# cure-lab/MagicDrive

Hardware: AMD Instinct MI355X
Metric: 6-view scenes/sec at 224x400, 50-step DDIM (higher is better)
Workload: dtype bf16; 1 GPU; configs[1]: 6-view 224x400, text-only conditioning (camera_param=None -> CFG off), 50-step DDIM, bf16; scenes_per_gpu=64, ddim_steps=50, scheduler=ddim, parallelism=scene-sharded x1, hipgraph=True, streams=2, output_type=latent

## Files before the change

include/mdx.h:

```cpp
#ifndef MDX_H_
#define MDX_H_

#include <stdint.h>

#ifdef __cplusplus
extern "C" {
#endif

#define MDX_OK 0
#define MDX_EINVAL (-1)
#define MDX_ELAUNCH (-2)
#define MDX_EUNSUPPORTED (-3)

#define MDX_ABI_VERSION 10

#define MDX_EPI_NONE 0
#define MDX_EPI_GEGLU 1
#define MDX_EPI_SILU 2

typedef struct MdxGemmDesc {
    const void* A; const void* W; void* C; const void* R;
    const float* bias; const float* temb; const int32_t* sel_ptr; float* ws;
    int64_t M, N, K;
    int64_t lda, ldw, ldc, ldr;
    int64_t batch, sA, sW, sC, sR;
    int64_t temb_sel_stride, temb_b_stride, rows_per_b;
    int64_t epilogue, splitk;
    int64_t c_is_f32;
    int64_t ws_bytes;
    void* Vt;
    int64_t vt_from, vt_T, vt_ld, vt_stride;
    double ln_eps;
    const float* ln_csum;
    void* ln_scratch;
    float* rowstat_out;
    int64_t rowstat_parts;
    const float* ln_stats;
    int64_t ln_stats_parts;
    const void* Wq;
} MdxGemmDesc;
int mdx_gemm_bf16(const MdxGemmDesc* d, void* stream);

typedef struct MdxConvDesc {
    const void* X; const void* Wt; void* Y; const void* R;
    const float* bias; const float* temb; const int32_t* sel_ptr; float* ws;
    int64_t B, Hi, Wi, Cin, Ho, Wo, Cout;
    int64_t kh, kw, sh, sw, ph, pw;
    int64_t ldx, ldy, ldr;
    int64_t temb_sel_stride, temb_b_stride;
    int64_t epilogue, splitk;
    int64_t ws_bytes, reserved1;
} MdxConvDesc;
int mdx_conv2d_bf16(const MdxConvDesc* d, void* stream);

typedef struct MdxConvDirectDesc {
    const void* X; const void* Wt; void* Y; const void* R;
    const float* bias; const float* temb; const int32_t* sel_ptr; void* reserved_p;
    int64_t B, Hi, Wi, Cin, Ho, Wo, Cout;
    int64_t kh, kw, sh, sw, ph, pw;
    int64_t ldx, ldy, ldr;
    int64_t temb_sel_stride, temb_b_stride;
    int64_t epilogue, x_is_f32, y_is_f32, reserved0;
} MdxConvDirectDesc;
int mdx_conv2d_direct(const MdxConvDirectDesc* d, void* stream);

typedef struct MdxAttnDesc {
    const void* Q; const void* K; const void* Vt; void* O;
    const int32_t* kvmap; void* reserved_p;
    int64_t B, H, Tq, Tk, d, nsrc;
    int64_t ldq, sQ, ldk, sK, ldv, sV, ldo, sO;
    double scale;
    int64_t joint;
    int64_t q_prescaled;
} MdxAttnDesc;
int mdx_attention_bf16(const MdxAttnDesc* d, void* stream);

typedef struct MdxGroupNormDesc {
    const void* X; void* Y; const float* gamma; const float* beta;
    int64_t B, HW, C, G, ldx, ldy;
    double eps;
    int64_t silu;
    float* ws; int64_t ws_bytes;
} MdxGroupNormDesc;
int mdx_groupnorm_bf16(const MdxGroupNormDesc* d, void* stream);

typedef struct MdxLayerNormDesc {
    const void* X; void* Y; const float* gamma; const float* beta;
    int64_t M, C, ldx, ldy;
    double eps;
    int64_t reserved0;
} MdxLayerNormDesc;
int mdx_layernorm_bf16(const MdxLayerNormDesc* d, void* stream);

typedef struct MdxSoftmaxDesc {
    const float* X; void* Y;
    int64_t rows, T, ldx, ldy;
    double scale;
    int64_t reserved0;
} MdxSoftmaxDesc;
int mdx_softmax_rows(const MdxSoftmaxDesc* d, void* stream);

#define MDX_EW_ADD 1
#define MDX_EW_COPY 2
#define MDX_EW_UPSAMPLE 3
#define MDX_EW_NCHW_TO_NHWC 4
#define MDX_EW_NHWC_TO_NCHW 5
#define MDX_EW_SILU 6
#define MDX_EW_SCALE 7
typedef struct MdxEwDesc {
    const void* X; void* Y; const int32_t* ymap; const int32_t* xmap;
    int64_t kind, M, C, ldx, ldy;
    int64_t B, Hi, Wi, Ho, Wo;
    int64_t x_is_f32, y_is_f32;
    double alpha;
} MdxEwDesc;
int mdx_elementwise(const MdxEwDesc* d, void* stream);

typedef struct MdxFourierDesc {
    const float* X; void* Y; const uint8_t* mask; const float* null_feat;
    int64_t n, P, F, ldy;
} MdxFourierDesc;
int mdx_fourier_embed(const MdxFourierDesc* d, void* stream);

typedef struct MdxGatherDesc {
    const void* T; void* Y; const int64_t* idx; const uint8_t* mask; const void* null_row; void* reserved_p;
    int64_t n, C, ldt, ldy, n_rows, reserved0;
} MdxGatherDesc;
int mdx_gather_rows(const MdxGatherDesc* d, void* stream);

typedef struct MdxTimeEmbDesc {
    const float* t; float* Y;
    int64_t n, dim, flip_sin_to_cos, ldy;
    double freq_shift, max_period;
} MdxTimeEmbDesc;
int mdx_timestep_embedding(const MdxTimeEmbDesc* d, void* stream);

typedef struct MdxDdimDesc {
    float* x; const float* eps; const float* coef; int32_t* step_ptr; void* x_in; void* reserved_p;
    int64_t n, cfg;
    double guidance;
    int64_t xin_c, xin_ld;
    const float* gv_cond; const float* gv_noise; const uint8_t* gv_mask;
    int64_t gv_mode, gv_view_elems, gv_last_step;
} MdxDdimDesc;
int mdx_cfg_ddim_step(const MdxDdimDesc* d, void* stream);

typedef struct MdxUniPCDesc {
    float* x; const float* eps; const float* coef; int32_t* step_ptr; void* x_in; float* x_last; float* m1; float* m2;
    int64_t n, cfg;
    double guidance;
    int64_t xin_c, xin_ld;
    const float* gv_cond; const float* gv_noise; const uint8_t* gv_mask;
    int64_t gv_mode, gv_view_elems, gv_last_step;
} MdxUniPCDesc;
int mdx_cfg_unipc_step(const MdxUniPCDesc* d, void* stream);

#define MDX_OP_GEMM 1
#define MDX_OP_CONV 2
#define MDX_OP_CONV_DIRECT 3
#define MDX_OP_ATTN 4
#define MDX_OP_GROUPNORM 5
#define MDX_OP_LAYERNORM 6
#define MDX_OP_EW 7
#define MDX_OP_FOURIER 8
#define MDX_OP_GATHER 9
#define MDX_OP_TIMEEMB 10
#define MDX_OP_DDIM 11
#define MDX_OP_UNIPC 12
#define MDX_OP_SOFTMAX 13

#define MDX_DTYPE_BF16 0
#define MDX_DTYPE_F16 1

#define MDX_OP_BYTES 512
typedef struct MdxOp {
    int64_t opcode;
    int64_t dtype;
    unsigned char desc[MDX_OP_BYTES - 16];
} MdxOp;

int mdx_gemm_f16(const MdxGemmDesc* d, void* stream);
int mdx_conv2d_f16(const MdxConvDesc* d, void* stream);
int mdx_conv2d_direct_f16(const MdxConvDirectDesc* d, void* stream);
int mdx_attention_f16(const MdxAttnDesc* d, void* stream);
int mdx_groupnorm_f16(const MdxGroupNormDesc* d, void* stream);
int mdx_layernorm_f16(const MdxLayerNormDesc* d, void* stream);
int mdx_elementwise_f16(const MdxEwDesc* d, void* stream);
int mdx_fourier_embed_f16(const MdxFourierDesc* d, void* stream);
int mdx_gather_rows_f16(const MdxGatherDesc* d, void* stream);
int mdx_timestep_embedding_f16(const MdxTimeEmbDesc* d, void* stream);
int mdx_cfg_ddim_step_f16(const MdxDdimDesc* d, void* stream);
int mdx_cfg_unipc_step_f16(const MdxUniPCDesc* d, void* stream);
int mdx_softmax_rows_f16(const MdxSoftmaxDesc* d, void* stream);

int mdx_program_run(const MdxOp* ops, int64_t n, void* stream);

int mdx_graph_create(const MdxOp* ops, int64_t n, void** graph_out);
int mdx_graph_launch(void* graph, void* stream);
int mdx_graph_destroy(void* graph);

int mdx_abi_version(void);
const char* mdx_build_id(void);
const char* mdx_last_error(void);
const char* mdx_last_kernel(void);
// ... 11 lines not shown
```

magicdrive_amd/_lib.py:

```python
from __future__ import annotations

import ctypes as C
import os
from typing import Dict, List, Tuple

_HERE = os.path.dirname(os.path.abspath(__file__))
LIB_PATH = os.environ.get("MDX_LIB_PATH") or os.path.join(_HERE, "libmdx.so")

ABI_VERSION = 10

OP_GEMM, OP_CONV, OP_CONV_DIRECT, OP_ATTN, OP_GROUPNORM, OP_LAYERNORM = 1, 2, 3, 4, 5, 6
OP_EW, OP_FOURIER, OP_GATHER, OP_TIMEEMB, OP_DDIM, OP_UNIPC, OP_SOFTMAX = 7, 8, 9, 10, 11, 12, 13
OP_BYTES = 512

EPI_NONE, EPI_GEGLU, EPI_SILU = 0, 1, 2
EW_ADD, EW_COPY, EW_UPSAMPLE, EW_NCHW_TO_NHWC, EW_NHWC_TO_NCHW, EW_SILU, EW_SCALE = 1, 2, 3, 4, 5, 6, 7

P, I, D = C.c_void_p, C.c_int64, C.c_double


def _struct(name: str, fields: List[Tuple[str, object]]):
    return type(name, (C.Structure,), {"_fields_": fields})


def _f(kind, names: str):
    return [(n, kind) for n in names.split()]


MdxGemmDesc = _struct("MdxGemmDesc", _f(P, "A W C R bias temb sel_ptr ws") + _f(I, "M N K lda ldw ldc ldr batch sA sW sC sR "
                      "temb_sel_stride temb_b_stride rows_per_b epilogue splitk c_is_f32 ws_bytes") + _f(P, "Vt") + _f(I, "vt_from vt_T vt_ld vt_stride")
                      + _f(D, "ln_eps") + _f(P, "ln_csum ln_scratch") + _f(P, "rowstat_out") + _f(I, "rowstat_parts") + _f(P, "ln_stats") + _f(I, "ln_stats_parts") + _f(P, "Wq"))
MdxConvDesc = _struct("MdxConvDesc", _f(P, "X Wt Y R bias temb sel_ptr ws") + _f(I, "B Hi Wi Cin Ho Wo Cout kh kw sh sw ph pw "
                      "ldx ldy ldr temb_sel_stride temb_b_stride epilogue splitk ws_bytes reserved1"))
MdxConvDirectDesc = _struct("MdxConvDirectDesc", _f(P, "X Wt Y R bias temb sel_ptr reserved_p") + _f(I, "B Hi Wi Cin Ho Wo Cout kh kw sh sw ph pw "
                            "ldx ldy ldr temb_sel_stride temb_b_stride epilogue x_is_f32 y_is_f32 reserved0"))
MdxAttnDesc = _struct("MdxAttnDesc", _f(P, "Q K Vt O kvmap reserved_p") + _f(I, "B H Tq Tk d nsrc ldq sQ ldk sK ldv sV ldo sO")
                      + _f(D, "scale") + _f(I, "joint q_prescaled"))
MdxGroupNormDesc = _struct("MdxGroupNormDesc", _f(P, "X Y gamma beta") + _f(I, "B HW C G ldx ldy") + _f(D, "eps") + _f(I, "silu") + _f(P, "ws") + _f(I, "ws_bytes"))
MdxLayerNormDesc = _struct("MdxLayerNormDesc", _f(P, "X Y gamma beta") + _f(I, "M C ldx ldy") + _f(D, "eps") + _f(I, "reserved0"))
MdxEwDesc = _struct("MdxEwDesc", _f(P, "X Y ymap xmap") + _f(I, "kind M C ldx ldy B Hi Wi Ho Wo x_is_f32 y_is_f32") + _f(D, "alpha"))
MdxFourierDesc = _struct("MdxFourierDesc", _f(P, "X Y mask null_feat") + _f(I, "n P F ldy"))
MdxGatherDesc = _struct("MdxGatherDesc", _f(P, "T Y idx mask null_row reserved_p") + _f(I, "n C ldt ldy n_rows reserved0"))
MdxTimeEmbDesc = _struct("MdxTimeEmbDesc", _f(P, "t Y") + _f(I, "n dim flip_sin_to_cos ldy") + _f(D, "freq_shift max_period"))
MdxDdimDesc = _struct("MdxDdimDesc", _f(P, "x eps coef step_ptr x_in reserved_p") + _f(I, "n cfg") + _f(D, "guidance") + _f(I, "xin_c xin_ld")
                      + _f(P, "gv_cond gv_noise gv_mask") + _f(I, "gv_mode gv_view_elems gv_last_step"))
MdxUniPCDesc = _struct("MdxUniPCDesc", _f(P, "x eps coef step_ptr x_in x_last m1 m2") + _f(I, "n cfg") + _f(D, "guidance") + _f(I, "xin_c xin_ld")
                       + _f(P, "gv_cond gv_noise gv_mask") + _f(I, "gv_mode gv_view_elems gv_last_step"))

MdxSoftmaxDesc = _struct("MdxSoftmaxDesc", _f(P, "X Y") + _f(I, "rows T ldx ldy") + _f(D, "scale") + _f(I, "reserved0"))
DESC_OF_OP = {
    OP_GEMM: MdxGemmDesc, OP_CONV: MdxConvDesc, OP_CONV_DIRECT: MdxConvDirectDesc, OP_ATTN: MdxAttnDesc,
    OP_GROUPNORM: MdxGroupNormDesc, OP_LAYERNORM: MdxLayerNormDesc, OP_EW: MdxEwDesc, OP_FOURIER: MdxFourierDesc,
    OP_GATHER: MdxGatherDesc, OP_TIMEEMB: MdxTimeEmbDesc, OP_DDIM: MdxDdimDesc, OP_UNIPC: MdxUniPCDesc, OP_SOFTMAX: MdxSoftmaxDesc,
}
DTYPE_BF16, DTYPE_F16 = 0, 1
ENTRY_OF_OP = {
    OP_GEMM: "mdx_gemm_bf16", OP_CONV: "mdx_conv2d_bf16", OP_CONV_DIRECT: "mdx_conv2d_direct", OP_ATTN: "mdx_attention_bf16",
    OP_GROUPNORM: "mdx_groupnorm_bf16", OP_LAYERNORM: "mdx_layernorm_bf16", OP_EW: "mdx_elementwise",
    OP_FOURIER: "mdx_fourier_embed", OP_GATHER: "mdx_gather_rows", OP_TIMEEMB: "mdx_timestep_embedding", OP_DDIM: "mdx_cfg_ddim_step",
    OP_UNIPC: "mdx_cfg_unipc_step", OP_SOFTMAX: "mdx_softmax_rows",
}
def entry_name(opcode: int, dtype: int = DTYPE_BF16) -> str:
    n = ENTRY_OF_OP[opcode]
    if dtype == DTYPE_BF16:
        return n
    return (n[:-5] if n.endswith("_bf16") else n) + "_f16"


EXPORTS = sorted(set(ENTRY_OF_OP.values()) | {entry_name(o, DTYPE_F16) for o in ENTRY_OF_OP} | {
    "mdx_program_run", "mdx_graph_create", "mdx_graph_launch", "mdx_graph_destroy",
    "mdx_abi_version", "mdx_build_id", "mdx_last_error", "mdx_last_kernel", "mdx_device_info", "mdx_set_option", "mdx_get_option", "mdx_option_name"})


class MdxOp(C.Structure):
    _fields_ = [("opcode", I), ("dtype", I), ("desc", C.c_ubyte * (OP_BYTES - 16))]


assert C.sizeof(MdxOp) == OP_BYTES
for _d in DESC_OF_OP.values():
    assert C.sizeof(_d) <= OP_BYTES - 16 and C.sizeof(_d) % 8 == 0


class MdxError(RuntimeError):
    pass


_LIB = None


def lib() -> C.CDLL:
    global _LIB
    if _LIB is not None:
        return _LIB
    if not os.path.exists(LIB_PATH):
        raise MdxError(
            f"{LIB_PATH} not found: build it with `python -c 'import __graft_entry__ as g; g.build()'` "
            f"or `make -C magicdrive_amd/csrc`. magicdrive_amd has no CPU / PyTorch fallback.")
    l = C.CDLL(LIB_PATH)
    for name in EXPORTS:
        if not hasattr(l, name):
            raise MdxError(f"libmdx.so does not export {name}")
    for name in list(ENTRY_OF_OP.values()) + [entry_name(o, DTYPE_F16) for o in ENTRY_OF_OP]:
        fn = getattr(l, name)
        fn.restype = C.c_int
        fn.argtypes = [C.c_void_p, C.c_void_p]
    l.mdx_program_run.restype = C.c_int
    l.mdx_program_run.argtypes = [C.c_void_p, C.c_int64, C.c_void_p]
    l.mdx_graph_create.restype = C.c_int
    l.mdx_graph_create.argtypes = [C.c_void_p, C.c_int64, C.POINTER(C.c_void_p)]
    l.mdx_graph_launch.restype = C.c_int
    l.mdx_graph_launch.argtypes = [C.c_void_p, C.c_void_p]
    l.mdx_graph_destroy.restype = C.c_int
    l.mdx_graph_destroy.argtypes = [C.c_void_p]
    l.mdx_abi_version.restype = C.c_int
    l.mdx_last_error.restype = C.c_char_p
    l.mdx_build_id.restype = C.c_char_p
    l.mdx_last_kernel.restype = C.c_char_p
    l.mdx_device_info.restype = C.c_int
    l.mdx_device_info.argtypes = [C.POINTER(C.c_int64)]
    l.mdx_set_option.restype = C.c_int
    l.mdx_set_option.argtypes = [C.c_char_p, C.c_int64]
    l.mdx_get_option.restype = C.c_int
    l.mdx_get_option.argtypes = [C.c_char_p, C.POINTER(C.c_int64)]
    l.mdx_option_name.restype = C.c_char_p
    l.mdx_option_name.argtypes = [C.c_int64]
    if l.mdx_abi_version() != ABI_VERSION:
        raise MdxError(f"libmdx.so ABI {l.mdx_abi_version()} != expected {ABI_VERSION}")
    _LIB = l
    return l


def check(rc: int, what: str = "") -> None:
    if rc != 0:
        msg = lib().mdx_last_error()
        raise MdxError(f"{what} failed (rc={rc}): {msg.decode() if msg else ''}")


def call_op(opcode: int, desc: C.Structure, stream: int, dtype: int = DTYPE_BF16) -> None:
    name = entry_name(opcode, dtype)
    fn = getattr(lib(), name)
    check(fn(C.byref(desc), C.c_void_p(stream)), name)


class Program:

    def __init__(self, ops: List[Tuple]):
        self.n = len(ops)
        self.buf = (MdxOp * max(self.n, 1))()
        for i, t in enumerate(ops):
            code, desc = t[0], t[1]
            self.buf[i].opcode = code
            self.buf[i].dtype = t[2] if len(t) > 2 else DTYPE_BF16
            C.memmove(C.addressof(self.buf[i]) + 16, C.byref(desc), C.sizeof(desc))
        self._graph = C.c_void_p(None)

    def run(self, stream: int) -> None:
        check(lib().mdx_program_run(C.byref(self.buf), self.n, C.c_void_p(stream)), "mdx_program_run")

    def capture(self) -> None:
        if not self._graph:
            check(lib().mdx_graph_create(C.byref(self.buf), self.n, C.byref(self._graph)), "mdx_graph_create")

    def launch(self, stream: int) -> None:
        if not self._graph:
            self.capture()
        check(lib().mdx_graph_launch(self._graph, C.c_void_p(stream)), "mdx_graph_launch")

    def destroy(self) -> None:
        if self._graph and _LIB is not None:
            _LIB.mdx_graph_destroy(self._graph)
        self._graph = C.c_void_p(None)

    def __del__(self):
        try:
            self.destroy()
        except Exception:
            pass


def set_option(key: str, value: int) -> None:
    check(lib().mdx_set_option(key.encode(), int(value)), f"mdx_set_option({key})")


def get_option(key: str) -> int:
    v = C.c_int64(0)
    check(lib().mdx_get_option(key.encode(), C.byref(v)), f"mdx_get_option({key})")
# ... 39 lines not shown
```

magicdrive_amd/csrc/gemm_conv.hip:

```cpp
#include "common.h"
#include "launch.h"
#include "options.h"
#include "gemm_params.h"

namespace mdx {


int launch_gemm_ws(const GCParams& p, hipStream_t st);
bool ws_supported(const GCParams& p);
bool ws_fuses_layernorm(const GCParams& p);
int launch_layernorm_plain(const bf16_t* X, bf16_t* Y, int M, int C, long ldx, long ldy, float eps, hipStream_t st);
int launch_rowstat(const bf16_t* X, int M, int C, long ldx, float* stat, int parts, hipStream_t st);
bool ws_emits_rowstat(const GCParams& p);
int launch_gemm_xl(const GCParams& p, bool conv, int bn, hipStream_t st);
bool xl_supported(const GCParams& p, bool conv, int bn);

template <int BM, int BN, int BK, int WM, int WN, bool CONV, bool PIPE>
__global__ __launch_bounds__(WM * WN * 64, (WM * WN >= 8) ? 2 : 1) void gemm_conv_kernel(GCParams p) {
    constexpr int NTH = WM * WN * 64;
    constexpr int LSTR = BK + 8;
    constexpr int KCH = BK / 8;
    constexpr int TM = BM / (WM * 32), TN = BN / (WN * 32);
    constexpr int A_CH = BM * BK / 8 / NTH;
    constexpr int B_CH = BN * BK / 8 / NTH;
// ... 190 lines not shown
        if (t + 1 < nt) store_tile(buf ^ 1);
        __syncthreads();
    }

    if (p.timing) ts2 = __builtin_amdgcn_s_memtime();
    if (coalesced_out) {
        epilogue_coalesced<BM, BN, TM, TN, NTH>(p, zb, m0, n0, wm * TM * 32, wn * TN * 32, lane, tid, acc, smem, er);
        if (p.timing && tid == 0) {
            unsigned long long* t = p.timing + 5 * ((long)tile_n * p.mt + tile_m);
            t[0] = ts0; t[1] = ts1; t[2] = ts2; t[3] = __builtin_amdgcn_s_memtime();
            t[4] = 0;
        }
        return;
    }
    const int half = lane >> 5;
#pragma unroll
    for (int i = 0; i < TM; ++i) {
        const int m = m0 + wm * TM * 32 + i * 32 + frow;
        if (m >= p.M) continue;
#pragma unroll
        for (int j = 0; j < TN; ++j) {
#pragma unroll
            for (int g = 0; g < 4; ++g) {
                const int nb = n0 + wn * TN * 32 + j * 32 + 8 * g + 4 * half;
                if (nb >= p.N) continue;
                float v[4] = {acc[i][j][4 * g], acc[i][j][4 * g + 1], acc[i][j][4 * g + 2], acc[i][j][4 * g + 3]};
                if (p.splitk > 1) {
                    float* w = p.ws + ((long)kz * p.M + m) * p.N + nb;
                    *(float4*)w = make_float4(v[0], v[1], v[2], v[3]);
                } else if (p.epi == 1) {
                    if (TN == 2 && j == 0) {
                        float gte[4] = {acc[i][TN - 1][4 * g], acc[i][TN - 1][4 * g + 1],
                                        acc[i][TN - 1][4 * g + 2], acc[i][TN - 1][4 * g + 3]};
                        epilogue_store(p, zb, m, nb, v, gte);
                    }
                } else {
                    epilogue_store(p, zb, m, nb, v, nullptr);
                }
            }
        }
    }
}

__global__ __launch_bounds__(256) void splitk_reduce_kernel(GCParams p) {
    const int n4 = p.N / 4;
    long idx = (long)blockIdx.x * 256 + threadIdx.x;
    if (idx >= (long)p.M * n4) return;
    int m = (int)(idx / n4);
    int nb = (int)(idx - (long)m * n4) * 4;
    const bool geglu = p.epi == 1;
    if (geglu && (nb & 63) >= 32) return;
    const int sel = (p.temb && p.sel) ? *p.sel : 0;
    float bv[4] = {0, 0, 0, 0}, bg[4] = {0, 0, 0, 0}, tv[4] = {0, 0, 0, 0};
    if (p.bias) {
#pragma unroll
        for (int j = 0; j < 4; ++j) { bv[j] = p.bias[nb + j]; if (geglu) bg[j] = p.bias[nb + 32 + j]; }
    }
    if (p.temb && !geglu) {
        const float* tb = p.temb + (long)sel * p.temb_sel_stride + (long)(m / p.rows_per_b) * p.temb_b_stride;
#pragma unroll
        for (int j = 0; j < 4; ++j) tv[j] = tb[nb + j];
    }
    const int ncol = geglu ? (nb >> 6) * 32 + (nb & 63) : nb;
    float rf[4] = {0, 0, 0, 0};
    if (p.R) {
        if (p.c_f32) {
            const float4 r4 = *(const float4*)((const float*)p.R + (long)m * p.ldr + ncol);
            rf[0] = r4.x; rf[1] = r4.y; rf[2] = r4.z; rf[3] = r4.w;
        } else {
            const uint2 rv = *(const uint2*)((const bf16_t*)p.R + (long)m * p.ldr + ncol);
            rf[0] = bf2f((bf16_t)(rv.x & 0xffff)); rf[1] = bf2f((bf16_t)(rv.x >> 16));
            rf[2] = bf2f((bf16_t)(rv.y & 0xffff)); rf[3] = bf2f((bf16_t)(rv.y >> 16));
        }
    }
    float v[4] = {0, 0, 0, 0}, g[4] = {0, 0, 0, 0};
    const float* w0 = p.ws + (long)m * p.N + nb;
    const long zs = (long)p.M * p.N;
    const int last = p.splitk - 1;
    for (int z0 = 0; z0 < p.splitk; z0 += 4) {
        float4 a[4], b[4];
#pragma unroll
        for (int i = 0; i < 4; ++i) {
            const float* w = w0 + (long)min(z0 + i, last) * zs;
            a[i] = *(const float4*)w;
            if (geglu) b[i] = *(const float4*)(w + 32);
        }
#pragma unroll
        for (int i = 0; i < 4; ++i) {
            const bool ok = z0 + i <= last;
            v[0] = ok ? v[0] + a[i].x : v[0]; v[1] = ok ? v[1] + a[i].y : v[1]; v[2] = ok ? v[2] + a[i].z : v[2]; v[3] = ok ? v[3] + a[i].w : v[3];
            if (geglu) { g[0] = ok ? g[0] + b[i].x : g[0]; g[1] = ok ? g[1] + b[i].y : g[1]; g[2] = ok ? g[2] + b[i].z : g[2]; g[3] = ok ? g[3] + b[i].w : g[3]; }
        }
    }
    float o[4];
#pragma unroll
    for (int j = 0; j < 4; ++j) {
        if (geglu) {
            float h = v[j], gt = g[j];
            if (p.bias) { h += bv[j]; gt += bg[j]; }
            o[j] = h * gelu_erf_f(gt);
        } else {
            float x = v[j];
            if (p.bias) x += bv[j];
            if (p.temb) x += tv[j];
            if (p.epi == 2) x = silu_f(x);
            o[j] = x;
        }
        if (p.R) o[j] += rf[j];
    }
    if (p.c_f32) {
        *(float4*)((float*)p.C + (long)m * p.ldc + ncol) = make_float4(o[0], o[1], o[2], o[3]);
    } else {
        uint2 ov; ov.x = pack2bf(o[0], o[1]); ov.y = pack2bf(o[2], o[3]);
        *(uint2*)((bf16_t*)p.C + (long)m * p.ldc + ncol) = ov;
    }
}

template <int BM, int BN, int BK, int WM, int WN, bool CONV, bool PIPE>
static int launch_one_(const GCParams& p, hipStream_t st) {
    constexpr size_t ring = (size_t)2 * (BM + BN) * (BK + 8) * sizeof(bf16_t), ctile = (size_t)BM * (BN + 8) * 2;
    constexpr size_t smem = ring > ctile ? ring : ctile;
    if (p.rowstat) return set_error(MDX_EINVAL, "gemm_conv_kernel: rowstat_out reached a route that does not emit row statistics");
    auto kern = gemm_conv_kernel<BM, BN, BK, WM, WN, CONV, PIPE>;
    if (int rc = ensure_dyn_smem((const void*)kern, smem, "gemm_conv")) return rc;
    GCParams q = p;
    q.mt = (p.M + BM - 1) / BM; q.nt = (p.N + BN - 1) / BN;
    const int swz = (int)opt(OPT_GEMM_SWZ);
    q.swz = swz && q.nt > 1 && q.mt >= 128;
    const unsigned nblk = q.swz ? (unsigned)((q.mt + 7) / 8 * 8 * q.nt) : (unsigned)(q.mt * q.nt);
    dim3 grid(nblk, 1, p.batch > 1 ? p.batch : p.splitk);
    hipLaunchKernelGGL(kern, grid, dim3(WM * WN * 64), smem, st, q);
    char tag[96];
    snprintf(tag, sizeof tag, "gemm_conv_kernel<%d,%d,%d,%d,%d,%s>", BM, BN, BK, WM, WN, CONV ? "conv" : "gemm");
    return check_launch(tag);
}

template <int BM, int BN, int BK, int WM, int WN, bool CONV>
static int launch_one(const GCParams& p, hipStream_t st) {
    const int pipe = (int)opt(OPT_GEMM_PIPE);
    if constexpr (BM == 128 && BN == 128 && BK == 64 && WM == 2 && WN == 2) {
        if (pipe) return launch_one_<BM, BN, BK, WM, WN, CONV, true>(p, st);
    }
    return launch_one_<BM, BN, BK, WM, WN, CONV, false>(p, st);
}

int launch_gemm_conv(GCParams p, bool conv, hipStream_t st) {
    if (p.M <= 0 || p.N <= 0 || p.K <= 0) return MDX_OK;
    const bool geglu = p.epi == 1;
    {
        const long nout = geglu ? p.N / 2 : p.N;
        const int wide_on = (int)opt(OPT_EPI_WIDE);
        p.wide = wide_on && !p.c_f32 && (nout % 8) == 0 && (p.ldc % 8) == 0 && (p.sC % 8) == 0 && (((uintptr_t)p.C) & 15) == 0 &&
                 (!p.R || ((p.ldr % 8) == 0 && (p.sR % 8) == 0 && (((uintptr_t)p.R) & 15) == 0));
    }
    if (!opt(OPT_LN_STATS)) { p.rowstat = nullptr; p.rowstat_parts = 0; p.ln_stats = nullptr; p.ln_stats_parts = 0; }
    if (geglu && (p.N % 64) != 0) return set_error(MDX_EINVAL, "GEGLU needs packed N %% 64 == 0 (N=%d)", p.N);
    constexpr int impl = 0;
    const int ws_mode = (int)opt(OPT_GEMM_WS);
    const int xl_mode = (int)opt(OPT_GEMM_XL);
    const int xl_k320 = (int)opt(OPT_XL_K320);
    const int xl_min_tiles = (int)opt(OPT_XL_MIN_TILES);
    const int xl_geglu320 = (int)opt(OPT_XL_GEGLU320);
    const bool geglu_xl = xl_geglu320 && xl_mode == 1 && impl == 0 && !conv && geglu && p.K == 320 && p.splitk <= 1 && ws_mode < 2 &&
                          xl_supported(p, false, 256) && (long)((p.M + 255) / 256) * ((p.N + 255) / 256) >= 1024;
    const bool ws_first = !conv && ws_mode > 0 && p.splitk <= 1 && ws_supported(p) && (ws_mode >= 2 || p.M >= 8192);
    const bool ws_taken = impl == 0 && !geglu_xl && ws_first && !(xl_k320 && xl_mode > 0);
    if (p.rowstat) {
        if (conv || p.batch > 1 || p.epi != 0 || p.c_f32 || p.Vt || p.rowstat_parts < 1) return set_error(MDX_EINVAL, "rowstat_out: plain 2-D GEMM with 16-bit C only");
        if (!(ws_taken && ws_emits_rowstat(p) && opt(OPT_LN_FUSE))) {
            GCParams q = p;
            q.rowstat = nullptr; q.rowstat_parts = 0;
            if (int rc = launch_gemm_conv(q, conv, st)) return rc;
            return launch_rowstat((const bf16_t*)p.C, p.M, p.N, p.ldc, p.rowstat, p.rowstat_parts, st);
        }
    }
    auto try_xl = [&](int& bn_out) -> bool {
        if (impl != 0 || xl_mode <= 0 || p.splitk > 1) return false;
        const int xl_bn = (int)opt(OPT_XL_BN);
        double best = 1e300;
        bn_out = 0;
        const double nslab = p.K / 64.0;
        for (int bn : {320, 256, 160}) {
            if (xl_bn && bn != xl_bn) continue;
            if (!xl_supported(p, conv, bn)) continue;
            const long t = (long)((p.M + 255) / 256) * ((p.N + bn - 1) / bn);
            if (xl_mode < 2 && t < xl_min_tiles) continue;
            const double a = bn == 320 ? 23.7 : bn == 256 ? 13.4 : 16.6, b = bn == 320 ? 1.896 : bn == 256 ? 1.565 : 1.116;
            const double c = (double)((t + 255) / 256) * (a + b * nslab);
            if (c < best) { best = c; bn_out = bn; }
        }
        return bn_out != 0;
    };
    if (p.ln_eps > 0.f) {
        if (conv || p.batch > 1) return set_error(MDX_EINVAL, "fused LayerNorm: plain 2-D GEMM only");
        if (!(ws_taken && ws_fuses_layernorm(p) && opt(OPT_LN_FUSE))) {
            if (!p.ln_scratch) return set_error(MDX_EINVAL, "fused LayerNorm: this shape is not normalised in-kernel and no ln_scratch was given");
            if (int rc = launch_layernorm_plain(p.A, p.ln_scratch, p.M, p.K, p.lda, p.lda, p.ln_eps, st)) return rc;
            p.A = p.ln_scratch; p.ln_eps = 0.f; p.ln_csum = nullptr; p.ln_stats = nullptr; p.ln_stats_parts = 0;
        }
    }
    if (xl_mode >= 2 && p.splitk <= 1 && p.batch <= 1 && !(p.K == 320 && !conv && !xl_k320)) {
        GCParams q = p;
        q.splitk = 1;
        int bn_f;
        const int keep = p.splitk;
        p.splitk = 1;
        const bool ok = try_xl(bn_f);
        p.splitk = keep;
        if (ok) return launch_gemm_xl(q, conv, bn_f, st);
    }
    if (geglu_xl) return launch_gemm_xl(p, false, 256, st);
    if (ws_taken) return launch_gemm_ws(p, st);
    int BM, BN;
    {
        BN = 128;
        if (!geglu && (p.N <= 64 || (p.N % 128 != 0 && p.N <= 192))) BN = 64;
        BM = p.M >= 2048 ? 128 : 64;
        if (opt(OPT_GEMM_SMALL_TILES) && p.batch <= 1) {
            const long t64 = (long)((p.M + 63) / 64) * ((p.N + 63) / 64);
            if (geglu) {
                BM = p.M >= 512 ? 128 : 64;
            } else if (!conv) {
                if (t64 <= 1408) BM = BN = 64;
            } else if (t64 * (long)((p.K + 63) / 64) <= 40000) {
                BM = BN = 64;
            } else if (BN == 128) {
                BM = 128;
            }
        }
        const int big = (int)opt(OPT_GEMM_BM256);
        if (big && BN == 128 && p.M >= big) BM = 256;
        const int fbm = (int)opt(OPT_GEMM_BM), fbn = (int)opt(OPT_GEMM_BN);
        if (fbm == 64 || fbm == 128) BM = fbm;
        if ((fbn == 64 && !geglu) || fbn == 128) BN = fbn;
    }
    long tiles = (long)((p.M + BM - 1) / BM) * ((p.N + BN - 1) / BN) * (p.batch > 1 ? p.batch : 1);
    int splitk = 1;
    if (p.splitk > 0) {
        splitk = p.splitk;
    } else if (p.batch <= 1 && p.ws && tiles < 384 && p.K >= 1024 && (p.N % 4) == 0) {
        long want = (768 + tiles - 1) / tiles;
        long maxs = p.K / 512;
        splitk = (int)min(min(want, maxs), 32L);
        if (splitk < 1) splitk = 1;
    }
    if (p.batch > 1) splitk = 1;
    if (splitk > 1) {
        long per = (long)p.M * p.N * (long)sizeof(float);
        long fit = per > 0 ? p.ws_bytes / per : 0;
        if (fit < splitk) splitk = fit < 1 ? 1 : (int)fit;
    }
    constexpr int BK = 64;
    int kchunk = ((p.K + splitk - 1) / splitk + BK - 1) / BK * BK;
    splitk = (p.K + kchunk - 1) / kchunk;
    if (splitk > 1 && !p.ws) return set_error(MDX_EINVAL, "split-K needs a workspace");
    p.splitk = splitk;
    p.kchunk = kchunk;
    const int timing = (int)opt(OPT_GEMM_TIMING);
    p.timing = (timing && p.ws && splitk == 1) ? (unsigned long long*)p.ws : nullptr;
    if (splitk == 1) {
        int bn_xl;
        if (try_xl(bn_xl)) return launch_gemm_xl(p, conv, bn_xl, st);
    }
    if (impl == 0 && ws_first) return launch_gemm_ws(p, st);
    int rc;
    {
        const int bk = (int)opt(OPT_GEMM_BK);
#define MDX_GC2(BM_, BN_, BK_, WM_, WN_) (conv ? launch_one<BM_, BN_, BK_, WM_, WN_, true>(p, st) : launch_one<BM_, BN_, BK_, WM_, WN_, false>(p, st))
#define MDX_GC(BM_, BN_) (bk == 32 ? MDX_GC2(BM_, BN_, 32, 2, 2) : MDX_GC2(BM_, BN_, 64, 2, 2))
        if (BM == 256 && BN == 128) rc = (bk == 32) ? MDX_GC2(256, 128, 32, 4, 2) : MDX_GC2(256, 128, 64, 4, 2);
        else if (BM == 128 && BN == 128) rc = MDX_GC(128, 128);
        else if (BM == 128 && BN == 64) rc = MDX_GC(128, 64);
        else if (BM == 64 && BN == 128) rc = MDX_GC(64, 128);
        else rc = MDX_GC(64, 64);
#undef MDX_GC2
#undef MDX_GC
    }
    if (rc != MDX_OK) return rc;
    if (splitk > 1) {
        long n = (long)p.M * (p.N / 4);
        hipLaunchKernelGGL(splitk_reduce_kernel, dim3((unsigned)((n + 255) / 256)), dim3(256), 0, st, p);
        return check_launch("splitk_reduce_kernel", false);
    }
    return MDX_OK;
}

}

using namespace mdx;

static int check_common(const char* op, int64_t K, int64_t lda, int64_t ldw, int64_t ldc, int64_t ldr, const void* A, const void* W,
                        const void* C, const char* nA, const char* nW, const char* nC, const char* nlda, const char* nldc) {
    MDX_NEED(need_multiple(op, "K", K, 8));
    MDX_NEED(need_multiple(op, nlda, lda, 8));
    MDX_NEED(need_multiple(op, "ldw", ldw, 8));
    MDX_NEED(need_multiple(op, nldc, ldc, 4));
    MDX_NEED(need_multiple(op, "ldr", ldr, 4));
    MDX_NEED(need_aligned(op, nA, A, 16));
    MDX_NEED(need_aligned(op, nW, W, 16));
    MDX_NEED(need_aligned(op, nC, C, 8));
    return MDX_OK;
}

static int check_epilogue_operands(const char* op, const void* R, const float* bias, const float* temb, const int32_t* sel, const float* ws,
                                   int64_t temb_sel_stride, int64_t temb_b_stride) {
    MDX_NEED(need_aligned(op, "R", R, 8));
    MDX_NEED(need_aligned(op, "bias", bias, 16));
    MDX_NEED(need_aligned(op, "temb", temb, 16));
    MDX_NEED(need_aligned(op, "sel_ptr", sel, 4));
    MDX_NEED(need_aligned(op, "ws", ws, 16));
    if (temb) {
        MDX_NEED(need_multiple(op, "temb_sel_stride", temb_sel_stride, 4));
        MDX_NEED(need_multiple(op, "temb_b_stride", temb_b_stride, 4));
    }
    return MDX_OK;
}

static int launch_gemm_flat(const mdx::GCParams& q, hipStream_t st) {
    using namespace mdx;
    const int xl_mode = (int)opt(OPT_GEMM_XL);
    if (xl_mode <= 0) return MDX_EUNSUPPORTED;
    double best = 1e300; int bn_best = 0;
    for (int bn : {320, 256, 160}) {
        if (!xl_supported(q, false, bn)) continue;
        const long t = (long)((q.M + 255) / 256) * ((q.N + bn - 1) / bn);
        if (t < 128) continue;
        const double a = bn == 320 ? 23.7 : bn == 256 ? 13.4 : 16.6, b = bn == 320 ? 1.896 : bn == 256 ? 1.565 : 1.116;
        const double c = (double)((t + 255) / 256) * (a + b * q.K / 64.0);
        if (c < best) { best = c; bn_best = bn; }
    }
    if (!bn_best) return MDX_EUNSUPPORTED;
    return launch_gemm_xl(q, false, bn_best, st);
}

extern "C" int mdx_gemm_bf16(const MdxGemmDesc* d, void* stream) {
    if (!d || !d->A || !d->W || !d->C) return set_error(MDX_EINVAL, "mdx_gemm_bf16: null operand");
    const char* op = "mdx_gemm_bf16";
    MDX_NEED(need_int(op, "M", d->M)); MDX_NEED(need_int(op, "N", d->N)); MDX_NEED(need_int(op, "K", d->K));
    MDX_NEED(need_int(op, "batch", d->batch)); MDX_NEED(need_int(op, "rows_per_b", d->rows_per_b));
    MDX_NEED(need_int(op, "splitk", d->splitk));
    MDX_NEED(check_common(op, d->K, d->lda, d->ldw, d->ldc, d->ldr, d->A, d->W, d->C, "A", "W", "C", "lda", "ldc"));
    MDX_NEED(check_epilogue_operands(op, d->R, d->bias, d->temb, d->sel_ptr, d->ws, d->temb_sel_stride, d->temb_b_stride));
    if (d->c_is_f32) {
        MDX_NEED(need_aligned(op, "C (fp32)", d->C, 16));
        MDX_NEED(need_aligned(op, "R (fp32)", d->R, 16));
    }
    if (d->batch > 1) {
        MDX_NEED(need_multiple(op, "sA", d->sA, 8)); MDX_NEED(need_multiple(op, "sW", d->sW, 8));
        MDX_NEED(need_multiple(op, "sC", d->sC, 4)); MDX_NEED(need_multiple(op, "sR", d->sR, 4));
    }
    if (d->N % 4) {
        if (d->bias || d->temb || d->R || d->epilogue || d->splitk > 1 || d->ldc < (d->N + 3) / 4 * 4)
            return set_error(MDX_EINVAL, "N=%ld not a multiple of 4 needs a plain epilogue and ldc >= roundup4(N)", (long)d->N);
    }
    GCParams p = {};
    p.A = (const bf16_t*)d->A; p.W = (const bf16_t*)d->W; p.C = d->C; p.R = d->R;
    p.bias = d->bias; p.temb = d->temb; p.sel = d->sel_ptr; p.ws = d->ws;
    p.M = (int)d->M; p.N = (int)d->N; p.K = (int)d->K;
    p.lda = d->lda; p.ldw = d->ldw; p.ldc = d->ldc; p.ldr = d->ldr;
    p.batch = d->batch > 1 ? (int)d->batch : 1;
    p.sA = d->sA; p.sW = d->sW; p.sC = d->sC; p.sR = d->sR;
    p.temb_sel_stride = d->temb_sel_stride; p.temb_b_stride = d->temb_b_stride;
    p.rows_per_b = d->rows_per_b > 0 ? (int)d->rows_per_b : 1;
    p.epi = (int)d->epilogue; p.splitk = (int)d->splitk; p.c_f32 = (int)d->c_is_f32; p.ws_bytes = d->ws_bytes;
    if (d->ln_eps > 0.0) {
        if (!d->ln_csum || p.batch > 1 || d->splitk > 1 || d->c_is_f32 || d->temb || ((uintptr_t)d->ln_scratch & 15))
            return set_error(MDX_EINVAL, "mdx_gemm_bf16: fused LayerNorm needs ln_csum, one batch, no split-K / fp32 C / temb, 16-byte aligned ln_scratch");
        p.ln_eps = (float)d->ln_eps; p.ln_csum = d->ln_csum; p.ln_scratch = (bf16_t*)d->ln_scratch;
        if (d->ln_stats) {
            if (d->ln_stats_parts < 1 || ((uintptr_t)d->ln_stats & 7)) return set_error(MDX_EINVAL, "mdx_gemm_bf16: ln_stats needs ln_stats_parts >= 1 and 8-byte alignment");
            p.ln_stats = d->ln_stats; p.ln_stats_parts = (int)d->ln_stats_parts;
        }
    } else if (d->ln_stats) {
        return set_error(MDX_EINVAL, "mdx_gemm_bf16: ln_stats without ln_eps");
    }
    if (d->Wq) {
        if ((uintptr_t)d->Wq & 15) return set_error(MDX_EINVAL, "mdx_gemm_bf16: Wq must be 16-byte aligned");
        p.Wq = (const bf16_t*)d->Wq;
    }
    if (d->rowstat_out) {
        if (d->rowstat_parts < 1 || ((uintptr_t)d->rowstat_out & 7) || d->Vt || d->epilogue || d->c_is_f32 || p.batch > 1)
            return set_error(MDX_EINVAL, "mdx_gemm_bf16: rowstat_out needs rowstat_parts >= 1, 8-byte alignment, a plain epilogue, 16-bit C, one batch, no Vt");
        p.rowstat = d->rowstat_out; p.rowstat_parts = (int)d->rowstat_parts;
    }
    if (d->Vt) {
        p.Vt = (bf16_t*)d->Vt; p.vt_from = (int)d->vt_from; p.vt_T = (int)d->vt_T; p.vt_ld = d->vt_ld; p.vt_stride = d->vt_stride;
        if (!ws_supported(p) || d->epilogue || d->R || (d->vt_from % 128) || d->vt_from <= 0 || d->vt_from >= d->N || d->vt_T <= 0 ||
            (d->vt_T % 8) || (d->M % d->vt_T) || (d->vt_ld % 8) || (d->vt_stride % 8) || ((uintptr_t)d->Vt & 15))
            return set_error(MDX_EINVAL, "mdx_gemm_bf16: transposed V output needs K=320, plain epilogue, no residual, vt_from %% 128 == 0, vt_T %% 8 == 0, aligned Vt");
        if (!opt(OPT_LN_STATS)) { p.ln_stats = nullptr; p.ln_stats_parts = 0; }
        if (p.ln_eps > 0.f && !opt(OPT_LN_FUSE)) {
            if (!p.ln_scratch) return set_error(MDX_EINVAL, "fused LayerNorm: LN_FUSE=0 needs ln_scratch");
            if (int rc2 = launch_layernorm_plain(p.A, p.ln_scratch, p.M, p.K, p.lda, p.lda, p.ln_eps, (hipStream_t)stream)) return rc2;
            p.A = p.ln_scratch; p.ln_eps = 0.f; p.ln_csum = nullptr; p.ln_stats = nullptr; p.ln_stats_parts = 0;
        }
        { GCParams q = p; const long nout = d->vt_from;
          q.wide = (nout % 8) == 0 && (p.ldc % 8) == 0 && (((uintptr_t)p.C) & 15) == 0;
          return launch_gemm_ws(q, (hipStream_t)stream); }
    }
    const int flatten = (int)opt(OPT_GEMM_FLATTEN);
    if (flatten && p.batch > 1 && p.sA == 0 && p.sW == (long)p.N * p.ldw && !p.bias && !p.temb && !p.R && !p.epi && !p.c_f32 && p.splitk <= 1 &&
        (long)p.batch * p.N < 0x7fffff00L && ((long)p.batch * p.N) % 4 == 0) {
        GCParams q = p;
        q.col_split = p.N; q.N = p.batch * p.N; q.batch = 1; q.sW = 0; q.wide = 0;
        int rcq = launch_gemm_flat(q, (hipStream_t)stream);
        if (rcq != MDX_EUNSUPPORTED) return rcq;
    }
    return launch_gemm_conv(p, false, (hipStream_t)stream);
}

extern "C" int mdx_conv2d_bf16(const MdxConvDesc* d, void* stream) {
    if (!d || !d->X || !d->Wt || !d->Y) return set_error(MDX_EINVAL, "mdx_conv2d_bf16: null operand");
    if (d->Cin % 8) return set_error(MDX_EINVAL, "mdx_conv2d_bf16: Cin=%ld must be a multiple of 8", (long)d->Cin);
    const char* op = "mdx_conv2d_bf16";
    MDX_NEED(need_int(op, "B", d->B)); MDX_NEED(need_int(op, "Hi", d->Hi)); MDX_NEED(need_int(op, "Wi", d->Wi)); MDX_NEED(need_int(op, "Cin", d->Cin));
    MDX_NEED(need_int(op, "Ho", d->Ho)); MDX_NEED(need_int(op, "Wo", d->Wo)); MDX_NEED(need_int(op, "Cout", d->Cout));
    MDX_NEED(need_int(op, "kh", d->kh)); MDX_NEED(need_int(op, "kw", d->kw)); MDX_NEED(need_int(op, "sh", d->sh)); MDX_NEED(need_int(op, "sw", d->sw));
    MDX_NEED(need_int(op, "ph", d->ph)); MDX_NEED(need_int(op, "pw", d->pw)); MDX_NEED(need_int(op, "splitk", d->splitk));
    if (d->B < 0 || d->Ho < 0 || d->Wo < 0 || d->kh < 0 || d->kw < 0 || d->Cin < 0) return set_error(MDX_EINVAL, "%s: negative size", op);
    MDX_NEED(need_int(op, "Ho * Wo", d->Ho * d->Wo));
    MDX_NEED(need_int(op, "B * Ho * Wo", d->B * (d->Ho * d->Wo)));
    MDX_NEED(need_int(op, "kh * kw", d->kh * d->kw));
    int64_t K = d->kh * d->kw * d->Cin;
    MDX_NEED(need_int(op, "kh * kw * Cin", K));
    MDX_NEED(check_common(op, K, d->ldx, K, d->ldy, d->ldr, d->X, d->Wt, d->Y, "X", "Wt", "Y", "ldx", "ldy"));
    MDX_NEED(check_epilogue_operands(op, d->R, d->bias, d->temb, d->sel_ptr, d->ws, d->temb_sel_stride, d->temb_b_stride));
    if (d->epilogue == MDX_EPI_GEGLU) return set_error(MDX_EINVAL, "conv has no GEGLU epilogue");
    if (d->Cout % 4) return set_error(MDX_EINVAL, "mdx_conv2d_bf16: Cout=%ld must be a multiple of 4", (long)d->Cout);
    GCParams p = {};
    p.A = (const bf16_t*)d->X; p.W = (const bf16_t*)d->Wt; p.C = d->Y; p.R = d->R;
    p.bias = d->bias; p.temb = d->temb; p.sel = d->sel_ptr; p.ws = d->ws;
    p.M = (int)(d->B * d->Ho * d->Wo); p.N = (int)d->Cout; p.K = (int)K;
    p.lda = d->ldx; p.ldw = K; p.ldc = d->ldy; p.ldr = d->ldr;
    p.batch = 1;
    p.temb_sel_stride = d->temb_sel_stride; p.temb_b_stride = d->temb_b_stride;
    p.rows_per_b = (int)(d->Ho * d->Wo);
    p.epi = (int)d->epilogue; p.splitk = (int)d->splitk; p.c_f32 = 0; p.ws_bytes = d->ws_bytes;
    p.Hi = (int)d->Hi; p.Wi = (int)d->Wi; p.Cin = (int)d->Cin; p.Ho = (int)d->Ho; p.Wo = (int)d->Wo;
    p.kh = (int)d->kh; p.kw = (int)d->kw; p.sh = (int)d->sh; p.sw = (int)d->sw; p.ph = (int)d->ph; p.pw = (int)d->pw;
    const int cim = (int)opt(OPT_CONV_CIMAJOR);
    p.cimajor = (cim && d->kh * d->kw > 1 && d->Cin % 64 == 0) ? 1 : 0;
    return launch_gemm_conv(p, true, (hipStream_t)stream);
}
```

magicdrive_amd/csrc/gemm_params.h:

```cpp
#pragma once
#include "common.h"

namespace mdx {

struct GCParams {
    const bf16_t* A; const bf16_t* W; void* C; const void* R;
    const float* bias; const float* temb; const int* sel; float* ws;
    int M, N, K;
    long lda, ldw, ldc, ldr;
    long sA, sW, sC, sR;
    long temb_sel_stride, temb_b_stride;
    int rows_per_b;
    int epi, splitk, kchunk, c_f32, batch;
    long ws_bytes;
    int mt, nt, swz;
    int gm, gn;
    int nblk;
    unsigned long long* timing;
    int Hi, Wi, Cin, Ho, Wo, kh, kw, sh, sw, ph, pw;
    int cimajor;
    int wide;
    bf16_t* Vt; int vt_from, vt_T; long vt_ld, vt_stride;
    int col_split;
    const float* ln_csum; float ln_eps; bf16_t* ln_scratch;
    float* rowstat; int rowstat_parts;
    const float* ln_stats; int ln_stats_parts;
    const bf16_t* Wq;
    int dbg;
};

__device__ __forceinline__ bool tile_coords_at(const GCParams& p, int bid, int& tm, int& tn) {
    if (!p.swz) { tm = bid % p.mt; tn = bid / p.mt; return true; }
    const int xcd = bid & 7, local = bid >> 3;
    tn = local % p.nt;
    tm = (local / p.nt) * 8 + xcd;
    return tm < p.mt;
}
__device__ __forceinline__ bool tile_coords(const GCParams& p, int& tm, int& tn) { return tile_coords_at(p, (int)blockIdx.x, tm, tn); }

__device__ __forceinline__ void epilogue_store(const GCParams& p, long zb, int m, int nb,
                                               const float* v, const float* gte) {
    float o[4];
    int ncol;
    const float* tb = nullptr;
    if (p.temb) {
        int sel = p.sel ? *p.sel : 0;
        tb = p.temb + (long)sel * p.temb_sel_stride + (long)(m / p.rows_per_b) * p.temb_b_stride;
    }
    if (p.epi == 1) {
        ncol = (nb >> 6) * 32 + (nb & 63);
#pragma unroll
        for (int j = 0; j < 4; ++j) {
            float h = v[j], g = gte[j];
            if (p.bias) { h += p.bias[nb + j]; g += p.bias[nb + 32 + j]; }
            o[j] = h * gelu_erf_f(g);
        }
    } else {
        ncol = nb;
#pragma unroll
        for (int j = 0; j < 4; ++j) {
            float x = v[j];
            if (p.bias) x += p.bias[nb + j];
            if (tb) x += tb[nb + j];
            if (p.epi == 2) x = silu_f(x);
            o[j] = x;
        }
    }
    if (p.c_f32) {
        float* c = (float*)p.C + zb * p.sC + (long)m * p.ldc + ncol;
        if (p.R) {
            const float* r = (const float*)p.R + zb * p.sR + (long)m * p.ldr + ncol;
#pragma unroll
            for (int j = 0; j < 4; ++j) o[j] += r[j];
        }
        *(float4*)c = make_float4(o[0], o[1], o[2], o[3]);
    } else {
        bf16_t* c = (bf16_t*)p.C + zb * p.sC + (long)m * p.ldc + ncol;
        if (p.R) {
            const bf16_t* r = (const bf16_t*)p.R + zb * p.sR + (long)m * p.ldr + ncol;
            uint2 rv = *(const uint2*)r;
            o[0] += bf2f((bf16_t)(rv.x & 0xffff)); o[1] += bf2f((bf16_t)(rv.x >> 16));
            o[2] += bf2f((bf16_t)(rv.y & 0xffff)); o[3] += bf2f((bf16_t)(rv.y >> 16));
        }
        uint2 ov; ov.x = pack2bf(o[0], o[1]); ov.y = pack2bf(o[2], o[3]);
        *(uint2*)c = ov;
    }
}


template <int BM, int BN, int TN, int NTHR>
struct EpiRegs {
    static constexpr int IT = (BM * (BN / 8) + NTHR - 1) / NTHR;
    float4 bv[TN][4];
    uint4 rv[IT];
};

template <int BM, int BN, int TN, int NTHR>
__device__ __forceinline__ void epi_prefetch(const GCParams& p, long zb, int m0, int n0, int wcol0, int lane, int tid,
                                             EpiRegs<BM, BN, TN, NTHR>& er) {
    const int half = lane >> 5;
    const float4 z4 = make_float4(0.f, 0.f, 0.f, 0.f);
#pragma unroll
    for (int j = 0; j < TN; ++j)
#pragma unroll
        for (int g = 0; g < 4; ++g) {
            const int nb = n0 + wcol0 + j * 32 + 8 * g + 4 * half;
            er.bv[j][g] = (p.bias && nb < p.N) ? *(const float4*)(p.bias + nb) : z4;
        }
    const bool geglu = p.epi == 1;
    const int cpr = (geglu ? BN / 2 : BN) / 8;
    const int n0o = geglu ? n0 / 2 : n0, Nout = geglu ? p.N / 2 : p.N;
    const bf16_t* Rg = (p.R && p.wide) ? (const bf16_t*)p.R + zb * p.sR : nullptr;
#pragma unroll
    for (int i = 0; i < EpiRegs<BM, BN, TN, NTHR>::IT; ++i) {
        const int idx = tid + i * NTHR;
        const int row = idx / cpr;
        const int c8 = (idx - row * cpr) * 8;
        const int m = m0 + row, n = n0o + c8;
        er.rv[i] = make_uint4(0, 0, 0, 0);
        if (Rg && idx < BM * cpr && m < p.M && n < Nout) er.rv[i] = *(const uint4*)(Rg + (long)m * p.ldr + n);
    }
}

__device__ __forceinline__ unsigned add2bf(unsigned a, unsigned b) {
    return pack2bf(bf2f((bf16_t)(a & 0xffff)) + bf2f((bf16_t)(b & 0xffff)), bf2f((bf16_t)(a >> 16)) + bf2f((bf16_t)(b >> 16)));
}

template <int BM, int BNO, int NTHR, int ITMAX>
__device__ __forceinline__ void store_tile_rows(const GCParams& p, long zb, int m0, int n0o, int Nout, int tid, const bf16_t* Cs,
                                                const uint4 (&rv)[ITMAX]) {
    constexpr int CSTR = BNO + 8;
    bf16_t* Cg = (bf16_t*)p.C + zb * p.sC;
    const bool has_r = p.R != nullptr;
    if (p.wide) {
        constexpr int CPR = BNO / 8;
        constexpr int IT = (BM * CPR + NTHR - 1) / NTHR;
        static_assert(IT <= ITMAX, "residual register tile too small");
#pragma unroll
        for (int i = 0; i < IT; ++i) {
            const int idx = tid + i * NTHR;
            const int row = idx / CPR;
            const int c8 = (idx - row * CPR) * 8;
            const int m = m0 + row, n = n0o + c8;
            if (!((idx < BM * CPR) && m < p.M && n < Nout)) continue;
            uint4 v = *(const uint4*)(Cs + row * CSTR + c8);
            if (has_r) { v.x = add2bf(v.x, rv[i].x); v.y = add2bf(v.y, rv[i].y); v.z = add2bf(v.z, rv[i].z); v.w = add2bf(v.w, rv[i].w); }
            *(uint4*)(Cg + (long)m * p.ldc + n) = v;
        }
        return;
    }
    constexpr int CPR = BNO / 4;
    constexpr int IT = (BM * CPR + NTHR - 1) / NTHR;
    const bf16_t* Rg = has_r ? (const bf16_t*)p.R + zb * p.sR : nullptr;
#pragma unroll 1
    for (int i0 = 0; i0 < IT; i0 += 4) {
        uint2 r2[4];
        bool ok[4];
#pragma unroll
        for (int u = 0; u < 4; ++u) {
            const int idx = tid + (i0 + u) * NTHR;
            const int row = idx / CPR, c4 = (idx - row * CPR) * 4;
            ok[u] = (i0 + u) < IT && idx < BM * CPR && m0 + row < p.M && n0o + c4 < Nout;
            r2[u] = make_uint2(0, 0);
            if (Rg && ok[u]) r2[u] = *(const uint2*)(Rg + (long)(m0 + row) * p.ldr + n0o + c4);
        }
#pragma unroll
        for (int u = 0; u < 4; ++u) {
            if (!ok[u]) continue;
            const int idx = tid + (i0 + u) * NTHR;
            const int row = idx / CPR, c4 = (idx - row * CPR) * 4;
            uint2 v = *(const uint2*)(Cs + row * CSTR + c4);
            if (has_r) { v.x = add2bf(v.x, r2[u].x); v.y = add2bf(v.y, r2[u].y); }
            *(uint2*)(Cg + (long)(m0 + row) * p.ldc + n0o + c4) = v;
        }
    }
}

template <int BM, int BN, int TM, int TN, int NTHR>
__device__ __forceinline__ void epilogue_coalesced(const GCParams& p, long zb, int m0, int n0, int wrow0, int wcol0, int lane,
                                                   int tid, f32x16_t (&acc)[TM][TN], unsigned char* smem,
                                                   const EpiRegs<BM, BN, TN, NTHR>& er) {
    const bool geglu = p.epi == 1;
// ... 65 lines not shown
```

magicdrive_amd/csrc/gemm_xl.hip:

```cpp
#include "common.h"
#include "launch.h"
#include "options.h"
#include "gemm_params.h"
#include "xl_layout.h"
#include "xl_dma.h"
#include <type_traits>

namespace mdx {

using namespace mdx_xl;

constexpr int XL_SLOTS = 12;

__device__ __forceinline__ bool xl_tile_coords_at(const GCParams& p, int bid, int& tm, int& tn) {
    if (p.swz != 2) return tile_coords_at(p, bid, tm, tn);
    return raster_tile(bid, p.mt, p.nt, p.gm, p.gn, &tm, &tn);
}
__device__ __forceinline__ bool xl_tile_coords(const GCParams& p, int& tm, int& tn) { return xl_tile_coords_at(p, (int)blockIdx.x, tm, tn); }

template <int BN, bool CONV, int SCHED>
__global__ __launch_bounds__(512, 2) void gemm_xl_kernel(GCParams p) {
    using G = Geo<BN>;
    constexpr int BM = 256, NTH = 512;
    constexpr int TI = G::TI, TJ = G::TJ, TJ0 = G::TJ0, TJ1 = TJ - TJ0, TIH = TI / 2;
    constexpr int A_BYTES = BM * 128, B_BYTES = G::BNP * 128, BUF = A_BYTES + B_BYTES;
    constexpr int PA = G::PA, PB0 = G::PB0, PB1 = G::PB1;
    constexpr int UNIT_MAX = PA > PB0 ? PA : PB0;
    constexpr bool KXS = SCHED == 4;
    static_assert(!KXS || (BN == 320 && CONV), "the shared-tap schedule is the 320-wide conv's");
    constexpr int AS_ROWS = 272, AS_BYTES = AS_ROWS * 128;
    constexpr int ZROW_OFF = 264 * 128;
    constexpr int B_STRIDE = KXS ? (G::BNP * 128) : (BM * 128 + G::BNP * 128);
    constexpr int B_BASE = KXS ? 2 * AS_BYTES - BM * 128 : 0;
    extern __shared__ __attribute__((aligned(16))) unsigned char smem[];

    const int tid = threadIdx.x, lane = tid & 63;
    const int wave = __builtin_amdgcn_readfirstlane(tid >> 6);
    const int grp = wave >> 2;
    const int wm = wave % G::WM, wn = wave / G::WM;
    int tile_m, tile_n;
    if (!xl_tile_coords(p, tile_m, tile_n)) return;
    unsigned long long ts_[8] = {0, 0, 0, 0, 0, 0, 0, 0};
#define XL_STAMP(k) if (p.timing) ts_[k] = __builtin_amdgcn_s_memtime();
    XL_STAMP(0)
    const int m0 = tile_m * BM, n0 = tile_n * BN;
    const int nt = p.K / 64;

    long a_base_el;
    int hw = 1, Wo = 1;
    if (CONV) {
        hw = p.Ho * p.Wo; Wo = p.Wo;
        const int b = m0 / hw, rem = m0 - b * hw;
        const int oy = rem / Wo, ox = rem - oy * Wo;
        a_base_el = (((long)b * p.Hi + (oy * p.sh - p.ph)) * p.Wi + (ox * p.sw - p.pw)) * p.lda;
    } else {
        a_base_el = (long)m0 * p.lda;
    }
    const xl_rsrc_t rsA = xl_make_rsrc(p.A + a_base_el);
    const xl_rsrc_t rsB = xl_make_rsrc(p.W + (long)n0 * p.ldw);
    const unsigned lds0 = (unsigned)(unsigned long long)(lds_void_t*)smem;

    unsigned xs_bits = 0;
    const unsigned xs_vb = (unsigned)((long)(lane >> 3) * p.lda * 2 + (((lane & 7) ^ ((lane >> 3) & 7)) << 4));
    const unsigned xb_vb = (unsigned)((long)(lane >> 3) * p.ldw * 2 + (((lane & 7) ^ ((lane >> 4) & 3)) << 4));
    unsigned a_voff[2][PA];
    unsigned a_taps[2][PA];
    int a_lds[2][PA];
#pragma unroll
    for (int h = 0; h < 2; ++h)
#pragma unroll
        for (int e = 0; e < PA; ++e) {
            const int row0 = a_piece_row0<BN>(h, wave, e);
            a_lds[h][e] = row0 * 128;
            const int R = piece_lane_row(row0, lane);
            const int cl = piece_lane_chunk(row0, lane);
            const int m = m0 + R;
            a_taps[h][e] = 0;
            if constexpr (KXS) {
                const long q = (long)m0 + R - 1;
                unsigned bits = 0;
                if (q >= 0 && q < p.M) {
                    const int b_ = (int)(q / hw), y_ = (int)(q - (long)b_ * hw) / Wo;
#pragma unroll
                    for (int ky = 0; ky < 3; ++ky) if ((unsigned)(y_ + ky - 1) < (unsigned)p.Hi) bits |= 1u << ky;
                }
                xs_bits |= bits << (3 * (2 * h + e));
            } else
            if (CONV) {
                const int mm = min(m, p.M - 1);
                const int b = mm / hw, rem = mm - b * hw;
                const int oy = rem / Wo, ox = rem - oy * Wo;
                const int iy0 = oy * p.sh - p.ph, ix0 = ox * p.sw - p.pw;
                const long pix = ((long)b * p.Hi + iy0) * p.Wi + ix0;
                a_voff[h][e] = (unsigned)((pix * p.lda - a_base_el) * 2 + cl * 16);
                unsigned bits = 0;
#pragma unroll
                for (int t = 0; t < 9; ++t) {
                    const int iy = iy0 + t / 3, ix = ix0 + t % 3;
                    if (m < p.M && (unsigned)iy < (unsigned)p.Hi && (unsigned)ix < (unsigned)p.Wi) bits |= 1u << t;
                }
                a_taps[h][e] = bits;
            } else {
                a_voff[h][e] = m < p.M ? (unsigned)(((long)R * p.lda) * 2 + cl * 16) : XL_OOB;
            }
        }
    unsigned b_voff[2][UNIT_MAX];
    int b_lds[2][UNIT_MAX];
#pragma unroll
    for (int part = 0; part < 2; ++part)
#pragma unroll
        for (int e = 0; e < (part ? PB1 : PB0); ++e) {
            const int row0 = b_piece_row0<BN>(part, wave, e);
            if (row0 < 0) {
                b_lds[part][e] = A_BYTES + b_dummy_row0<BN>(wave) * 128;
                b_voff[part][e] = XL_OOB;
            } else {
                b_lds[part][e] = A_BYTES + row0 * 128;
                const int R = piece_lane_row(row0, lane);
                const int cl = piece_lane_chunk(row0, lane);
                b_voff[part][e] = (n0 + R < p.N) ? (unsigned)(((long)R * p.ldw) * 2 + cl * 16) : XL_OOB;
            }
        }

    if constexpr (KXS) {
        const int R = 256 + (lane >> 3);
        const long q = (long)m0 + R - 1;
        if (wave == 7 && R < 258 && q < p.M) {
            const int b_ = (int)(q / hw), y_ = (int)(q - (long)b_ * hw) / Wo;
#pragma unroll
            for (int ky = 0; ky < 3; ++ky) if ((unsigned)(y_ + ky - 1) < (unsigned)p.Hi) xs_bits |= 1u << (12 + ky);
        }
    }
    const int row_bytes = (int)(p.lda * 2);
    auto a_soff = [&](int T, int& tap) -> int {
        if (CONV) {
            const int cb = T / 9;
            tap = T - cb * 9;
            const int ky = tap / 3, kx = tap - ky * 3;
            return (ky * p.Wi + kx) * row_bytes + cb * 128;
        }
        tap = 0;
        return T * 128;
    };
    auto b_soff = [&](int T) -> int {
        if (CONV) {
            const int cb = T / 9, tap = T - cb * 9;
            return (tap * p.Cin + cb * 64) * 2;
        }
        return T * 128;
    };
#ifdef MDX_XL_ABLATE
    const bool do_mma = !(p.dbg & 1), do_dma = !(p.dbg & 2);
    const bool a_oob = CONV && (p.dbg & 16), a_skip = CONV && (p.dbg & 32);
    const bool a_oob_kx = CONV && (p.dbg & 64);
#else
    constexpr bool do_mma = true, do_dma = true, a_oob = false, a_skip = false, a_oob_kx = false;
#endif
#define XL_PIECE_A(h, e, T)                                                                                                       \
    if constexpr ((e) < PA) {                                                                                                     \
        if ((T) < nt && do_dma && !(a_skip && ((T) % 9) != 0)) {                                                                  \
            int tap_;                                                                                                             \
            const int so_ = a_soff((T), tap_);                                                                                    \
            unsigned vo_ = CONV ? (((a_taps[h][(e) < PA ? (e) : 0] >> tap_) & 1u) ? a_voff[h][(e) < PA ? (e) : 0] : XL_OOB)       \
                                : a_voff[h][(e) < PA ? (e) : 0];                                                                  \
            if ((a_oob && tap_ != 0) || (a_oob_kx && (tap_ % 3) != 0)) vo_ = XL_OOB;                                              \
            xl_glds(rsA, lds0 + ((T) & 1) * BUF + a_lds[h][(e) < PA ? (e) : 0], vo_, so_);                                        \
        }                                                                                                                         \
    }
#define XL_PIECE_B(part, e, T)                                                                                                    \
    if constexpr ((e) < ((part) ? PB1 : PB0)) {                                                                                   \
        if ((T) < nt && do_dma)                                                                                                   \
            xl_glds_b(rsB, lds0 + ((T) & 1) * B_STRIDE + B_BASE + b_lds[part][(e) < UNIT_MAX ? (e) : 0],                            \
                      b_voff[part][(e) < UNIT_MAX ? (e) : 0], b_soff((T)));                                                       \
    }
#define XL_ISSUE_A(h, T) { XL_PIECE_A(h, 0, T) XL_PIECE_A(h, 1, T) }
#define XS_PIECE_A(h, e, G)                                                                                                       \
    if ((G) < ng && do_dma) {                                                                                                     \
        unsigned va_ = xs_vb;                                                                                                     \
        asm volatile("" : "+v"(va_));                                                                                             \
        const unsigned vo_ = va_ + (unsigned)((a_lds[h][e] >> 7) * row_bytes);                                                    \
        xl_glds(rsA, lds0 + ((G) & 1) * AS_BYTES + a_lds[h][e], ((xs_bits >> (3 * (2 * (h) + (e)) + xs_ky)) & 1u) ? vo_ : XL_OOB, xs_so); \
    }
#define XS_PIECE_B(part, e, T)                                                                                                    \
    if constexpr ((e) < ((part) ? PB1 : PB0)) {                                                                                   \
        if ((T) < nt && do_dma) {                                                                                                 \
            const int r0_ = (b_lds[part][(e) < UNIT_MAX ? (e) : 0] - A_BYTES) >> 7;                                               \
            unsigned vb_ = xb_vb;                                                                                                 \
            asm volatile("" : "+v"(vb_));    \
            const unsigned vo_ = (vb_ ^ (unsigned)(((r0_ >> 3) & 1) << 6)) + (unsigned)(r0_ * (int)(p.ldw * 2));                  \
            xl_glds_b(rsB, lds0 + ((T) & 1) * B_STRIDE + B_BASE + b_lds[part][(e) < UNIT_MAX ? (e) : 0], vo_, b_soff((T)));        \
        }                                                                                                                         \
    }
#define XS_ISSUE_B(part, T) { XS_PIECE_B(part, 0, T) XS_PIECE_B(part, 1, T) XS_PIECE_B(part, 2, T) }
#define XS_ISSUE_A0(G) { XS_PIECE_A(0, 0, G) XS_PIECE_A(0, 1, G) }
#define XS_ISSUE_A1X(G)                                                                                                           \
    {                                                                                                                             \
        XS_PIECE_A(1, 0, G) XS_PIECE_A(1, 1, G)                                                                                   \
        unsigned va2_ = xs_vb;                                                                                                    \
        asm volatile("" : "+v"(va2_));                                                                                            \
        if ((G) < ng && do_dma)                                                                                                   \
            xl_glds(rsA, lds0 + ((G) & 1) * AS_BYTES + (wave == 7 ? 256 * 128 : ZROW_OFF),                                        \
                    ((xs_bits >> (12 + xs_ky)) & 1u) ? va2_ + (unsigned)(256 * row_bytes) : XL_OOB, xs_so);                       \
    }
#define XL_ISSUE_B(part, T) { XL_PIECE_B(part, 0, T) XL_PIECE_B(part, 1, T) XL_PIECE_B(part, 2, T) }

    const int fo0 = frag_off(0, lane, 0), fo1 = frag_off(0, lane, 1);
    const int a_rd = a_tile_row0<BN>(wm, 0) * 128;
    const int b_rd = A_BYTES + b_tile_row0<BN>(wn, 0) * 128;
    if constexpr (KXS) {
#pragma unroll
        for (int i = 0; i < TI; ++i) {
            const int m_ = m0 + a_tile_row0<BN>(wm, i) + (lane & 15);
            const int ox_ = m_ % Wo;
            if (ox_ == 0) xs_bits |= 1u << (16 + i);
            if (ox_ == Wo - 1) xs_bits |= 1u << (24 + i);
        }
    }

    f32x4_t acc[TI][TJ];
#pragma unroll
    for (int i = 0; i < TI; ++i)
#pragma unroll
        for (int j = 0; j < TJ; ++j)
#pragma unroll
            for (int r = 0; r < 4; ++r) acc[i][j][r] = 0.f;

    constexpr int NBF = (BN == 320) ? TJ0 : TJ;
    Frag8 af[TIH][2], bfr[NBF][2];
#define XL_READ_A(h, buf_)                                                                                                        \
    {                                                                                                                             \
        const unsigned char* s_ = smem + (buf_) * BUF + a_rd + (h) * TIH * 2048;                                                  \
        _Pragma("unroll") for (int i = 0; i < TIH; ++i) {                                                                         \
            af[i][0].u = *(const uint4*)(s_ + i * 2048 + fo0);                                                                    \
            af[i][1].u = *(const uint4*)(s_ + i * 2048 + fo1);                                                                    \
        }                                                                                                                         \
    }
#define XS_READ_A(h, ab_)                                                                                                         \
    {                                                                                                                             \
        const unsigned char* s_ = smem + (ab_) * AS_BYTES;                                                                        \
        unsigned bb_ = xs_bsel;                                                                                                   \
        asm volatile("" : "+v"(bb_));    \
        const int f0_ = xs_f0, f1_ = xs_f0 ^ 64;                                                                                  \
        _Pragma("unroll") for (int i = 0; i < TIH; ++i) {                                                                         \
            const int it_ = (h) * TIH + i;                                                                                        \
            const bool z_ = (bb_ >> it_) & 1u;                                                                                    \
            const int o0_ = z_ ? ZROW_OFF - it_ * 2048 : f0_, o1_ = z_ ? ZROW_OFF - it_ * 2048 : f1_;                             \
            af[i][0].u = *(const uint4*)(s_ + o0_ + it_ * 2048);                                                                  \
            af[i][1].u = *(const uint4*)(s_ + o1_ + it_ * 2048);                                                                  \
        }                                                                                                                         \
    }
#define XL_READ_B(J0, NJ, buf_)                                                                                                   \
    {                                                                                                                             \
        const unsigned char* s_ = smem + (buf_) * B_STRIDE + B_BASE + b_rd;                                                       \
        _Pragma("unroll") for (int j = (J0); j < (J0) + (NJ); ++j) {                                                              \
            bfr[j][0].u = *(const uint4*)(s_ + j * 2048 + fo0);                                                                   \
            bfr[j][1].u = *(const uint4*)(s_ + j * 2048 + fo1);                                                                   \
        }                                                                                                                         \
    }
#define XL_READ_B_TO(D0, J0, NJ, buf_)                                                                                            \
    {                                                                                                                             \
        const unsigned char* s_ = smem + (buf_) * B_STRIDE + B_BASE + b_rd;                                                       \
        _Pragma("unroll") for (int j = 0; j < (NJ); ++j) {                                                                        \
            bfr[(D0) + j][0].u = *(const uint4*)(s_ + ((J0) + j) * 2048 + fo0);                                                   \
            bfr[(D0) + j][1].u = *(const uint4*)(s_ + ((J0) + j) * 2048 + fo1);                                                   \
        }                                                                                                                         \
    }
#define XL_MMA_TO(h, D0, J0, NJ)                                                                                                  \
    if (do_mma) {                                                                                                                 \
        __builtin_amdgcn_s_setprio(1);                                                                                            \
        _Pragma("unroll") for (int kk = 0; kk < 2; ++kk)                                                                          \
            _Pragma("unroll") for (int i = 0; i < TIH; ++i)                                                                       \
                _Pragma("unroll") for (int j = 0; j < (NJ); ++j)                                                                  \
                    acc[(h) * TIH + i][(J0) + j] =                                                                                \
                        MDX_MFMA_16x16x32(bfr[(D0) + j][kk].v, af[i][kk].v, acc[(h) * TIH + i][(J0) + j]); \
        __builtin_amdgcn_s_setprio(0);                                                                                            \
    }
#define XL_MMA(h, J0, NJ)                                                                                                         \
    if (do_mma) {                                                                                                                 \
        __builtin_amdgcn_s_setprio(1);                                                                                            \
        _Pragma("unroll") for (int kk = 0; kk < 2; ++kk)                                                                          \
            _Pragma("unroll") for (int i = 0; i < TIH; ++i)                                                                       \
                _Pragma("unroll") for (int j = (J0); j < (J0) + (NJ); ++j)                                                        \
                    acc[(h) * TIH + i][j] =                                                                                       \
                        MDX_MFMA_16x16x32(bfr[j][kk].v, af[i][kk].v, acc[(h) * TIH + i][j]);       \
        __builtin_amdgcn_s_setprio(0);                                                                                            \
    }
#define XL_MSEG(h, I0, I1, I2, I3)                                                                                                \
    {                                                                                                                             \
        __builtin_amdgcn_s_setprio(1);                                                                                            \
        constexpr int P_ = 2 * TIH;                                                                                               \
        _Pragma("unroll") for (int pr = 0; pr < P_; ++pr) {                                                                       \
            const int kk = pr / TIH, i = pr % TIH;                                                                                \
            if (pr == 1) { I0 }                                                                                                   \
            if (pr == 1 + (P_ - 1) / 4) { I1 }                                                                                    \
            if (pr == 1 + 2 * (P_ - 1) / 4) { I2 }                                                                                \
            if (pr == 1 + 3 * (P_ - 1) / 4) { I3 }                                                                                \
            __builtin_amdgcn_sched_barrier(0);                                                                                    \
            if (do_mma) {                                                                                                         \
                _Pragma("unroll") for (int j = 0; j < TJ; ++j)                                                                    \
// ... 170 lines not shown
            XL_READ_B(TJ0, TJ1, buf)
            XL_SEG2(XL_ISSUE_B(0, t + 1))
            XL_MMA(0, TJ0, TJ1)
            XL_MMA_END()
            XL_READ_A(1, buf)
            XL_SEG2(XL_ISSUE_A(0, t + 2))
            XL_MMA(1, TJ0, TJ1)
            XL_MMA_END()
            XL_SEG2(XL_ISSUE_B(1, t + 2) if (t + 2 < nt) xl_wait_vmcnt<PA + PB1>(); else xl_wait_vmcnt<0>();)
            XL_MMA(1, 0, TJ0)
            XL_MMA_END()
        }
#undef XL_SEG2
    } else     if constexpr (SCHED == 0) {
        constexpr int INFLIGHT = PA + PB0 + PB1;
        XL_ISSUE_A(0, 0)
        XL_ISSUE_B(0, 0)
        XL_ISSUE_B(1, 0)
        XL_ISSUE_A(1, 0)
        XL_ISSUE_A(0, 1)
        XL_ISSUE_B(0, 1)
        XL_ISSUE_B(1, 1)
        if (nt > 1) xl_wait_vmcnt<INFLIGHT>(); else xl_wait_vmcnt<0>();
        __builtin_amdgcn_s_barrier();
        __builtin_amdgcn_sched_barrier(0);
        XL_STAMP(2)
        if (grp == 1) {
            __builtin_amdgcn_s_barrier();
            __builtin_amdgcn_sched_barrier(0);
        }
        for (int t = 0; t < nt; ++t) {
            const int buf = t & 1;
            XL_READ_A(0, buf)
            XL_READ_B(0, TJ0, buf)
            XL_ISSUE_A(1, t + 1)
            XL_SEG_END()
            XL_MMA(0, 0, TJ0)
            XL_MMA_END()
            XL_READ_B(TJ0, TJ1, buf)
            XL_ISSUE_A(0, t + 2)
            XL_SEG_END()
            XL_MMA(0, TJ0, TJ1)
            XL_MMA_END()
            XL_READ_A(1, buf)
            XL_ISSUE_B(0, t + 2)
            XL_SEG_END()
            XL_MMA(1, TJ0, TJ1)
            XL_MMA_END()
            XL_ISSUE_B(1, t + 2)
            if (t + 2 < nt) xl_wait_vmcnt<INFLIGHT>(); else xl_wait_vmcnt<0>();
            XL_SEG_END()
            XL_MMA(1, 0, TJ0)
            XL_MMA_END()
        }
    } else {
        XL_ISSUE_A(0, 0)
        XL_ISSUE_B(0, 0)
        XL_ISSUE_B(1, 0)
        XL_ISSUE_A(1, 0)
        XL_ISSUE_A(0, 1)
        XL_ISSUE_B(0, 1)
        if (nt > 1) xl_wait_vmcnt<PA + PB0>(); else xl_wait_vmcnt<0>();
        __builtin_amdgcn_s_barrier();
        __builtin_amdgcn_sched_barrier(0);
        XL_STAMP(2)
        if (grp == 1) {
            __builtin_amdgcn_s_barrier();
            __builtin_amdgcn_sched_barrier(0);
        }
        for (int t = 0; t < nt; ++t) {
            const int buf = t & 1;
            XL_READ_A(0, buf)
            XL_READ_B(0, TJ, buf)
            if (t + 1 < nt) xl_wait_vmcnt<PA + PB0>(); else xl_wait_vmcnt<0>();
            XL_SEG_END()
            XL_MSEG(0, XL_PIECE_B(1, 0, t + 1), XL_PIECE_B(1, 1, t + 1), XL_PIECE_A(1, 0, t + 1), XL_PIECE_A(1, 1, t + 1))
            XL_MMA_END()
            XL_READ_A(1, buf)
            if (t + 1 < nt) xl_wait_vmcnt<PA>();
            XL_SEG_END()
            XL_MSEG(1, XL_PIECE_A(0, 0, t + 2), XL_PIECE_A(0, 1, t + 2), XL_PIECE_B(0, 0, t + 2), XL_PIECE_B(0, 1, t + 2))
            XL_MMA_END()
        }
    }
    if (grp == 0) {
        __builtin_amdgcn_s_barrier();
        __builtin_amdgcn_sched_barrier(0);
    }
#undef XL_PIECE_A
#undef XS_PIECE_A
#undef XS_PIECE_B
#undef XS_ISSUE_B
#undef XS_ISSUE_A0
#undef XS_ISSUE_A1X
#undef XS_READ_A
#undef XL_PIECE_B
#undef XL_ISSUE_A
#undef XL_ISSUE_B
#undef XL_READ_A
#undef XL_READ_B
#undef XL_READ_B_TO
#undef XL_MMA_TO
#undef XL_MMA
#undef XL_MSEG
#undef XL_SEG_END
#undef XL_MMA_END

    XL_STAMP(3)
#ifdef MDX_XL_ABLATE
    if (p.dbg & 4) return;
#endif
    constexpr int NH = (BN == 320) ? 2 : 1;
    constexpr int HROWS = BM / NH;
    const bool geglu = p.epi == 1;
    const bool has_t = p.temb != nullptr && !geglu;
    const int BNo = geglu ? BN / 2 : BN;
    const int CSTR = BNo + 8;
    bf16_t* Cs = (bf16_t*)smem;
    float* addend = (float*)(smem + (size_t)HROWS * (BN + 8) * 2);
    const int b0 = has_t ? m0 / p.rows_per_b : 0;
    if (add_early) {
#pragma unroll
        for (int u = 0; u < ADD_N; ++u) {
            const int idx = u * NTH + tid;
            if (idx < BN) addend[idx] = (n0 + idx < p.N) ? addb[u] : 0.f;
        }
    } else {
        const int nslots = has_t ? XL_SLOTS : 1;
        const int sel = (has_t && p.sel) ? *p.sel : 0;
        const int bmax = has_t ? (p.M - 1) / p.rows_per_b : 0;
        for (int idx = tid; idx < nslots * BN; idx += NTH) {
            const int slot = idx / BN, n = idx - slot * BN, col = n0 + n;
            float v = 0.f;
            if (col < p.N) {
                if (p.bias) v = p.bias[col];
                if (has_t && b0 + slot <= bmax) v += p.temb[(long)sel * p.temb_sel_stride + (long)(b0 + slot) * p.temb_b_stride + col];
            }
            addend[idx] = v;
        }
    }
    const int n0o = geglu ? n0 / 2 : n0, Nout = geglu ? p.N / 2 : p.N;
    const bf16_t* Rg = p.R ? (const bf16_t*)p.R : nullptr;
    bf16_t* Cg = (bf16_t*)p.C;
    constexpr int CPR = BN >> 3;
    constexpr int RPP = NTH / CPR;
    constexpr int RIT = (HROWS + RPP - 1) / RPP;
    const int rrow0 = tid / CPR, rc8 = (tid - rrow0 * CPR) * 8;
    const bool ractive = tid < RPP * CPR && n0 + rc8 < p.N;
#ifdef MDX_XL_R2_RESIDUAL
    const bool rpref = NH == 1 && Rg != nullptr && p.wide && !geglu;
#else
    const bool rpref = Rg != nullptr && p.wide && !geglu;
#endif
    uint4 rpre[RIT];
    auto fetch_residual = [&](int hh) {
        const int mh_ = m0 + hh * HROWS;
        const int c8 = (n0 + rc8 + 8 > p.N) ? (p.N - 8 - n0 < 0 ? 0 : p.N - 8 - n0) : rc8;
        const bf16_t* rb = Rg + n0 + c8;
        const int rmax = min(HROWS - 1, p.M - 1 - mh_);
#pragma unroll
        for (int u = 0; u < RIT; ++u) {
            const int row = min(rrow0 + u * RPP, rmax);
            rpre[u] = *(const uint4*)(rb + (long)(mh_ + row) * p.ldr);
        }
    };
#pragma unroll 1
    for (int hh = 0; hh < NH; ++hh) {
        if (rpref && NH == 1) fetch_residual(hh);
        xl_wait_lgkm0();
        __builtin_amdgcn_s_barrier();
        asm volatile("" ::: "memory");
        XL_STAMP(6)
        {
            const int fr = lane & 15, fq = lane >> 4;
            auto stage = [&](auto epi_c, auto hast_c) {
                constexpr int EPI = decltype(epi_c)::value;
                constexpr bool HAS_T = decltype(hast_c)::value;
                constexpr bool HOIST = BN != 320 && !HAS_T;
                float4 a4h[HOIST ? TJ : 1], g4h[HOIST ? TJ : 1];
                if constexpr (HOIST) {
#pragma unroll
                    for (int j = 0; j < TJ; ++j) {
                        const int nl = wn * TJ * 16 + j * 16 + 4 * fq;
                        a4h[j] = *(const float4*)(addend + nl);
                        if constexpr (EPI == 1) g4h[j] = *(const float4*)(addend + ((nl + 32) < BN ? nl + 32 : nl));
                    }
                }
#pragma unroll
                for (int i = 0; i < TI; ++i) {
                    const int mt_ = wm * TI * 16 + i * 16;
                    if (NH > 1 && mt_ / HROWS != hh) continue;
                    const int ml = mt_ + fr;
                    int slot = 0;
                    if constexpr (HAS_T) slot = min(min(m0 + ml, p.M - 1) / p.rows_per_b - b0, XL_SLOTS - 1);
                    const float* ad = addend + slot * BN;
                    bf16_t* crow = Cs + (ml - hh * HROWS) * CSTR;
#pragma unroll
                    for (int j = 0; j < TJ; ++j) {
                        if (EPI == 1 && (j & 2)) continue;
                        const int nl = wn * TJ * 16 + j * 16 + 4 * fq;
                        float4 a4;
                        if constexpr (HOIST) a4 = a4h[j]; else a4 = *(const float4*)(ad + nl);
                        const float bb[4] = {a4.x, a4.y, a4.z, a4.w};
                        float o[4];
                        if constexpr (EPI == 1) {
                            float4 g4;
                            if constexpr (HOIST) g4 = g4h[j]; else g4 = *(const float4*)(ad + nl + 32);
                            const float gg[4] = {g4.x, g4.y, g4.z, g4.w};
#pragma unroll
                            for (int e = 0; e < 4; e += 2) {
                                const float x0 = acc[i][j][e] + bb[e], x1 = acc[i][j][e + 1] + bb[e + 1];
                                const f32x2_t gt = {acc[i][(TJ == 4) ? (j | 2) : j][e] + gg[e], acc[i][(TJ == 4) ? (j | 2) : j][e + 1] + gg[e + 1]};
                                const f32x2_t ge = gelu_erf_f2(gt);
                                o[e] = x0 * ge.x; o[e + 1] = x1 * ge.y;
                            }
                        } else {
#pragma unroll
                            for (int e = 0; e < 4; ++e) {
                                float x = acc[i][j][e] + bb[e];
                                if constexpr (EPI == 2) x = silu_f(x);
                                o[e] = x;
                            }
                        }
                        const int cl = EPI == 1 ? ((nl >> 6) * 32 + (nl & 31)) : nl;
                        uint2 ov; ov.x = pack2bf(o[0], o[1]); ov.y = pack2bf(o[2], o[3]);
                        *(uint2*)(crow + cl) = ov;
                    }
                }
            };
            using std::integral_constant;
            if (geglu) {
                if constexpr (BN == 256) stage(integral_constant<int, 1>{}, integral_constant<bool, false>{});
            } else {
                if (has_t) stage(integral_constant<int, 0>{}, integral_constant<bool, true>{});
                else stage(integral_constant<int, 0>{}, integral_constant<bool, false>{});
            }
        }
        XL_STAMP(7)
        xl_wait_lgkm0();
        __builtin_amdgcn_s_barrier();
        asm volatile("" ::: "memory");
        XL_STAMP(4)
#ifdef MDX_XL_ABLATE
        if (p.dbg & 8) continue;
#endif
        const int mh = m0 + hh * HROWS;
        if (p.col_split) {
            const int cs = p.col_split;
            const bool pairs = (cs & 1) == 0;
            const int cpr = BNo >> 1;
            const int total = HROWS * cpr;
            const int bfirst = n0 / cs;
            const int tfirst = n0 - bfirst * cs;
            bool fast_done = false;
            if constexpr (NTH % (BN >> 1) == 0) if (!geglu) {
                fast_done = true;
                constexpr int RPP2 = NTH / (BN >> 1);
                constexpr int UB = 8;
                static_assert((HROWS / RPP2) % UB == 0, "col_split fast epilogue: the row walk has no remainder handling");
                const int c2 = (tid % cpr) * 2, r0 = tid / cpr;
                int b = bfirst, t = tfirst + c2;
                while (t >= cs) { t -= cs; ++b; }
                const bool ok0 = n0 + c2 < p.N, ok1 = n0 + c2 + 1 < p.N;
                const bool split = !pairs && t + 1 >= cs;
                bf16_t* d0 = Cg + (long)b * p.sC + (long)(mh + r0) * p.ldc + t;
                bf16_t* d1 = split ? Cg + (long)(b + 1) * p.sC + (long)(mh + r0) * p.ldc : d0 + 1;
                const bf16_t* src = Cs + r0 * CSTR + c2;
                const int rmax = min(HROWS, p.M - mh);
#pragma unroll 1
                for (int u0 = 0; u0 < HROWS / RPP2; u0 += UB) {
                    unsigned v[UB];
#pragma unroll
                    for (int u = 0; u < UB; ++u) v[u] = *(const unsigned*)(src + (long)(u0 + u) * RPP2 * CSTR);
#pragma unroll
                    for (int u = 0; u < UB; ++u) {
                        const int row = r0 + (u0 + u) * RPP2;
                        if (row >= rmax || !ok0) continue;
                        const long ro = (long)(u0 + u) * RPP2 * p.ldc;
                        if (pairs && ok1) {
                            *(unsigned*)(d0 + ro) = v[u];
                        } else {
                            d0[ro] = (bf16_t)(v[u] & 0xffffu);
                            if (ok1) d1[ro] = (bf16_t)(v[u] >> 16);
                        }
                    }
                }
            }
            if (!fast_done) {
#pragma unroll 1
            for (int idx = tid; idx < total; idx += NTH) {
                const int row = idx / cpr, c2 = (idx - row * cpr) * 2;
                if (mh + row >= p.M || n0 + c2 >= p.N) continue;
                const unsigned v = *(const unsigned*)(Cs + row * CSTR + c2);
                int b = bfirst, t = tfirst + c2;
                while (t >= cs) { t -= cs; ++b; }
                bf16_t* dst = Cg + (long)b * p.sC + (long)(mh + row) * p.ldc + t;
                if (pairs) {
                    *(unsigned*)dst = v;
                } else {
                    *dst = (bf16_t)(v & 0xffffu);
                    if (n0 + c2 + 1 < p.N) {
                        if (t + 1 < cs) dst[1] = (bf16_t)(v >> 16);
                        else Cg[(long)(b + 1) * p.sC + (long)(mh + row) * p.ldc] = (bf16_t)(v >> 16);
                    }
                }
            }
            }
        } else if (rpref) {
            if (NH == 2) fetch_residual(hh);
            const bf16_t* cs_ = Cs + rrow0 * CSTR + rc8;
            bf16_t* cg_ = Cg + (long)(mh + rrow0) * p.ldc + n0 + rc8;
#pragma unroll
            for (int u = 0; u < RIT; ++u) {
                const int row = rrow0 + u * RPP;
                if (!ractive || row >= HROWS || mh + row >= p.M) continue;
                uint4 v = *(const uint4*)(cs_ + u * RPP * CSTR);
                v.x = add2bf(v.x, rpre[u].x); v.y = add2bf(v.y, rpre[u].y); v.z = add2bf(v.z, rpre[u].z); v.w = add2bf(v.w, rpre[u].w);
                *(uint4*)(cg_ + (long)u * RPP * p.ldc) = v;
            }
        } else if (BN != 320 && p.wide && !Rg) {
            const int cpr = BNo >> 3;
            const int total = HROWS * cpr;
#pragma unroll 1
            for (int i0 = 0; i0 < total; i0 += 8 * NTH) {
                uint4 v[8];
#pragma unroll
                for (int u = 0; u < 8; ++u) {
                    const int idx = min(i0 + u * NTH + tid, total - 1);
                    const int row = idx / cpr;
                    v[u] = *(const uint4*)(Cs + row * CSTR + (idx - row * cpr) * 8);
                }
#pragma unroll
                for (int u = 0; u < 8; ++u) {
                    const int idx = i0 + u * NTH + tid;
                    const int row = idx / cpr, c8 = (idx - row * cpr) * 8;
                    if (idx < total && mh + row < p.M && n0o + c8 < Nout) *(uint4*)(Cg + (long)(mh + row) * p.ldc + n0o + c8) = v[u];
                }
            }
        } else if (p.wide) {
            const int cpr = BNo >> 3;
            const int total = HROWS * cpr;
#pragma unroll 1
            for (int i0 = 0; i0 < total; i0 += 4 * NTH) {
                uint4 rv[4];
                int row[4], c8[4];
                bool ok[4];
#pragma unroll
                for (int u = 0; u < 4; ++u) {
                    const int idx = i0 + u * NTH + tid;
                    row[u] = idx / cpr;
                    c8[u] = (idx - row[u] * cpr) * 8;
                    ok[u] = idx < total && mh + row[u] < p.M && n0o + c8[u] < Nout;
                    rv[u] = make_uint4(0, 0, 0, 0);
                    if (Rg && ok[u]) rv[u] = *(const uint4*)(Rg + (long)(mh + row[u]) * p.ldr + n0o + c8[u]);
                }
#pragma unroll
                for (int u = 0; u < 4; ++u) {
                    if (!ok[u]) continue;
                    uint4 v = *(const uint4*)(Cs + row[u] * CSTR + c8[u]);
                    if (Rg) { v.x = add2bf(v.x, rv[u].x); v.y = add2bf(v.y, rv[u].y); v.z = add2bf(v.z, rv[u].z); v.w = add2bf(v.w, rv[u].w); }
                    *(uint4*)(Cg + (long)(mh + row[u]) * p.ldc + n0o + c8[u]) = v;
                }
            }
        } else {
            const int cpr = BNo >> 2;
            const int total = HROWS * cpr;
#pragma unroll 1
            for (int i0 = 0; i0 < total; i0 += 4 * NTH) {
                uint2 rv[4];
                int row[4], c4[4];
                bool ok[4];
#pragma unroll
                for (int u = 0; u < 4; ++u) {
                    const int idx = i0 + u * NTH + tid;
                    row[u] = idx / cpr;
                    c4[u] = (idx - row[u] * cpr) * 4;
                    ok[u] = idx < total && mh + row[u] < p.M && n0o + c4[u] < Nout;
                    rv[u] = make_uint2(0, 0);
                    if (Rg && ok[u]) rv[u] = *(const uint2*)(Rg + (long)(mh + row[u]) * p.ldr + n0o + c4[u]);
                }
#pragma unroll
                for (int u = 0; u < 4; ++u) {
                    if (!ok[u]) continue;
                    uint2 v = *(const uint2*)(Cs + row[u] * CSTR + c4[u]);
                    if (Rg) { v.x = add2bf(v.x, rv[u].x); v.y = add2bf(v.y, rv[u].y); }
                    *(uint2*)(Cg + (long)(mh + row[u]) * p.ldc + n0o + c4[u]) = v;
                }
            }
        }
    }
    XL_STAMP(5)
    if (p.timing && tid == 0) {
        unsigned long long* t = p.timing + 8 * (long)blockIdx.x;
#pragma unroll
        for (int k = 0; k < 8; ++k) t[k] = ts_[k];
    }
#undef XL_STAMP
}

template <bool GEGLU, bool HAS_R>
__global__ __launch_bounds__(512, 2) void gemm_xlp_kernel(GCParams p) {
    using G = Geo<256>;
    constexpr int BM = 256, BN = 256;
    constexpr int TI = G::TI, TJ = G::TJ, TJ0 = G::TJ0, TJ1 = TJ - TJ0, TIH = TI / 2;
    constexpr int A_BYTES = BM * 128, B_BYTES = G::BNP * 128, BUF = A_BYTES + B_BYTES;
    constexpr int PA = G::PA, PB0 = G::PB0, PB1 = G::PB1;
    static_assert(TJ == 4 && TI == 8 && PB0 == PB1, "the register epilogue is written for the 128 x 64 wave tile");
    extern __shared__ __attribute__((aligned(16))) unsigned char smem[];

    const int tid = threadIdx.x, lane = tid & 63;
    const int wave = __builtin_amdgcn_readfirstlane(tid >> 6);
    const int grp = wave >> 2;
    const int wm = wave % G::WM, wn = wave / G::WM;
    const int nt = p.K / 64;
    const unsigned lds0 = (unsigned)(unsigned long long)(lds_void_t*)smem;

    unsigned a_voff[2][PA]; int a_lds[2][PA];
#pragma unroll
    for (int h = 0; h < 2; ++h)
#pragma unroll
        for (int e = 0; e < PA; ++e) {
            const int row0 = a_piece_row0<BN>(h, wave, e);
            a_lds[h][e] = row0 * 128;
            a_voff[h][e] = (unsigned)(((long)piece_lane_row(row0, lane) * p.lda) * 2 + piece_lane_chunk(row0, lane) * 16);
        }
    unsigned b_voff[2][PB0]; int b_lds[2][PB0];
#pragma unroll
    for (int part = 0; part < 2; ++part)
#pragma unroll
        for (int e = 0; e < PB0; ++e) {
            const int row0 = b_piece_row0<BN>(part, wave, e);
            b_lds[part][e] = A_BYTES + row0 * 128;
            b_voff[part][e] = (unsigned)(((long)piece_lane_row(row0, lane) * p.ldw) * 2 + piece_lane_chunk(row0, lane) * 16);
        }
    const int fo0 = frag_off(0, lane, 0), fo1 = frag_off(0, lane, 1);
    const int a_rd = a_tile_row0<BN>(wm, 0) * 128;
    const int b_rd = A_BYTES + b_tile_row0<BN>(wn, 0) * 128;
    const int fr = lane & 15, fq = lane >> 4;

    int bid = blockIdx.x, tm = 0, tn = 0;
    auto advance = [&](int& b) -> bool {
        for (; b < p.nblk; b += (int)gridDim.x)
            if (xl_tile_coords_at(p, b, tm, tn)) return true;
        return false;
    };
    if (!advance(bid)) return;
    int m0 = tm * BM, n0 = tn * BN;
    xl_rsrc_t rsA, rsB;
    auto set_tile = [&](int m, int n) {
        rsA = xl_make_rsrc_bounded(p.A + (long)m * p.lda, (long)(p.M - m) * p.lda * 2);
        rsB = xl_make_rsrc_bounded(p.W + (long)n * p.ldw, (long)(p.N - n) * p.ldw * 2);
    };
    set_tile(m0, n0);

#define XLP_PIECE_A(h, e, T) { if ((T) < nt) xl_glds(rsA, lds0 + ((T) & 1) * BUF + a_lds[h][e], a_voff[h][e], (T) * 128); }
#define XLP_PIECE_B(part, e, T) { if ((T) < nt) xl_glds_b(rsB, lds0 + ((T) & 1) * BUF + b_lds[part][e], b_voff[part][e], (T) * 128); }
#define XLP_ISSUE_A(h, T) { XLP_PIECE_A(h, 0, T) XLP_PIECE_A(h, 1, T) }
#define XLP_ISSUE_B(part, T) { XLP_PIECE_B(part, 0, T) XLP_PIECE_B(part, 1, T) }
#define XLP_PROLOGUE() { XLP_ISSUE_A(0, 0) XLP_ISSUE_B(0, 0) XLP_ISSUE_B(1, 0) XLP_ISSUE_A(1, 0) XLP_ISSUE_A(0, 1) XLP_ISSUE_B(0, 1) XLP_ISSUE_B(1, 1) }

    float4 bq[TJ];
    const bool has_bias = p.bias != nullptr;
    auto load_bias = [&](int n) {
#pragma unroll
        for (int j = 0; j < TJ; ++j) bq[j] = make_float4(0.f, 0.f, 0.f, 0.f);
        if (has_bias) {
#pragma unroll
            for (int j = 0; j < TJ; ++j) {
                const int col = n + wn * 64 + j * 16 + 4 * fq;
                bq[j] = *(const float4*)(p.bias + min(col, p.N - 4));
            }
        }
    };
    load_bias(n0);
    XLP_PROLOGUE()

    constexpr int INFLIGHT = PA + PB0 + PB1;
    constexpr int NST = GEGLU ? TI : 2 * TI;
    bool first = true, counted = false;
    f32x4_t acc[TI][TJ];
    Frag8 af[TIH][2], bfr[TJ][2];
#define XLP_READ_A(h, buf_)                                                                                                       \
    {                                                                                                                             \
        const unsigned char* s_ = smem + (buf_) * BUF + a_rd + (h) * TIH * 2048;                                                  \
        _Pragma("unroll") for (int i = 0; i < TIH; ++i) {                                                                         \
            af[i][0].u = *(const uint4*)(s_ + i * 2048 + fo0);                                                                    \
            af[i][1].u = *(const uint4*)(s_ + i * 2048 + fo1);                                                                    \
        }                                                                                                                         \
    }
#define XLP_READ_B(J0, NJ, buf_)                                                                                                  \
    {                                                                                                                             \
        const unsigned char* s_ = smem + (buf_) * BUF + b_rd;                                                                     \
        _Pragma("unroll") for (int j = (J0); j < (J0) + (NJ); ++j) {                                                              \
            bfr[j][0].u = *(const uint4*)(s_ + j * 2048 + fo0);                                                                   \
            bfr[j][1].u = *(const uint4*)(s_ + j * 2048 + fo1);                                                                   \
        }                                                                                                                         \
    }
#define XLP_MMA(h, J0, NJ)                                                                                                        \
    {                                                                                                                             \
        __builtin_amdgcn_s_setprio(1);                                                                                            \
        _Pragma("unroll") for (int kk = 0; kk < 2; ++kk)                                                                          \
            _Pragma("unroll") for (int i = 0; i < TIH; ++i)                                                                       \
                _Pragma("unroll") for (int j = (J0); j < (J0) + (NJ); ++j)                                                        \
                    acc[(h) * TIH + i][j] = MDX_MFMA_16x16x32(bfr[j][kk].v, af[i][kk].v, acc[(h) * TIH + i][j]);                  \
        __builtin_amdgcn_s_setprio(0);                                                                                            \
    }
#define XLP_SEG_END() { xl_wait_lgkm0(); __builtin_amdgcn_sched_barrier(0); __builtin_amdgcn_s_barrier(); __builtin_amdgcn_sched_barrier(0); }
#define XLP_MMA_END() { __builtin_amdgcn_sched_barrier(0); __builtin_amdgcn_s_barrier(); __builtin_amdgcn_sched_barrier(0); }

    for (;;) {
#pragma unroll
        for (int i = 0; i < TI; ++i)
#pragma unroll
            for (int j = 0; j < TJ; ++j)
#pragma unroll
                for (int r = 0; r < 4; ++r) acc[i][j][r] = 0.f;
        if (nt <= 1) xl_wait_vmcnt<0>();
        else if (first) xl_wait_vmcnt<INFLIGHT>();
        else if (counted) { if (has_bias) xl_wait_vmcnt<INFLIGHT + NST + TJ>(); else xl_wait_vmcnt<INFLIGHT + NST>(); }
        else xl_wait_vmcnt<INFLIGHT>();
        __builtin_amdgcn_s_barrier();
        __builtin_amdgcn_sched_barrier(0);
        if (grp == 1) {
            __builtin_amdgcn_s_barrier();
            __builtin_amdgcn_sched_barrier(0);
        }
        for (int t = 0; t < nt; ++t) {
            const int buf = t & 1;
            XLP_READ_A(0, buf)
            XLP_READ_B(0, TJ0, buf)
            XLP_ISSUE_A(1, t + 1)
            XLP_SEG_END()
            XLP_MMA(0, 0, TJ0)
            XLP_MMA_END()
            XLP_READ_B(TJ0, TJ1, buf)
            XLP_ISSUE_A(0, t + 2)
            XLP_SEG_END()
            XLP_MMA(0, TJ0, TJ1)
            XLP_MMA_END()
            XLP_READ_A(1, buf)
            XLP_ISSUE_B(0, t + 2)
            XLP_SEG_END()
            XLP_MMA(1, TJ0, TJ1)
            XLP_MMA_END()
            XLP_ISSUE_B(1, t + 2)
            if (t + 2 < nt) xl_wait_vmcnt<INFLIGHT>(); else xl_wait_vmcnt<0>();
            XLP_SEG_END()
            XLP_MMA(1, 0, TJ0)
            XLP_MMA_END()
        }
        if (grp == 0) {
            __builtin_amdgcn_s_barrier();
            __builtin_amdgcn_sched_barrier(0);
        }
#pragma unroll
        for (int j = 0; j < TJ; ++j) asm volatile("" : "+v"(bq[j].x), "+v"(bq[j].y), "+v"(bq[j].z), "+v"(bq[j].w));

        int nb = bid + (int)gridDim.x;
        const int cm0 = m0, cn0 = n0;
        const bool has_next = advance(nb);
        if (has_next) {
            m0 = tm * BM; n0 = tn * BN;
            set_tile(m0, n0);
            XLP_PROLOGUE()
        }

        {
            const int No = GEGLU ? p.N / 2 : p.N;
            const int ocol0 = (GEGLU ? cn0 / 2 + wn * 32 : cn0 + wn * 64) + 8 * fq;
            const int rowb = cm0 + wm * (TI * 16) + fr;
            const bool interior = cm0 + BM <= p.M && cn0 + BN <= p.N;
            bf16_t* cg = (bf16_t*)p.C + (long)rowb * p.ldc + ocol0;
            constexpr int NCH = GEGLU ? 1 : 2;
            const bool lo8 = fr < 8;
            const int rA = (fr & 7), rB = 8 + (fr & 7);
            const int cA = lo8 ? 0 : 32, cB = lo8 ? 32 : 0;
            const int rowt = cm0 + wm * (TI * 16);
            bf16_t* cgA = (bf16_t*)p.C + (long)(rowt + rA) * p.ldc + ocol0 + cA;
            bf16_t* cgB = (bf16_t*)p.C + (long)(rowt + rB) * p.ldc + ocol0 + cB;
            uint4 rres[HAS_R ? TI : 1][NCH];
            if (HAS_R) {
#pragma unroll
                for (int i = 0; i < TI; ++i) {
                    if (GEGLU) {
                        rres[HAS_R ? i : 0][0] = *(const uint4*)((const bf16_t*)p.R + (long)min(rowb + 16 * i, p.M - 1) * p.ldr + min(ocol0, No - 8));
                    } else {
                        const int ra = min(rowt + 16 * i + rA, p.M - 1), rb = min(rowt + 16 * i + rB, p.M - 1);
                        rres[HAS_R ? i : 0][0] = *(const uint4*)((const bf16_t*)p.R + (long)ra * p.ldr + min(ocol0 + cA, No - 8));
                        rres[HAS_R ? i : 0][NCH - 1] = *(const uint4*)((const bf16_t*)p.R + (long)rb * p.ldr + min(ocol0 + cB, No - 8));
                    }
                }
            }
#pragma unroll
            for (int i = 0; i < TI; ++i) {
                unsigned tx[TJ], ty[TJ];
#pragma unroll
                for (int j = 0; j < (GEGLU ? 2 : TJ); ++j) {
                    const float bb[4] = {bq[j].x, bq[j].y, bq[j].z, bq[j].w};
                    float o[4];
                    if (GEGLU) {
                        const float gg[4] = {bq[j + 2].x, bq[j + 2].y, bq[j + 2].z, bq[j + 2].w};
#pragma unroll
                        for (int e = 0; e < 4; e += 2) {
                            const f32x2_t ge = gelu_erf_f2(f32x2_t{acc[i][j + 2][e] + gg[e], acc[i][j + 2][e + 1] + gg[e + 1]});
                            o[e] = (acc[i][j][e] + bb[e]) * ge.x; o[e + 1] = (acc[i][j][e + 1] + bb[e + 1]) * ge.y;
                        }
                    } else {
#pragma unroll
                        for (int e = 0; e < 4; ++e) o[e] = acc[i][j][e] + bb[e];
                    }
                    tx[j] = pack2bf(o[0], o[1]); ty[j] = pack2bf(o[2], o[3]);
                }
                uint4 ch[NCH];
#pragma unroll
                for (int c = 0; c < NCH; ++c) {
                    unsigned ax = tx[2 * c], ay = ty[2 * c], bx = tx[2 * c + 1], by = ty[2 * c + 1];
                    { auto r_ = __builtin_amdgcn_permlane32_swap(ax, bx, false, false); ax = r_[0]; bx = r_[1]; }
                    { auto r_ = __builtin_amdgcn_permlane32_swap(ay, by, false, false); ay = r_[0]; by = r_[1]; }
                    { auto r_ = __builtin_amdgcn_permlane16_swap(ax, bx, false, false); ax = r_[0]; bx = r_[1]; }
                    { auto r_ = __builtin_amdgcn_permlane16_swap(ay, by, false, false); ay = r_[0]; by = r_[1]; }
                    ch[c] = make_uint4(ax, ay, bx, by);
                }
                if (GEGLU) {
                    if (HAS_R) {
                        const uint4 r4 = rres[HAS_R ? i : 0][0];
                        ch[0].x = add2bf(ch[0].x, r4.x); ch[0].y = add2bf(ch[0].y, r4.y); ch[0].z = add2bf(ch[0].z, r4.z); ch[0].w = add2bf(ch[0].w, r4.w);
                    }
                    bf16_t* crow = cg + (long)(16 * i) * p.ldc;
                    if (interior) *(uint4*)crow = ch[0];
                    else if (rowb + 16 * i < p.M && ocol0 + 8 <= No) *(uint4*)crow = ch[0];
                } else {
                    uint4 rot;
                    rot.x = (unsigned)__builtin_amdgcn_mov_dpp((int)ch[NCH - 1].x, 0x128, 0xf, 0xf, false);
                    rot.y = (unsigned)__builtin_amdgcn_mov_dpp((int)ch[NCH - 1].y, 0x128, 0xf, 0xf, false);
                    rot.z = (unsigned)__builtin_amdgcn_mov_dpp((int)ch[NCH - 1].z, 0x128, 0xf, 0xf, false);
                    rot.w = (unsigned)__builtin_amdgcn_mov_dpp((int)ch[NCH - 1].w, 0x128, 0xf, 0xf, false);
                    uint4 vA, vB;
                    vA.x = lo8 ? ch[0].x : rot.x; vA.y = lo8 ? ch[0].y : rot.y; vA.z = lo8 ? ch[0].z : rot.z; vA.w = lo8 ? ch[0].w : rot.w;
                    vB.x = lo8 ? rot.x : ch[0].x; vB.y = lo8 ? rot.y : ch[0].y; vB.z = lo8 ? rot.z : ch[0].z; vB.w = lo8 ? rot.w : ch[0].w;
                    if (HAS_R) {
                        const uint4 r0 = rres[HAS_R ? i : 0][0], r1 = rres[HAS_R ? i : 0][NCH - 1];
                        vA.x = add2bf(vA.x, r0.x); vA.y = add2bf(vA.y, r0.y); vA.z = add2bf(vA.z, r0.z); vA.w = add2bf(vA.w, r0.w);
                        vB.x = add2bf(vB.x, r1.x); vB.y = add2bf(vB.y, r1.y); vB.z = add2bf(vB.z, r1.z); vB.w = add2bf(vB.w, r1.w);
                    }
                    bf16_t* pa = cgA + (long)(16 * i) * p.ldc;
                    bf16_t* pb = cgB + (long)(16 * i) * p.ldc;
                    if (interior) {
                        *(uint4*)pa = vA; *(uint4*)pb = vB;
                    } else {
                        if (rowt + 16 * i + rA < p.M && ocol0 + cA + 8 <= No) *(uint4*)pa = vA;
                        if (rowt + 16 * i + rB < p.M && ocol0 + cB + 8 <= No) *(uint4*)pb = vB;
                    }
                }
            }
            counted = interior;
        }
        if (!has_next) break;
        bid = nb;
        first = false;
        load_bias(n0);
    }
#undef XLP_PIECE_A
#undef XLP_PIECE_B
#undef XLP_ISSUE_A
#undef XLP_ISSUE_B
#undef XLP_PROLOGUE
#undef XLP_READ_A
#undef XLP_READ_B
#undef XLP_MMA
#undef XLP_SEG_END
#undef XLP_MMA_END
}

template <int BN>
constexpr size_t xl_smem_bytes() {
    constexpr size_t ring = (size_t)2 * (256 + Geo<BN>::BNP) * 128;
    constexpr size_t epi = (size_t)(BN == 320 ? 128 : 256) * (BN + 8) * 2 + (size_t)XL_SLOTS * BN * sizeof(float);
    return ring > epi ? ring : epi;
}

bool xd_supported(const GCParams& q);
int launch_gemm_xd(const GCParams& q, int cus, hipStream_t st);

template <int BN, bool CONV, int SCHED>
static int launch_xl(const GCParams& p, hipStream_t st) {
    constexpr size_t smem_kxs = (size_t)2 * 272 * 128 + (size_t)2 * Geo<BN>::BNP * 128;
    constexpr size_t smem = (SCHED == 4 && smem_kxs > xl_smem_bytes<BN>()) ? smem_kxs : xl_smem_bytes<BN>();
    static_assert(smem <= 163840, "LDS budget");
    auto kern = gemm_xl_kernel<BN, CONV, SCHED>;
    if (int rc = ensure_dyn_smem((const void*)kern, smem, "xl")) return rc;
    GCParams q = p;
    q.mt = (p.M + 255) / 256; q.nt = (p.N + BN - 1) / BN;
    const int swz = (int)opt(OPT_GEMM_SWZ);
    const int dbg = (int)opt(OPT_XL_DBG);
    q.dbg = dbg;
    q.swz = swz && q.nt > 1 && q.mt >= 64;
    unsigned nblk_raster = 0;
    const int raster = (int)opt(OPT_XL_RASTER);
    if (raster == 0) q.swz = 0;
    if (raster == 2 && q.mt >= 64) {
        raster_shape(q.mt, q.nt, &q.gm, &q.gn);
        if (const int fgm = (int)opt(OPT_XL_GM)) q.gm = fgm < q.mt ? fgm : q.mt;
        if (const int fgn = (int)opt(OPT_XL_GN)) q.gn = fgn < q.nt ? fgn : q.nt;
        const long nb = raster_blocks(q.mt, q.nt, q.gm, q.gn);
        if ((q.mt + q.gm - 1) / q.gm >= 64 && nb < 0x7fffffffL) { q.swz = 2; nblk_raster = (unsigned)nb; }
    }
    const int timing = (int)opt(OPT_XL_TIMING);
    const unsigned nblk_t = q.swz == 2 ? nblk_raster : q.swz ? (unsigned)((q.mt + 7) / 8 * 8 * q.nt) : (unsigned)(q.mt * q.nt);
    q.timing = (timing && p.ws && (long)nblk_t * 64 <= p.ws_bytes) ? (unsigned long long*)p.ws : nullptr;
    const unsigned nblk = nblk_t;
    q.nblk = (int)nblk;
    if constexpr (BN == 256 && !CONV && SCHED == 0) {
        static const int cus = [] { int d = 0, n = 256; if (hipGetDevice(&d) == hipSuccess) (void)hipDeviceGetAttribute(&n, hipDeviceAttributeMultiprocessorCount, d); return n > 0 ? n : 256; }();
        if (opt(OPT_XL_PERSIST) && q.wide && !q.col_split && !q.temb && (q.epi == 0 || q.epi == 1) && !q.timing && nblk >= 2u * (unsigned)cus &&
            (long)q.M * q.lda * 2 > 0 && q.bias != (const float*)q.C) {
            const bool geglu = q.epi == 1, has_r = q.R != nullptr;
            if (geglu && has_r) goto not_persistent;
            if (opt(OPT_XD) && xd_supported(q)) return launch_gemm_xd(q, cus, st);
            {
                auto launch_p = [&](auto kp) -> int {
                    if (int rc = ensure_dyn_smem((const void*)kp, smem, "xlp")) return rc;
                    hipLaunchKernelGGL(kp, dim3((unsigned)cus), dim3(512), smem, st, q);
                    char tag[96];
                    snprintf(tag, sizeof tag, "gemm_xlp_kernel<256x256,%s%s>", geglu ? "geglu" : "gemm", has_r ? "+res" : "");
                    return check_launch(tag);
                };
                if (geglu) return launch_p(gemm_xlp_kernel<true, false>);
                if (has_r) return launch_p(gemm_xlp_kernel<false, true>);
                return launch_p(gemm_xlp_kernel<false, false>);
            }
        }
    not_persistent:;
    }
    hipLaunchKernelGGL(kern, dim3(nblk), dim3(512), smem, st, q);
    char tag[96];
    snprintf(tag, sizeof tag, "gemm_xl_kernel<256x%d,%s>", BN, CONV ? (SCHED == 4 ? "conv,kxs" : "conv") : "gemm");
    return check_launch(tag);
}

bool xl_supported(const GCParams& p, bool conv, int bn) {
    if (p.batch > 1 || p.splitk > 1 || p.c_f32 || (p.N % 4) || (p.K % 64) || p.Vt) return false;
    if (p.col_split && (conv || p.bias || p.temb || p.R || p.epi || (p.sC & 1) || (p.ldc & 1) || p.col_split < 16)) return false;
    if (bn != 256 && bn != 160 && bn != 320) return false;
    if (p.epi == 1 && (bn != 256 || (p.N % 64))) return false;
    if (p.epi == 2) return false;
    if (conv) {
        if (p.kh != 3 || p.kw != 3 || p.ph != 1 || p.pw != 1 || (p.Cin % 64) || !p.cimajor) return false;
        const long span = ((long)(256 / p.Wo + 3) * p.sh * p.Wi + 256L * p.sw + 3 * p.Wi) * p.lda * 2;
        if (span >= 0x40000000L) return false;
    } else if ((long)256 * p.lda * 2 >= 0x40000000L) return false;
    if ((long)bn * p.ldw * 2 >= 0x40000000L) return false;
    if (p.temb && p.epi != 1) {
        const int rows = p.rows_per_b > 0 ? p.rows_per_b : 1;
        if (256 / rows + 2 > XL_SLOTS) return false;
    }
    return true;
}

int launch_gemm_xl(const GCParams& p, bool conv, int bn, hipStream_t st) {
    if (p.rowstat) return set_error(MDX_EINVAL, "gemm_xl: rowstat_out reached a route that does not emit row statistics");
    const int sched = (int)opt(OPT_XL_SCHED);
#define XL_GO(BN_, S_) (conv ? launch_xl<BN_, true, S_>(p, st) : launch_xl<BN_, false, S_>(p, st))
    if (bn == 320) {
#ifdef MDX_XL_KXS
        if (conv && opt(OPT_XL_KXSHARE) && p.sh == 1 && p.sw == 1 && p.Hi == p.Ho && p.Wi == p.Wo && p.Wo >= 2 && (p.K / 64) % 9 == 0 && p.N % 320 == 0)
            return launch_xl<320, true, 4>(p, st);
#endif
        return XL_GO(320, 0);
    }
    if (bn == 256) return sched == 1 ? XL_GO(256, 1) : sched == 2 ? XL_GO(256, 2) : sched == 3 ? XL_GO(256, 3) : XL_GO(256, 0);
    return sched == 1 ? XL_GO(160, 1) : sched == 2 ? XL_GO(160, 2) : sched == 3 ? XL_GO(160, 3) : XL_GO(160, 0);
#undef XL_GO
}

}
```

magicdrive_amd/engine.py:

```python
from __future__ import annotations

from typing import Dict, List, Optional, Sequence, Tuple

import torch

from . import _lib as L
from . import ops as O
from . import packing as PK
from .networks.spec import heads_at

BF16, F32 = torch.bfloat16, torch.float32


def q_prescale(head_dim: int) -> float:
    return float(head_dim) ** -0.5 * 1.4426950408889634


class PackedNet:

    def __init__(self, sd: Dict[str, torch.Tensor], device, dtype=BF16):
        assert dtype in (torch.bfloat16, torch.float16), "the kernels take bf16 or fp16 operands (fp32 accumulate)"
        self.sd = sd
        self.device = device
        self.dtype = dtype
        self.cache: Dict[Tuple, torch.Tensor] = {}

    def has(self, key: str) -> bool:
        return key in self.sd

    def _get(self, tag, keys, fn):
        ck = (tag,) + tuple(keys)
        if ck not in self.cache:
            self.cache[ck] = fn(*[self.sd[k].detach().float() for k in keys]).to(self.device)
        return self.cache[ck]

    def lin(self, key, scale: float = 1.0):
        return self._get(("lin", scale), [key], lambda w: (w.reshape(w.shape[0], -1) * scale).contiguous().to(self.dtype))

    def conv(self, key):
        return self._get("conv", [key], lambda w: PK.pack_conv_weight(w, self.dtype))

    def conv_cin_padded(self, key, cin_pad: int):
        def f(w):
            wp = torch.zeros(w.shape[0], cin_pad, w.shape[2], w.shape[3])
            wp[:, :w.shape[1]] = w
            return PK.pack_conv_weight(wp, self.dtype)
        return self._get(("convpad", cin_pad), [key], f)

    def vec(self, key, scale: float = 1.0):
        return self._get(("vec", scale), [key], lambda v: (v.reshape(-1) * scale).contiguous().to(F32))

    def vec_bf16(self, key):
        return self._get("vecbf", [key], lambda v: v.reshape(-1).contiguous().to(self.dtype))

    def cat_lin(self, keys: Sequence[str], scales: Sequence[float] = ()):
        sc = tuple(scales) if scales else (1.0,) * len(keys)
        return self._get(("catlin",) + sc, keys,
                         lambda *ws: torch.cat([w.reshape(w.shape[0], -1) * f for w, f in zip(ws, sc)], 0).contiguous().to(self.dtype))

    def ln_lin(self, keys: Sequence[str], ln_pre: str, scales: Sequence[float] = ()):
        sc = tuple(scales) if scales else (1.0,) * len(keys)
        allk = list(keys) + [ln_pre + "weight", ln_pre + "bias"]

        def cat(*ts):
            ws, g, b = ts[:-2], ts[-2].reshape(-1), ts[-1].reshape(-1)
            return torch.cat([w.reshape(w.shape[0], -1) * f for w, f in zip(ws, sc)], 0), g, b

        w = self._get(("lnw",) + sc, allk, lambda *ts: (cat(*ts)[0] * cat(*ts)[1][None, :]).contiguous().to(self.dtype))
        b = self._get(("lnb",) + sc, allk, lambda *ts: (cat(*ts)[0] @ cat(*ts)[2]).contiguous().to(F32))
        cs = self._get(("lncs",) + sc, allk, lambda *ts: (cat(*ts)[0] * cat(*ts)[1][None, :]).to(self.dtype).float().sum(1).contiguous())
        return w, b, cs

    def cat_vec(self, keys: Sequence[str]):
        return self._get("catvec", keys, lambda *vs: torch.cat([v.reshape(-1) for v in vs]).contiguous().to(F32))

    def geglu(self, wkey, bkey):
        w = self._get("gegluw", [wkey, bkey], lambda w, b: PK.pack_geglu(w, b, self.dtype)[0])
        b = self._get("geglub", [wkey, bkey], lambda w, b: PK.pack_geglu(w, b, self.dtype)[1])
        return w, b

    def ln_geglu(self, wkey, bkey, ln_pre: str):
        keys = [wkey, bkey, ln_pre + "weight", ln_pre + "bias"]
        fold = lambda w, b, g, be: PK.pack_geglu(w * g.reshape(-1)[None, :], b.reshape(-1) + w @ be.reshape(-1), self.dtype)
        w = self._get("lngegluw", keys, lambda w, b, g, be: fold(w, b, g, be)[0])
        bb = self._get("lngeglub", keys, lambda w, b, g, be: fold(w, b, g, be)[1])
        cs = self._get("lngeglucs", keys, lambda w, b, g, be: fold(w, b, g, be)[0].float().sum(1).contiguous())
        return w, bb, cs

    def folded_affine(self, w2key, b2key, w1key, b1key, b1_scale: float = 1.0):
        keys = [w2key, b2key, w1key, b1key]
        w = self._get(("foldw", b1_scale), keys, lambda w2, b2, w1, b1: (w2 @ w1).contiguous().to(self.dtype))
        b = self._get(("foldb", b1_scale), keys, lambda w2, b2, w1, b1: (w2 @ (b1 * b1_scale) + b2).contiguous().to(F32))
        return w, b

    def gated_affine(self, w1key, b1key, alpha_key: Optional[str], b1_scale: float = 1.0):
        keys = [w1key, b1key] + ([alpha_key] if alpha_key else [])
        gate = lambda a: torch.tanh(a[0].reshape(-1)) if a else None
        w = self._get(("gatew", b1_scale), keys, lambda w1, b1, *a: (w1 if not a else gate(a)[:, None] * w1).contiguous().to(self.dtype))
        b = self._get(("gateb", b1_scale), keys, lambda w1, b1, *a: (b1 * b1_scale if not a else gate(a) * b1 * b1_scale).contiguous().to(F32))
        return w, b

    def table(self, key):
        return self._get("table", [key], lambda t: t.contiguous().to(self.dtype))


class Pool:

    guard = False
    GUARD_SEGMENT = 12 << 20

    def __init__(self, device, dtype=BF16):
        self.device = device
        self.dtype = dtype
        self.free_list: Dict[Tuple, List[torch.Tensor]] = {}
        self.total_bytes = 0

    @staticmethod
    def alloc(n: int, dtype, device) -> torch.Tensor:
        if not Pool.guard:
            return torch.empty(n, dtype=dtype, device=device)
        nbytes = n * torch.empty(0, dtype=dtype).element_size()
        seg = max(Pool.GUARD_SEGMENT, -(-nbytes // (2 << 20)) * (2 << 20))
        raw = torch.empty(seg, dtype=torch.uint8, device=device)
        off = (seg - nbytes) & ~15
        return raw[off:off + nbytes].view(dtype)

    def _alloc(self, n: int, dtype) -> torch.Tensor:
        return Pool.alloc(n, dtype, self.device)

    def get(self, shape, dtype=None) -> torch.Tensor:
        dtype = dtype or self.dtype
        n = 1
        for s in shape:
            n *= int(s)
        key = (n, dtype)
        fl = self.free_list.get(key)
        if fl:
            return fl.pop().view(*shape)
        self.total_bytes += n * torch.empty(0, dtype=dtype).element_size()
        return self._alloc(n, dtype).view(*shape)

    def put(self, t: Optional[torch.Tensor]):
        if t is None:
            return
        base = t.reshape(-1) if t.is_contiguous() else None
        assert base is not None, "only whole contiguous buffers go back to the pool"
        self.free_list.setdefault((base.numel(), base.dtype), []).append(base)


def level_sizes(h: int, w: int, n_levels: int) -> List[Tuple[int, int]]:
    out = [(h, w)]
    for _ in range(n_levels - 1):
        h, w = (h - 1) // 2 + 1, (w - 1) // 2 + 1
        out.append((h, w))
    return out


def skip_geometry(cfg, h: int, w: int) -> List[Tuple[int, int, int]]:
    boc = cfg["block_out_channels"]
    sizes = level_sizes(h, w, len(boc))
    geo = [(sizes[0][0], sizes[0][1], boc[0])]
    for i in range(len(boc)):
        geo += [(sizes[i][0], sizes[i][1], boc[i])] * cfg["layers_per_block"]
        if i + 1 < len(boc):
            geo.append((sizes[i + 1][0], sizes[i + 1][1], boc[i]))
    return geo


class Act:

    __slots__ = ("t", "B", "H", "W", "C")

    def __init__(self, t, B, H, W, C):
        self.t, self.B, self.H, self.W, self.C = t, B, H, W, C

    @property
    def tok(self):
        return self.t.view(self.B * self.H * self.W, self.C)

    @property
    def bhwc(self):
        return self.t.view(self.B, self.H, self.W, self.C)

    @property
    def btc(self):
        return self.t.view(self.B, self.H * self.W, self.C)

    def channels(self, c0: int, c1: int) -> "ActSlice":
        return ActSlice(self, c0, c1)


class ActSlice:

    __slots__ = ("parent", "c0", "B", "H", "W", "C")

    def __init__(self, parent: Act, c0: int, c1: int):
        self.parent, self.c0, self.B, self.H, self.W, self.C = parent, c0, parent.B, parent.H, parent.W, c1 - c0

    @property
    def tok(self):
        return self.parent.tok[:, self.c0:self.c0 + self.C]

    @property
    def bhwc(self):
        return self.parent.bhwc[..., self.c0:self.c0 + self.C]

    @property
    def btc(self):
        return self.parent.btc[..., self.c0:self.c0 + self.C]


class Builder:

    def __init__(self, cfg, device, n_views: int, n_cam: int, ws_mb: int = 64, dtype=BF16):
        self.cfg = cfg
        self.device = device
        self.B = n_views
        self.n_cam = n_cam
        self.dtype = dtype
        self.pool = Pool(device, dtype)
        self.ops: List[object] = []
        self.ws = torch.empty(ws_mb * 1024 * 1024 // 4, dtype=F32, device=device)
        self.groups = cfg["norm_num_groups"]
        self.eps = cfg["norm_eps"]
        pair = cfg["neighboring_view_pair"]
        pair = {int(k): [int(x) for x in v] for k, v in pair.items()}
        self.nattn = cfg.get("neighboring_attn_type", "add")
        if self.nattn not in ("add", "concat", "self"):
            raise NotImplementedError(f"Unknown type: {self.nattn}")
        kv = []
        for i in range(n_views):
            base = (i // n_cam) * n_cam
            srcs = list(range(n_cam)) if self.nattn == "self" else pair[i % n_cam]
            for nb in srcs:
                kv.append(base + nb)
        if self.nattn == "add":
            assert all(len(v) == 2 for v in pair.values()), "the summed cross-view form handles exactly 2 neighbours per view"
        else:
            assert len({len(v) for v in pair.values()}) == 1 and (self.nattn == "self" or len(pair[0]) <= 8), "concat / self: equal source counts, <= 8"
        self.xv_nsrc = n_cam if self.nattn == "self" else len(pair[0])
        assert self.xv_nsrc <= 8, "joint cross-view attention handles <= 8 sources"
        self.kvmap = torch.tensor(kv, dtype=torch.int32, device=device)

    def emit(self, op):
        self.ops.append(op)
        return op

    def new(self, B, H, W, C) -> Act:
        return Act(self.pool.get((B * H * W, C)), B, H, W, C)

    def free(self, a):
        if isinstance(a, ActSlice):
            return
        self.pool.put(a.t if isinstance(a, Act) else a)

    def groupnorm(self, net, pre, x: Act, eps, silu, name) -> Act:
        y = self.new(x.B, x.H, x.W, x.C)
        self.emit(O.GroupNorm(x.btc, y.btc, net.vec(pre + "weight"), net.vec(pre + "bias"), self.groups, eps, silu, ws=self.ws, name=name))
        return y

    def layernorm(self, net, pre, x: torch.Tensor, name) -> torch.Tensor:
        y = self.pool.get(tuple(x.shape))
        self.emit(O.LayerNorm(x, y, net.vec(pre + "weight"), net.vec(pre + "bias"), 1e-5, name=name))
        return y

    @staticmethod
    def wq_of(W: torch.Tensor, M: int, epilogue: int) -> Optional[torch.Tensor]:
        if W.dim() != 2 or not W.is_contiguous() or epilogue not in (L.EPI_NONE, L.EPI_GEGLU) or not L.get_option("XD"):
            return None
        N, K = W.shape
        if K % 128 or K < 640 or N % 16 or ((M + 255) // 256) * ((N + 255) // 256) < 512:
            return None
        wq = getattr(W, "_mdx_wq", None)
        if wq is None:
            wq = PK.pack_wq(W)
            W._mdx_wq = wq
        return wq

    def gemm(self, A, W, N_out, bias=None, R=None, epilogue=L.EPI_NONE, name="", out=None, **kw) -> torch.Tensor:
        C = out if out is not None else self.pool.get((A.shape[0], N_out))
        if "Wq" not in kw and not any(kw.get(k) is not None for k in ("Vt", "temb", "rowstat")) and not kw.get("ln_eps"):
            kw["Wq"] = self.wq_of(W, A.shape[0], epilogue)
        self.emit(O.Gemm(A, W, C, bias=bias, R=R, epilogue=epilogue, ws=self.ws, name=name, **kw))
        return C

    def resnet(self, net, pre, x: Act, temb: "TembTable", name, out=None) -> Act:
        cout = net.sd[pre + "conv1.weight"].shape[0]
        a = self.groupnorm(net, pre + "norm1.", x, self.eps, True, name + ".norm1")
        h = self.new(x.B, x.H, x.W, cout)
        off = temb.offset[pre + "time_emb_proj.weight"]
        self.emit(O.Conv(a.bhwc, net.conv(pre + "conv1.weight"), h.bhwc, bias=net.vec(pre + "conv1.bias"),
                         temb=temb.table[:, off:], sel=temb.sel, temb_sel_stride=temb.sel_stride, temb_b_stride=temb.b_stride,
                         ws=self.ws, name=name + ".conv1"))
        self.free(a)
        b = self.groupnorm(net, pre + "norm2.", h, self.eps, True, name + ".norm2")
        self.free(h)
        if net.has(pre + "conv_shortcut.weight"):
            sc = self.new(x.B, x.H, x.W, cout)
            self.gemm(x.tok, net.lin(pre + "conv_shortcut.weight"), cout, bias=net.vec(pre + "conv_shortcut.bias"), out=sc.tok, name=name + ".shortcut")
        else:
            sc = x
        if out is None:
            out = self.new(x.B, x.H, x.W, cout)
        assert (out.B, out.H, out.W, out.C) == (x.B, x.H, x.W, cout)
        self.emit(O.Conv(b.bhwc, net.conv(pre + "conv2.weight"), out.bhwc, bias=net.vec(pre + "conv2.bias"), R=sc.bhwc, ws=self.ws, name=name + ".conv2"))
        self.free(b)
        if sc is not x:
            self.free(sc)
        return out

    @staticmethod
    def fuses_qkv(B, T, C) -> bool:
        return C == 320 and T % 8 == 0 and B * T >= 8192

    def self_like_attention(self, net, pre, n: torch.Tensor, B, T, C, heads, cross_view: bool, name, ln_pre: Optional[str] = None,
                            ln_scratch: Optional[torch.Tensor] = None, ln_stats: Optional[torch.Tensor] = None) -> torch.Tensor:
        ldv = PK.round_up(T, 8)
        vt = self.pool.get((B, C, ldv))
        qs = q_prescale(C // heads)
        qkv_keys = [pre + "to_q.weight", pre + "to_k.weight", pre + "to_v.weight"]
        if self.fuses_qkv(B, T, C):
            qk = self.pool.get((B * T, 2 * C))
            if ln_pre is not None:
                w, b, cs = net.ln_lin(qkv_keys, ln_pre, (qs, 1.0, 1.0))
                self.emit(O.Gemm(n, w, qk, bias=b, Vt=vt, vt_from=2 * C, vt_T=T, ln_eps=1e-5, ln_csum=cs, ln_scratch=ln_scratch, ln_stats=ln_stats,
                                 ws=self.ws, name=name + ".ln+qkv"))
            else:
                self.emit(O.Gemm(n, net.cat_lin(qkv_keys, (qs, 1.0, 1.0)), qk, Vt=vt, vt_from=2 * C, vt_T=T, ws=self.ws, name=name + ".qkv"))
        else:
            assert ln_pre is None
            qk = self.gemm(n, net.cat_lin([pre + "to_q.weight", pre + "to_k.weight"], (qs, 1.0)), 2 * C, name=name + ".qk")
            self.emit(O.Gemm(net.lin(pre + "to_v.weight"), n.view(B, T, C), vt[:, :, :T], name=name + ".vT"))
        ao = self.pool.get((B * T, C))
        qk3 = qk.view(B, T, 2 * C)
        self.emit(O.Attn(qk3[:, :, :C], qk3[:, :, C:], vt, ao.view(B, T, C), heads=heads, Tk=T, scale=(C // heads) ** -0.5, q_prescaled=True,
                         kvmap=self.kvmap if cross_view else None, nsrc=self.xv_nsrc if cross_view else 1,
                         joint=cross_view and self.nattn != "add", name=name + ".attn"))
        self.pool.put(qk)
        self.pool.put(vt)
        return ao

    ROWSTAT_PARTS = 3
    FOLD_NORM3 = False

    def rowstat(self, M: int) -> torch.Tensor:
        return self.pool.get((self.ROWSTAT_PARTS, M, 2), F32)

    def transformer_block(self, net, pre, h: torch.Tensor, B, T, C, heads, ctx_kv, name, h_stats: Optional[torch.Tensor] = None,
                          out_stats: bool = False):
        fuse_ln = self.fuses_qkv(B, T, C)
        assert (h_stats is not None) == fuse_ln
        M = B * T
        if fuse_ln:
            n1 = self.pool.get(tuple(h.shape))
            ao = self.self_like_attention(net, pre + "attn1.", h, B, T, C, heads, False, name + ".attn1", ln_pre=pre + "norm1.", ln_scratch=n1, ln_stats=h_stats)
            self.pool.put(h_stats)
        else:
            n1 = self.layernorm(net, pre + "norm1.", h, name + ".norm1")
            ao = self.self_like_attention(net, pre + "attn1.", n1, B, T, C, heads, False, name + ".attn1")
        self.pool.put(n1)
        s1 = self.rowstat(M) if fuse_ln else None
        h1 = self.gemm(ao, net.lin(pre + "attn1.to_out.0.weight"), C, bias=net.vec(pre + "attn1.to_out.0.bias"), R=h, rowstat=s1, name=name + ".attn1.out")
        self.pool.put(ao); self.pool.put(h)
        if fuse_ln:
            n2 = self.pool.get(tuple(h1.shape))
            w, b, cs = net.ln_lin([pre + "attn2.to_q.weight"], pre + "norm2.", (q_prescale(C // heads),))
            q2 = self.gemm(h1, w, C, bias=b, ln_eps=1e-5, ln_csum=cs, ln_scratch=n2, ln_stats=s1, name=name + ".attn2.ln+q")
            self.pool.put(s1)
        else:
            n2 = self.layernorm(net, pre + "norm2.", h1, name + ".norm2")
            q2 = self.gemm(n2, net.lin(pre + "attn2.to_q.weight", q_prescale(C // heads)), C, name=name + ".attn2.q")
        self.pool.put(n2)
        Kc, Vtc, S = ctx_kv[pre + "attn2."]
        ao2 = self.pool.get((B * T, C))
        self.emit(O.Attn(q2.view(B, T, C), Kc, Vtc, ao2.view(B, T, C), heads=heads, Tk=S, scale=(C // heads) ** -0.5, q_prescaled=True, name=name + ".attn2"))
        self.pool.put(q2)
        has4 = net.has(pre + "attn4.to_q.weight")
        fold3 = fuse_ln and self.FOLD_NORM3
        s2 = self.rowstat(M) if (fuse_ln and (has4 or fold3)) else None
        h2 = self.gemm(ao2, net.lin(pre + "attn2.to_out.0.weight"), C, bias=net.vec(pre + "attn2.to_out.0.bias"), R=h1, rowstat=s2, name=name + ".attn2.out")
        self.pool.put(ao2); self.pool.put(h1)
        s3 = s2
        if has4:
            if fuse_ln:
                n4 = self.pool.get(tuple(h2.shape))
                ao4 = self.self_like_attention(net, pre + "attn4.", h2, B, T, C, heads, True, name + ".attn4", ln_pre=pre + "norm4.", ln_scratch=n4, ln_stats=s2)
                self.pool.put(s2)
            else:
                n4 = self.layernorm(net, pre + "norm4.", h2, name + ".norm4")
                ao4 = self.self_like_attention(net, pre + "attn4.", n4, B, T, C, heads, True, name + ".attn4")
            self.pool.put(n4)
            bo_scale = 2.0 if self.nattn == "add" else 1.0
            if net.has(pre + "connector.weight"):
                wf, bf_ = net.folded_affine(pre + "connector.weight", pre + "connector.bias", pre + "attn4.to_out.0.weight", pre + "attn4.to_out.0.bias", bo_scale)
            else:
                wf, bf_ = net.gated_affine(pre + "attn4.to_out.0.weight", pre + "attn4.to_out.0.bias",
                                           pre + "connector.alpha" if net.has(pre + "connector.alpha") else None, bo_scale)
            s3 = self.rowstat(M) if fold3 else None
            h3 = self.gemm(ao4, wf, C, bias=bf_, R=h2, rowstat=s3, name=name + ".attn4.out+connector")
            self.pool.put(ao4); self.pool.put(h2)
        else:
            h3 = h2
        if fold3:
            n3 = self.pool.get(tuple(h3.shape))
            wg, bg, csg = net.ln_geglu(pre + "ff.net.0.proj.weight", pre + "ff.net.0.proj.bias", pre + "norm3.")
            g = self.gemm(h3, wg, 4 * C, bias=bg, epilogue=L.EPI_GEGLU, ln_eps=1e-5, ln_csum=csg, ln_scratch=n3, ln_stats=s3, name=name + ".ff.ln+geglu")
            self.pool.put(s3)
        else:
            n3 = self.layernorm(net, pre + "norm3.", h3, name + ".norm3")
            wg, bg = net.geglu(pre + "ff.net.0.proj.weight", pre + "ff.net.0.proj.bias")
            g = self.gemm(n3, wg, 4 * C, bias=bg, epilogue=L.EPI_GEGLU, name=name + ".ff.geglu")
        self.pool.put(n3)
        s4 = self.rowstat(M) if (fuse_ln and out_stats) else None
        h4 = self.gemm(g, net.lin(pre + "ff.net.2.weight"), C, bias=net.vec(pre + "ff.net.2.bias"), R=h3, rowstat=s4, name=name + ".ff.out")
        self.pool.put(g); self.pool.put(h3)
        return (h4, s4) if out_stats else h4

    def transformer2d(self, net, pre, x: Act, heads, ctx_kv, name, out=None) -> Act:
        B, T, C = x.B, x.H * x.W, x.C
        gn = self.groupnorm(net, pre + "norm.", x, 1e-6, False, name + ".norm")
        fuse_ln = self.fuses_qkv(B, T, C)
        hs = self.rowstat(B * T) if fuse_ln else None
        h = self.gemm(gn.tok, net.lin(pre + "proj_in.weight"), C, bias=net.vec(pre + "proj_in.bias"), rowstat=hs, name=name + ".proj_in")
        self.free(gn)
        i = 0
        while net.has(f"{pre}transformer_blocks.{i}.norm1.weight"):
            more = net.has(f"{pre}transformer_blocks.{i + 1}.norm1.weight")
            r = self.transformer_block(net, f"{pre}transformer_blocks.{i}.", h, B, T, C, heads, ctx_kv, f"{name}.tb{i}", h_stats=hs, out_stats=more)
            h, hs = r if more else (r, None)
            i += 1
        if out is None:
            out = self.new(x.B, x.H, x.W, C)
        assert (out.B, out.H, out.W, out.C) == (x.B, x.H, x.W, C)
        self.gemm(h, net.lin(pre + "proj_out.weight"), C, bias=net.vec(pre + "proj_out.bias"), R=x.tok, out=out.tok, name=name + ".proj_out")
        self.pool.put(h)
        return out

    def encoder(self, net, x0: Act, temb, ctx_kv, tag, mid_out=None) -> Tuple[Act, List[Act]]:
        cfg = self.cfg
        skips = [x0]
        x = x0
        nblk = len(cfg["block_out_channels"])
        for i in range(nblk):
            has_attn = cfg["down_block_types"][i].startswith("CrossAttn")
            for j in range(cfg["layers_per_block"]):
                y = self.resnet(net, f"down_blocks.{i}.resnets.{j}.", x, temb, f"{tag}.d{i}.r{j}")
                if has_attn:
                    z = self.transformer2d(net, f"down_blocks.{i}.attentions.{j}.", y, heads_at(cfg, i), ctx_kv, f"{tag}.d{i}.a{j}")
                    self.free(y)
                    y = z
                skips.append(y)
                x = y
            dk = f"down_blocks.{i}.downsamplers.0.conv."
            if net.has(dk + "weight"):
                Ho, Wo = (x.H - 1) // 2 + 1, (x.W - 1) // 2 + 1
                y = self.new(x.B, Ho, Wo, x.C)
                self.emit(O.Conv(x.bhwc, net.conv(dk + "weight"), y.bhwc, bias=net.vec(dk + "bias"), stride=(2, 2), pad=(1, 1), ws=self.ws, name=f"{tag}.d{i}.down"))
                skips.append(y)
                x = y
        m = self.resnet(net, "mid_block.resnets.0.", x, temb, f"{tag}.mid.r0")
        m2 = self.transformer2d(net, "mid_block.attentions.0.", m, heads_at(cfg, nblk - 1), ctx_kv, f"{tag}.mid.a0")
        self.free(m)
        m3 = self.resnet(net, "mid_block.resnets.1.", m2, temb, f"{tag}.mid.r1", out=mid_out)
        self.free(m2)
        return m3, skips

    def decoder_concats(self, net, B: int, x_c: int, skip_geo: Sequence[Tuple[int, int, int]]) -> List[Act]:
        cfg = self.cfg
        geo = list(skip_geo)
        cats = []
        for i in range(len(cfg["block_out_channels"])):
            for j in range(cfg["layers_per_block"] + 1):
                H, W, sc = geo.pop()
                cats.append(self.new(B, H, W, x_c + sc))
                x_c = net.sd[f"up_blocks.{i}.resnets.{j}.conv1.weight"].shape[0]
        assert not geo
        return cats

    def decoder(self, net, x: Act, skips: List[Act], temb, ctx_kv, tag, cats: Optional[List[Act]] = None) -> Act:
        cfg = self.cfg
        nblk = len(cfg["block_out_channels"])
        rev_heads = [heads_at(cfg, k) for k in reversed(range(nblk))]
        n_layers = cfg["layers_per_block"] + 1
        placed = cats is not None
        cats = list(cats) if placed else None
        skips = list(skips)
        cat = None
        if placed:
            cat = cats.pop(0)
            assert isinstance(x, ActSlice) and x.parent is cat and x.c0 == 0, "with pre-placed concats the mid output must live in cats[0]"
        for i in range(nblk):
            has_attn = cfg["up_block_types"][i].startswith("CrossAttn")
            for j in range(n_layers):
                s = skips.pop()
                if cat is None:
                    cat = self.new(x.B, x.H, x.W, x.C + s.C)
                    self.emit(O.Ew(L.EW_COPY, x.tok, cat.tok[:, :x.C], name=f"{tag}.u{i}.cat{j}a"))
                    self.free(x)
                assert cat.C == x.C + s.C and (cat.H, cat.W) == (s.H, s.W)
                if not placed:
                    self.emit(O.Ew(L.EW_COPY, s.tok, cat.tok[:, x.C:], name=f"{tag}.u{i}.cat{j}b"))
                    self.free(s)
                cout = net.sd[f"up_blocks.{i}.resnets.{j}.conv1.weight"].shape[0]
                nxt = None
                if j + 1 < n_layers:
                    nxt = cats.pop(0) if placed else self.new(x.B, x.H, x.W, cout + skips[-1].C)
                    assert (nxt.B, nxt.H, nxt.W, nxt.C) == (x.B, x.H, x.W, cout + skips[-1].C)
                dst = nxt.channels(0, cout) if nxt is not None else None
                y = self.resnet(net, f"up_blocks.{i}.resnets.{j}.", cat, temb, f"{tag}.u{i}.r{j}", out=None if has_attn else dst)
                self.free(cat)
                if has_attn:
                    z = self.transformer2d(net, f"up_blocks.{i}.attentions.{j}.", y, rev_heads[i], ctx_kv, f"{tag}.u{i}.a{j}", out=dst)
                    self.free(y)
                    y = z
                x, cat = y, nxt
            uk = f"up_blocks.{i}.upsamplers.0.conv."
            if net.has(uk + "weight"):
                Ho, Wo = skips[-1].H, skips[-1].W
                up = self.new(x.B, Ho, Wo, x.C)
                self.emit(O.Upsample(x.bhwc, up.bhwc, PK.nearest_index(x.H, Ho).to(self.device), PK.nearest_index(x.W, Wo).to(self.device), name=f"{tag}.u{i}.nearest"))
                self.free(x)
                cat = cats.pop(0) if placed else self.new(x.B, Ho, Wo, x.C + skips[-1].C)
                assert (cat.H, cat.W, cat.C) == (Ho, Wo, x.C + skips[-1].C)
                y = cat.channels(0, x.C)
                self.emit(O.Conv(up.bhwc, net.conv(uk + "weight"), y.bhwc, bias=net.vec(uk + "bias"), ws=self.ws, name=f"{tag}.u{i}.upconv"))
                self.free(up)
                x = y
        assert not placed or not cats
        y = self.groupnorm(net, "conv_norm_out.", x, self.eps, True, f"{tag}.norm_out")
        self.free(x)
        return y


class TembTable:

    def __init__(self, net: PackedNet, rows: int, device, per_sample: bool):
        keys = [k for k in net.sd.keys() if k.endswith("time_emb_proj.weight")]
        self.keys = keys
        self.offset: Dict[str, int] = {}
        off = 0
        for k in keys:
            self.offset[k] = off
            off += net.sd[k].shape[0]
        self.width = off
        self.rows = rows
        self.table = torch.zeros(rows, off, dtype=F32, device=device)
        self.sel = torch.zeros(1, dtype=torch.int32, device=device)
        self.sel_stride = 0 if per_sample else off
        self.b_stride = off if per_sample else 0
        self.t = torch.zeros(rows, dtype=F32, device=device)

    def emit_fill(self, bld: Builder, net: PackedNet, cfg):
        c0 = cfg["block_out_channels"][0]
        dev = bld.device
        sin = torch.empty(self.rows, c0, dtype=F32, device=dev)
        bld.emit(O.TimeEmb(self.t, sin, flip_sin_to_cos=cfg["flip_sin_to_cos"], freq_shift=cfg["freq_shift"], name="temb.sin"))
        h1 = torch.empty(self.rows, 4 * c0, dtype=F32, device=dev)
        h2 = torch.empty(self.rows, 4 * c0, dtype=F32, device=dev)
        act = torch.empty(self.rows, 4 * c0, dtype=net.dtype, device=dev)
        as4 = lambda t: t.view(self.rows, 1, 1, t.shape[1])
        w1 = net.lin("time_embedding.linear_1.weight"); w2 = net.lin("time_embedding.linear_2.weight")
        bld.emit(O.Conv(as4(sin), w1.view(w1.shape[0], 1, 1, w1.shape[1]), as4(h1), bias=net.vec("time_embedding.linear_1.bias"),
                        pad=(0, 0), epilogue=L.EPI_SILU, direct=True, name="temb.linear_1+silu"))
        bld.emit(O.Conv(as4(h1), w2.view(w2.shape[0], 1, 1, w2.shape[1]), as4(h2), bias=net.vec("time_embedding.linear_2.bias"),
                        pad=(0, 0), direct=True, name="temb.linear_2"))
        bld.emit(O.Ew(L.EW_SILU, h2, act, name="temb.silu"))
        wcat = net.cat_lin(self.keys)
        bcat = net.cat_vec([k[:-len("weight")] + "bias" for k in self.keys])
        bld.emit(O.Gemm(act, wcat, self.table, bias=bcat, name="temb.table"))
        self._keep = (sin, h1, h2, act)


def build_context_kv(bld: Builder, net: PackedNet, ctx: torch.Tensor, B: int, S: int) -> Dict[str, Tuple[torch.Tensor, torch.Tensor, int]]:
    out = {}
    D = ctx.shape[-1]
    ldv = PK.round_up(S, 8)
    for k in net.sd.keys():
        if not k.endswith("attn2.to_k.weight"):
            continue
        pre = k[:-len("to_k.weight")]
        C = net.sd[k].shape[0]
        Kc = torch.empty(B, S, C, dtype=net.dtype, device=bld.device)
        Vt = torch.zeros(B, C, ldv, dtype=net.dtype, device=bld.device)
        bld.emit(O.Gemm(ctx.view(B * S, D), net.lin(k), Kc.view(B * S, C), ws=bld.ws, name=pre + "K"))
        bld.emit(O.Gemm(net.lin(pre + "to_v.weight"), ctx, Vt[:, :, :S], name=pre + "vT"))
        out[pre] = (Kc, Vt, S)
    return out
```

magicdrive_amd/flops.py:

```python
from __future__ import annotations

from collections import defaultdict
from typing import Dict, Iterable

from . import ops as O


def kernel_family(op) -> str:
    if isinstance(op, O.Conv):
        return "conv_direct" if op.direct else "gemm_conv_kernel<conv>"
    if isinstance(op, O.Gemm):
        return "gemm_conv_kernel<gemm>"
    if isinstance(op, O.Attn):
        return "attn_kernel"
    if isinstance(op, O.GroupNorm):
        return "groupnorm_kernel"
    if isinstance(op, O.LayerNorm):
        return "layernorm_kernel"
    return "elementwise"


def op_flops(op) -> float:
    if isinstance(op, O.Gemm):
        C = op.C
        batch = C.shape[0] if C.dim() == 3 else 1
        M = C.shape[-2]
        N = op.W.shape[-2]
        K = op.W.shape[-1]
        return 2.0 * batch * M * N * K
    if isinstance(op, O.Conv):
        B, Ho, Wo, Cout = op.Y.shape
        _, kh, kw, Cin = op.Wt.shape
        return 2.0 * B * Ho * Wo * Cout * kh * kw * Cin
    if isinstance(op, O.Attn):
        B, Tq, C = op.Q.shape
        return 4.0 * B * Tq * op.Tk * C * op.nsrc
    return 0.0


def op_bytes(op) -> float:
    def nb(t):
        return 0 if t is None else t.numel() * t.element_size()
    if isinstance(op, O.Gemm):
        return nb(op.A) + nb(op.W) + nb(op.C) + nb(op.R)
    if isinstance(op, O.Conv):
        return nb(op.X) + nb(op.Wt) + nb(op.Y) + nb(op.R)
    if isinstance(op, O.Attn):
        return nb(op.Q) + op.nsrc * (nb(op.K) + op.K.shape[0] * op.K.shape[2] * op.Tk * 2) // max(op.nsrc, 1) + nb(op.O)
    if isinstance(op, (O.GroupNorm, O.LayerNorm)):
        return nb(op.X) + nb(op.Y)
    if isinstance(op, (O.Ew, O.Upsample, O.Layout)):
        return nb(op.X) + nb(op.Y) * (2 if getattr(op, "kind", 0) == 1 else 1)
    return 0.0


def program_flops(ops: Iterable) -> Dict[str, float]:
    out: Dict[str, float] = defaultdict(float)
    for op in ops:
        out[kernel_family(op)] += op_flops(op)
    out["total"] = sum(v for k, v in out.items() if k != "total")
    return dict(out)
```

magicdrive_amd/ops.py:

```python
from __future__ import annotations

from dataclasses import dataclass, field
from typing import Optional

import torch

from . import _lib as L

BF16 = torch.bfloat16
F16 = torch.float16
H16 = (BF16, F16)
F32 = torch.float32


def _p(t: Optional[torch.Tensor]):
    return None if t is None else t.data_ptr()


def _chk(cond: bool, msg: str):
    if not cond:
        raise ValueError(msg)


def _rows2d(t: torch.Tensor):
    _chk(t.dim() == 2 and (t.shape[1] == 1 or t.stride(1) == 1), f"need [M,C] view with unit inner stride, got {tuple(t.shape)} {t.stride()}")
    return t.shape[0], t.shape[1], t.stride(0)


def _nhwc(t: torch.Tensor):
    _chk(t.dim() == 4 and t.stride(3) == 1, f"need [B,H,W,C] view, got {tuple(t.shape)} {t.stride()}")
    B, H, W, Cc = t.shape
    ld = t.stride(2)
    _chk((W == 1 or True) and (H == 1 or t.stride(1) == W * ld) and (B == 1 or t.stride(0) == H * W * ld),
         f"pixels must be dense: shape {tuple(t.shape)} stride {t.stride()}")
    return B, H, W, Cc, ld


@dataclass
class Gemm:
    A: torch.Tensor
    W: torch.Tensor
    C: torch.Tensor
    bias: Optional[torch.Tensor] = None
    R: Optional[torch.Tensor] = None
    temb: Optional[torch.Tensor] = None
    sel: Optional[torch.Tensor] = None
    epilogue: int = L.EPI_NONE
    temb_sel_stride: int = 0
    temb_b_stride: int = 0
    rows_per_b: int = 1
    splitk: int = 0
    ws: Optional[torch.Tensor] = None
    name: str = ""
    Vt: Optional[torch.Tensor] = None
    vt_from: int = 0
    vt_T: int = 0
    ln_eps: float = 0.0
    ln_csum: Optional[torch.Tensor] = None
    ln_scratch: Optional[torch.Tensor] = None
    rowstat: Optional[torch.Tensor] = None
    ln_stats: Optional[torch.Tensor] = None
    Wq: Optional[torch.Tensor] = None
    opcode = L.OP_GEMM

    def lower(self):
        A, W, Cm = self.A, self.W, self.C
        batch = 1
        sA = sW = sC = sR = 0
        if Cm.dim() == 3:
            batch = Cm.shape[0]
            sC = Cm.stride(0)
            if A.dim() == 3:
                sA = A.stride(0); A = A[0]
            if W.dim() == 3:
                sW = W.stride(0); W = W[0]
            C2 = Cm[0]
        else:
            C2 = Cm
        M, K, lda = _rows2d(A)
        N, K2, ldw = _rows2d(W)
        Mc, No, ldc = _rows2d(C2)
        _chk(K == K2 and M == Mc, f"gemm {self.name}: shape mismatch A{tuple(A.shape)} W{tuple(W.shape)} C{tuple(C2.shape)}")
        if self.Vt is not None:
            _chk(self.epilogue == L.EPI_NONE and batch == 1 and No == self.vt_from and 0 < self.vt_from < N and self.vt_T > 0,
                 f"gemm {self.name}: fused V^T output needs a plain epilogue and C with vt_from columns")
            _chk(self.Vt.dim() == 3 and self.Vt.dtype == A.dtype and self.Vt.stride(2) == 1 and self.Vt.shape[1] == N - self.vt_from
                 and self.Vt.shape[0] * self.vt_T == M and self.Vt.shape[2] >= self.vt_T, f"gemm {self.name}: Vt shape {tuple(self.Vt.shape)}")
        else:
            _chk(No == (N // 2 if self.epilogue == L.EPI_GEGLU else N), f"gemm {self.name}: C has {No} cols for N={N}")
        _chk(A.dtype in H16 and W.dtype == A.dtype and Cm.dtype in (A.dtype, F32), f"gemm {self.name}: dtypes")
        d = L.MdxGemmDesc()
        d.A, d.W, d.C = _p(A), _p(W), _p(C2)
        ldr = 0
        if self.R is not None:
            R2 = self.R
            if R2.dim() == 3:
                sR = R2.stride(0); R2 = R2[0]
            _chk(R2.dtype == Cm.dtype and tuple(R2.shape) == tuple(C2.shape), f"gemm {self.name}: residual shape/dtype")
            ldr = R2.stride(0)
            d.R = _p(R2)
        if self.bias is not None:
            _chk(self.bias.dtype == F32 and self.bias.numel() == N, f"gemm {self.name}: bias")
            d.bias = _p(self.bias)
        if self.temb is not None:
            _chk(self.temb.dtype == F32, "temb must be fp32")
            d.temb = _p(self.temb)
        if self.sel is not None:
            _chk(self.sel.dtype == torch.int32, "sel must be int32")
            d.sel_ptr = _p(self.sel)
        if self.ws is not None:
            d.ws = _p(self.ws); d.ws_bytes = self.ws.numel() * self.ws.element_size()
        d.M, d.N, d.K = M, N, K
        d.lda, d.ldw, d.ldc, d.ldr = lda, ldw, ldc, ldr
        d.batch, d.sA, d.sW, d.sC, d.sR = batch, sA, sW, sC, sR
        d.temb_sel_stride, d.temb_b_stride, d.rows_per_b = self.temb_sel_stride, self.temb_b_stride, self.rows_per_b
        d.epilogue, d.splitk, d.c_is_f32 = self.epilogue, self.splitk, int(Cm.dtype == F32)
        if self.Vt is not None:
            d.Vt = _p(self.Vt)
            d.vt_from, d.vt_T, d.vt_ld, d.vt_stride = self.vt_from, self.vt_T, self.Vt.stride(1), self.Vt.stride(0)
        if self.ln_eps > 0:
            _chk(batch == 1 and self.ln_csum is not None and self.ln_csum.dtype == F32 and self.ln_csum.numel() == N, f"gemm {self.name}: ln_csum")
            _chk(self.ln_scratch is None or (self.ln_scratch.dtype == A.dtype and self.ln_scratch.is_contiguous() and self.ln_scratch.numel() >= M * lda),
                 f"gemm {self.name}: ln_scratch must be a contiguous [M, lda] buffer of the operand type")
            d.ln_eps, d.ln_csum, d.ln_scratch = float(self.ln_eps), _p(self.ln_csum), _p(self.ln_scratch)
            if self.ln_stats is not None:
                st = self.ln_stats
                _chk(st.dtype == F32 and st.dim() == 3 and st.is_contiguous() and st.shape[1] == M and st.shape[2] == 2, f"gemm {self.name}: ln_stats must be fp32 [parts, M, 2]")
                d.ln_stats, d.ln_stats_parts = _p(st), st.shape[0]
        else:
            _chk(self.ln_stats is None, f"gemm {self.name}: ln_stats without ln_eps")
        if self.rowstat is not None:
            rs = self.rowstat
            _chk(rs.dtype == F32 and rs.dim() == 3 and rs.is_contiguous() and rs.shape[1] == M and rs.shape[2] == 2 and rs.shape[0] >= 1,
                 f"gemm {self.name}: rowstat must be fp32 [parts, M, 2]")
            _chk(batch == 1 and self.epilogue == L.EPI_NONE and self.Vt is None and Cm.dtype in H16, f"gemm {self.name}: rowstat needs a plain 2-D GEMM with 16-bit C")
            d.rowstat_out, d.rowstat_parts = _p(rs), rs.shape[0]
        if self.Wq is not None:
            _chk(batch == 1 and self.Wq.dtype == W.dtype and self.Wq.is_contiguous() and self.Wq.numel() == (N + 255) // 256 * 256 * K and K % 32 == 0,
                 f"gemm {self.name}: Wq must be packing.pack_wq(W)")
            d.Wq = _p(self.Wq)
        return self.opcode, d


@dataclass
class Conv:
    X: torch.Tensor
    Wt: torch.Tensor
    Y: torch.Tensor
    bias: Optional[torch.Tensor] = None
    R: Optional[torch.Tensor] = None
    temb: Optional[torch.Tensor] = None
    sel: Optional[torch.Tensor] = None
    stride: tuple = (1, 1)
    pad: tuple = (1, 1)
    pad_end: Optional[tuple] = None
    epilogue: int = L.EPI_NONE
    temb_sel_stride: int = 0
    temb_b_stride: int = 0
    direct: bool = False
    splitk: int = 0
    ws: Optional[torch.Tensor] = None
    name: str = ""

    @property
    def opcode(self):
        return L.OP_CONV_DIRECT if self.direct else L.OP_CONV

    def lower(self):
        B, Hi, Wi, Cin, ldx = _nhwc(self.X)
        B2, Ho, Wo, Cout, ldy = _nhwc(self.Y)
        Co2, kh, kw, Ci2 = self.Wt.shape
        _chk(self.Wt.is_contiguous() and self.Wt.dtype in H16, f"conv {self.name}: weights must be packed bf16 / fp16")
        _chk(B == B2 and Cout == Co2 and Cin == Ci2, f"conv {self.name}: shape mismatch")
        sh, sw = self.stride
        ph, pw = self.pad
        phe, pwe = self.pad_end if self.pad_end is not None else self.pad
        _chk(Ho == (Hi + ph + phe - kh) // sh + 1 and Wo == (Wi + pw + pwe - kw) // sw + 1, f"conv {self.name}: output size")
        d = L.MdxConvDirectDesc() if self.direct else L.MdxConvDesc()
        d.X, d.Wt, d.Y = _p(self.X), _p(self.Wt), _p(self.Y)
        if self.R is not None:
            rB, rH, rW, rC, ldr = _nhwc(self.R)
            _chk((rB, rH, rW, rC) == (B, Ho, Wo, Cout) and self.R.dtype == self.Y.dtype, f"conv {self.name}: residual")
            d.R, d.ldr = _p(self.R), ldr
        if self.bias is not None:
            _chk(self.bias.dtype == F32 and self.bias.numel() == Cout, f"conv {self.name}: bias")
            d.bias = _p(self.bias)
        if self.temb is not None:
            d.temb = _p(self.temb)
        if self.sel is not None:
            d.sel_ptr = _p(self.sel)
        d.B, d.Hi, d.Wi, d.Cin, d.Ho, d.Wo, d.Cout = B, Hi, Wi, Cin, Ho, Wo, Cout
        d.kh, d.kw, d.sh, d.sw, d.ph, d.pw = kh, kw, sh, sw, ph, pw
        d.ldx, d.ldy = ldx, ldy
        d.temb_sel_stride, d.temb_b_stride = self.temb_sel_stride, self.temb_b_stride
        d.epilogue = self.epilogue
        if self.direct:
            d.x_is_f32 = int(self.X.dtype == F32)
            d.y_is_f32 = int(self.Y.dtype == F32)
        else:
            _chk(self.X.dtype == self.Wt.dtype and self.Y.dtype == self.Wt.dtype, f"conv {self.name}: the MFMA path takes one 16-bit type")
            d.splitk = self.splitk
            if self.ws is not None:
                d.ws = _p(self.ws); d.ws_bytes = self.ws.numel() * self.ws.element_size()
        return self.opcode, d


@dataclass
class Attn:
    Q: torch.Tensor
    K: torch.Tensor
    Vt: torch.Tensor
    O: torch.Tensor
    heads: int
    Tk: int
    scale: float
    kvmap: Optional[torch.Tensor] = None
    nsrc: int = 1
    name: str = ""
    joint: bool = False
    q_prescaled: bool = False
    opcode = L.OP_ATTN

    def lower(self):
        Q, K, Vt, O = self.Q, self.K, self.Vt, self.O
        B, Tq, Cc = Q.shape
        _chk(Q.stride(2) == 1 and K.stride(2) == 1 and O.stride(2) == 1 and Vt.stride(2) == 1, f"attn {self.name}: inner strides")
        _chk(Cc % self.heads == 0 and K.shape[2] == Cc and Vt.shape[1] == Cc and O.shape == Q.shape, f"attn {self.name}: shapes")
        _chk(K.shape[1] == self.Tk and Vt.shape[2] >= self.Tk and Vt.shape[0] == K.shape[0], f"attn {self.name}: kv shapes")
        d = L.MdxAttnDesc()
        d.Q, d.K, d.Vt, d.O = _p(Q), _p(K), _p(Vt), _p(O)
        if self.kvmap is not None:
            _chk(self.kvmap.dtype == torch.int32 and self.kvmap.numel() == B * self.nsrc, f"attn {self.name}: kvmap")
            d.kvmap = _p(self.kvmap)
        else:
            _chk(self.nsrc == 1 and K.shape[0] == B, f"attn {self.name}: identity kv map needs Bkv == B")
        d.B, d.H, d.Tq, d.Tk, d.d, d.nsrc = B, self.heads, Tq, self.Tk, Cc // self.heads, self.nsrc
        d.ldq, d.sQ = Q.stride(1), Q.stride(0)
        d.ldk, d.sK = K.stride(1), K.stride(0)
        d.ldv, d.sV = Vt.stride(1), Vt.stride(0)
        d.ldo, d.sO = O.stride(1), O.stride(0)
        d.scale = float(self.scale)
        d.joint = int(self.joint)
        d.q_prescaled = int(self.q_prescaled)
        _chk(self.nsrc >= 1 and (self.nsrc <= 8 if self.joint else self.nsrc <= 2), f"attn {self.name}: nsrc={self.nsrc} (joint={self.joint})")
        return self.opcode, d


@dataclass
class GroupNorm:
    X: torch.Tensor
    Y: torch.Tensor
    gamma: torch.Tensor
    beta: torch.Tensor
    groups: int
    eps: float
    silu: bool = False
    ws: Optional[torch.Tensor] = None
    name: str = ""
    opcode = L.OP_GROUPNORM

    def lower(self):
        B, HW, Cc = self.X.shape
        _chk(self.X.stride(2) == 1 and self.Y.stride(2) == 1 and self.Y.shape == self.X.shape, f"gn {self.name}: layout")
        _chk(B == 1 or (self.X.stride(0) == HW * self.X.stride(1) and self.Y.stride(0) == HW * self.Y.stride(1)), f"gn {self.name}: batch stride")
        _chk(self.gamma.dtype == F32 and self.beta.dtype == F32 and self.gamma.numel() == Cc, f"gn {self.name}: affine")
        d = L.MdxGroupNormDesc()
        d.X, d.Y, d.gamma, d.beta = _p(self.X), _p(self.Y), _p(self.gamma), _p(self.beta)
        d.B, d.HW, d.C, d.G, d.ldx, d.ldy = B, HW, Cc, self.groups, self.X.stride(1), self.Y.stride(1)
        d.eps, d.silu = float(self.eps), int(self.silu)
        if self.ws is not None:
            d.ws = _p(self.ws); d.ws_bytes = self.ws.numel() * self.ws.element_size()
        return self.opcode, d


@dataclass
class LayerNorm:
    X: torch.Tensor
    Y: torch.Tensor
    gamma: torch.Tensor
    beta: torch.Tensor
    eps: float = 1e-5
    name: str = ""
    opcode = L.OP_LAYERNORM

    def lower(self):
        M, Cc, ldx = _rows2d(self.X)
        M2, C2, ldy = _rows2d(self.Y)
        _chk(M == M2 and Cc == C2, f"ln {self.name}: shapes")
        d = L.MdxLayerNormDesc()
        d.X, d.Y, d.gamma, d.beta = _p(self.X), _p(self.Y), _p(self.gamma), _p(self.beta)
        d.M, d.C, d.ldx, d.ldy, d.eps = M, Cc, ldx, ldy, float(self.eps)
        return self.opcode, d


@dataclass
class Softmax:
    X: torch.Tensor
    Y: torch.Tensor
    T: int
    scale: float = 1.0
    name: str = ""
    opcode = L.OP_SOFTMAX

    def lower(self):
        _chk(self.X.dtype == F32 and self.Y.dtype in H16 and self.X.dim() == 2 and self.Y.dim() == 2, "softmax: dtypes / rank")
        _chk(self.X.stride(1) == 1 and self.Y.stride(1) == 1 and self.X.shape[0] == self.Y.shape[0], "softmax: layout")
        _chk(0 < self.T <= self.X.shape[1] and self.T <= self.Y.shape[1], "softmax: T")
        d = L.MdxSoftmaxDesc()
        d.X, d.Y, d.rows, d.T, d.ldx, d.ldy, d.scale = _p(self.X), _p(self.Y), self.X.shape[0], self.T, self.X.stride(0), self.Y.stride(0), float(self.scale)
        _chk(self.Y.shape[1] == self.Y.stride(0), "softmax: Y rows must be dense (the pad columns are written)")
        return self.opcode, d


@dataclass
class Ew:
    kind: int
    X: torch.Tensor
    Y: torch.Tensor
    alpha: float = 1.0
    name: str = ""
    opcode = L.OP_EW
# ... 251 lines not shown
```

magicdrive_amd/packing.py:

```python
from __future__ import annotations

import numpy as np
import torch


def pack_conv_weight(w: torch.Tensor, dtype=torch.bfloat16) -> torch.Tensor:
    assert w.dim() == 4
    return w.detach().permute(0, 2, 3, 1).contiguous().to(dtype)


def pack_linear_weight(w: torch.Tensor, dtype=torch.bfloat16) -> torch.Tensor:
    assert w.dim() == 2
    return w.detach().contiguous().to(dtype)


def pack_geglu(w: torch.Tensor, b: torch.Tensor, dtype=torch.bfloat16):
    two_f, k = w.shape
    f = two_f // 2
    assert two_f == 2 * f and f % 32 == 0, f"GEGLU inner dim {f} must be a multiple of 32"
    wv = w[:f].reshape(f // 32, 32, k)
    wg = w[f:].reshape(f // 32, 32, k)
    wp = torch.stack([wv, wg], dim=1).reshape(two_f, k)
    bv = b[:f].reshape(f // 32, 32)
    bg = b[f:].reshape(f // 32, 32)
    bp = torch.stack([bv, bg], dim=1).reshape(two_f)
    return wp.contiguous().to(dtype), bp.contiguous().to(torch.float32)


def pack_wq(w: torch.Tensor) -> torch.Tensor:
    n, k = w.shape
    assert k % 32 == 0, f"pack_wq: K={k} must be a multiple of 32"
    npad = round_up(n, 256)
    wp = w if npad == n else torch.cat([w, torch.zeros(npad - n, k, dtype=w.dtype, device=w.device)], 0)
    return wp.reshape(npad // 16, 16, k // 32, 4, 8).permute(0, 2, 3, 1, 4).contiguous().reshape(npad, k)


def nearest_index(n_in: int, n_out: int) -> torch.Tensor:
    scale = np.float32(n_in) / np.float32(n_out)
    dst = np.arange(n_out, dtype=np.float32)
    src = np.minimum(np.floor(dst * scale).astype(np.int64), n_in - 1)
    return torch.from_numpy(src.astype(np.int32))


def round_up(x: int, m: int) -> int:
    return (x + m - 1) // m * m
```

magicdrive_amd/vae.py:

```python
from __future__ import annotations

from typing import List

import torch

from . import _lib as L
from . import ops as O
from . import packing as PK
from .engine import PackedNet, Pool

BF16, F32 = torch.bfloat16, torch.float32
ZPAD = 8


def _vae_attention(plan, net, x, a, G, eps, buf, emit):
    return VaeDecodePlan._attention(plan, net, x, a, G, eps, buf, emit)


class VaeEncodePlan:

    def __init__(self, vcfg, net: PackedNet, device, n_img: int, image_hw):
        self.vcfg, self.device, self.n = vcfg, device, n_img
        H, W = image_hw
        G, eps = vcfg["norm_num_groups"], 1e-6
        zc = vcfg["latent_channels"]
        cin = vcfg.get("in_channels", 3)
        self.ops: List[object] = []
        self.keep: List[torch.Tensor] = []
        self.ws = torch.empty(64 * 1024 * 1024 // 4, dtype=F32, device=device)
        emit = self.ops.append
        H16 = net.dtype

        def buf(*shape, dtype=H16, zero=False):
            n_ = 1
            for d_ in shape:
                n_ *= int(d_)
            t = Pool.alloc(n_, dtype, device).view(*shape)
            if zero:
                t.zero_()
            self.keep.append(t)
            return t

        def gn(x, pre, silu):
            y = buf(*x.shape)
            n_, h_, w_, C = x.shape
            emit(O.GroupNorm(x.view(n_, h_ * w_, C), y.view(n_, h_ * w_, C), net.vec(pre + "weight"), net.vec(pre + "bias"), G, eps, silu, ws=self.ws, name="vae." + pre))
            return y

        def conv3(x, key, R=None):
            wt = net.conv(key + "weight")
            y = buf(x.shape[0], x.shape[1], x.shape[2], wt.shape[0])
            emit(O.Conv(x, wt, y, bias=net.vec(key + "bias"), R=R, ws=self.ws, name="vae." + key))
            return y

        def resnet(x, pre):
            a = gn(x, pre + "norm1.", True)
            hcv = conv3(a, pre + "conv1.")
            b = gn(hcv, pre + "norm2.", True)
            sc = x
            if net.has(pre + "conv_shortcut.weight"):
                cout = net.sd[pre + "conv_shortcut.weight"].shape[0]
                sc = buf(x.shape[0], x.shape[1], x.shape[2], cout)
                emit(O.Gemm(x.view(-1, x.shape[3]), net.lin(pre + "conv_shortcut.weight"), sc.view(-1, cout), bias=net.vec(pre + "conv_shortcut.bias"),
                            ws=self.ws, name="vae." + pre + "shortcut"))
            return conv3(b, pre + "conv2.", R=sc)

        self.x_in = torch.zeros(n_img, cin, H, W, dtype=F32, device=device)
        xp = buf(n_img, H, W, ZPAD, zero=True)
        emit(O.Layout(self.x_in, xp[..., :cin], True, name="vae.x.nhwc"))
        c0 = net.sd["encoder.conv_in.weight"].shape[0]
        x = buf(n_img, H, W, c0)
        emit(O.Conv(xp, net.conv_cin_padded("encoder.conv_in.weight", ZPAD), x, bias=net.vec("encoder.conv_in.bias"), ws=self.ws, name="vae.enc.conv_in"))
        nlev = len(vcfg["block_out_channels"])
        for i in range(nlev):
            for j in range(vcfg["layers_per_block"]):
                x = resnet(x, f"encoder.down_blocks.{i}.resnets.{j}.")
            if i != nlev - 1:
                key = f"encoder.down_blocks.{i}.downsamplers.0.conv."
                Ho, Wo = (x.shape[1] + 1 - 3) // 2 + 1, (x.shape[2] + 1 - 3) // 2 + 1
                y = buf(n_img, Ho, Wo, x.shape[3])
                emit(O.Conv(x, net.conv(key + "weight"), y, bias=net.vec(key + "bias"), stride=(2, 2), pad=(0, 0), pad_end=(1, 1), ws=self.ws, name="vae." + key))
                x = y
        x = resnet(x, "encoder.mid_block.resnets.0.")
        x = _vae_attention(self, net, x, "encoder.mid_block.attentions.0.", G, eps, buf, emit)
        x = resnet(x, "encoder.mid_block.resnets.1.")
        x = gn(x, "encoder.conv_norm_out.", True)
        m1 = buf(n_img, x.shape[1], x.shape[2], 2 * zc, dtype=F32)
        emit(O.Conv(x, net.conv("encoder.conv_out.weight"), m1, bias=net.vec("encoder.conv_out.bias"), direct=True, name="vae.enc.conv_out"))
        self.moments_nhwc = buf(n_img, x.shape[1], x.shape[2], 2 * zc, dtype=F32)
        emit(O.Conv(m1, net.conv("quant_conv.weight"), self.moments_nhwc, bias=net.vec("quant_conv.bias"), stride=(1, 1), pad=(0, 0), direct=True, name="vae.quant_conv"))
        self.program = None

    def compile(self):
        self.program = O.build_program(self.ops)

    def run(self, x: torch.Tensor) -> torch.Tensor:
        if self.program is None:
            self.compile()
        with torch.cuda.device(self.device):
            self.x_in.copy_(x.to(self.device, F32))
            self.program.run(torch.cuda.current_stream(self.device).cuda_stream)
            return self.moments_nhwc.permute(0, 3, 1, 2).contiguous()

    def release(self):
        if self.program is not None:
            self.program.destroy()
        self.program = None
        self.ops, self.keep = [], []


class VaeDecodePlan:
    def __init__(self, vcfg, net: PackedNet, device, n_img: int, latent_hw):
        self.vcfg, self.device, self.n = vcfg, device, n_img
        h, w = latent_hw
        G, eps = vcfg["norm_num_groups"], 1e-6
        zc = vcfg["latent_channels"]
        self.ops: List[object] = []
        self.keep: List[torch.Tensor] = []
        self.ws = torch.empty(64 * 1024 * 1024 // 4, dtype=F32, device=device)
        emit = self.ops.append

        H16 = net.dtype

        def buf(*shape, dtype=H16, zero=False):
            n_ = 1
            for d_ in shape:
                n_ *= int(d_)
            t = Pool.alloc(n_, dtype, device).view(*shape)
            if zero:
                t.zero_()
            self.keep.append(t)
            return t

        def gn(x, pre, silu):
            y = buf(*x.shape)
            n_, H, W, C = x.shape
            emit(O.GroupNorm(x.view(n_, H * W, C), y.view(n_, H * W, C), net.vec(pre + "weight"), net.vec(pre + "bias"), G, eps, silu, ws=self.ws, name="vae." + pre))
            return y

        def conv3(x, key, R=None, name=""):
            wt = net.conv(key + "weight")
            y = buf(x.shape[0], x.shape[1], x.shape[2], wt.shape[0])
            emit(O.Conv(x, wt, y, bias=net.vec(key + "bias"), R=R, ws=self.ws, name="vae." + key))
            return y

        def resnet(x, pre):
            a = gn(x, pre + "norm1.", True)
            hcv = conv3(a, pre + "conv1.")
            b = gn(hcv, pre + "norm2.", True)
            sc = x
            if net.has(pre + "conv_shortcut.weight"):
                cout = net.sd[pre + "conv_shortcut.weight"].shape[0]
                sc = buf(x.shape[0], x.shape[1], x.shape[2], cout)
                emit(O.Gemm(x.view(-1, x.shape[3]), net.lin(pre + "conv_shortcut.weight"), sc.view(-1, cout), bias=net.vec(pre + "conv_shortcut.bias"),
                            ws=self.ws, name="vae." + pre + "shortcut"))
            return conv3(b, pre + "conv2.", R=sc)

        self.z_in = torch.zeros(n_img, zc, h, w, dtype=F32, device=device)
        z_nhwc = buf(n_img, h, w, zc, dtype=F32)
        emit(O.Layout(self.z_in, z_nhwc, True, name="vae.z.nhwc"))
        zq = buf(n_img, h, w, ZPAD, zero=True)
        emit(O.Conv(z_nhwc, net.conv("post_quant_conv.weight"), zq[..., :zc], bias=net.vec("post_quant_conv.bias"), stride=(1, 1), pad=(0, 0),
                    direct=True, name="vae.post_quant_conv"))
        top = net.sd["decoder.conv_in.weight"].shape[0]
        x = buf(n_img, h, w, top)
        emit(O.Conv(zq, net.conv_cin_padded("decoder.conv_in.weight", ZPAD), x, bias=net.vec("decoder.conv_in.bias"), ws=self.ws, name="vae.conv_in"))
        x = resnet(x, "decoder.mid_block.resnets.0.")
        x = self._attention(net, x, "decoder.mid_block.attentions.0.", G, eps, buf, emit)
        x = resnet(x, "decoder.mid_block.resnets.1.")
        nlev = len(vcfg["block_out_channels"])
        for i in range(nlev):
            for j in range(vcfg["layers_per_block"] + 1):
                x = resnet(x, f"decoder.up_blocks.{i}.resnets.{j}.")
            if i != nlev - 1:
                H2, W2 = 2 * x.shape[1], 2 * x.shape[2]
                up = buf(n_img, H2, W2, x.shape[3])
                emit(O.Upsample(x, up, PK.nearest_index(x.shape[1], H2).to(device), PK.nearest_index(x.shape[2], W2).to(device), name=f"vae.up{i}.nearest"))
                x = conv3(up, f"decoder.up_blocks.{i}.upsamplers.0.conv.")
        x = gn(x, "decoder.conv_norm_out.", True)
        oc = vcfg["out_channels"]
        self.out_nhwc = buf(n_img, x.shape[1], x.shape[2], oc, dtype=F32)
        emit(O.Conv(x, net.conv("decoder.conv_out.weight"), self.out_nhwc, bias=net.vec("decoder.conv_out.bias"), direct=True, name="vae.conv_out"))
        self.program = None

    def _attention(self, net, x, a, G, eps, buf, emit):
        n, H, W, C = x.shape
        T = H * W
        Tp = PK.round_up(T, 8)
        t = buf(n, H, W, C)
        emit(O.GroupNorm(x.view(n, T, C), t.view(n, T, C), net.vec(a + "group_norm.weight"), net.vec(a + "group_norm.bias"), G, eps, False, ws=self.ws, name="vae.attn.gn"))
        qk = buf(n * T, 2 * C)
        emit(O.Gemm(t.view(n * T, C), net.cat_lin([a + "to_q.weight", a + "to_k.weight"]), qk, bias=net.cat_vec([a + "to_q.bias", a + "to_k.bias"]),
                    ws=self.ws, name="vae.attn.qk"))
        vt = buf(n, C, Tp, zero=True)
        emit(O.Gemm(net.lin(a + "to_v.weight"), t.view(n, T, C), vt[:, :, :T], name="vae.attn.vT"))
        qk3 = qk.view(n, T, 2 * C)
        S = buf(n, T, Tp, dtype=F32)
        emit(O.Gemm(qk3[:, :, :C], qk3[:, :, C:], S[:, :, :T], name="vae.attn.scores"))
        P = buf(n * T, Tp)
        emit(O.Softmax(S.view(n * T, Tp), P, T, scale=float(C) ** -0.5, name="vae.attn.softmax"))
        o = buf(n, T, C)
        emit(O.Gemm(P.view(n, T, Tp), vt, o, name="vae.attn.pv"))
        wo = net.lin(a + "to_out.0.weight")
        bo = net._get("vae_attn_bias", [a + "to_out.0.weight", a + "to_out.0.bias", a + "to_v.bias"], lambda w, b, bv: (w @ bv + b).contiguous().to(F32))
        y = buf(n, H, W, C)
        emit(O.Gemm(o.view(n * T, C), wo, y.view(n * T, C), bias=bo, R=x.view(n * T, C), ws=self.ws, name="vae.attn.out"))
        return y

    def compile(self):
        self.program = O.build_program(self.ops)

    def run(self, z: torch.Tensor) -> torch.Tensor:
        if self.program is None:
            self.compile()
        with torch.cuda.device(self.device):
            self.z_in.copy_(z.to(self.device, F32))
            self.program.run(torch.cuda.current_stream(self.device).cuda_stream)
            return self.out_nhwc.permute(0, 3, 1, 2).contiguous()

    def release(self):
        if self.program is not None:
            self.program.destroy()
        self.program = None
        self.ops, self.keep = [], []
```

Baseline: 7.382 scenes/s.

## Fold nearest-2x upsample into phase-decomposed 2x2 convs for UNet upsamplers

Replaces the nearest-upsample followed by a 3x3 conv with four (or more, when cropping) 2x2 phase convolutions on the low-resolution input, using pre-folded weights. The XL GEMM kernel gains a TAPS=4 variant that maps M-tiles to phases and scatters outputs to strided positions. This removes the upsampled intermediate buffer and cuts conv MACs by about 9/4 per output. The cost is more complex tile mapping and strided epilogue stores, and the rounding order changes slightly because the weights are pre-summed in bf16.

```diff
diff --git a/include/mdx.h b/include/mdx.h
--- a/include/mdx.h
+++ b/include/mdx.h
@@ -12,7 +12,7 @@
 #define MDX_ELAUNCH (-2)
 #define MDX_EUNSUPPORTED (-3)
 
-#define MDX_ABI_VERSION 10
+#define MDX_ABI_VERSION 11
 
 #define MDX_EPI_NONE 0
 #define MDX_EPI_GEGLU 1
@@ -49,7 +49,8 @@
     int64_t ldx, ldy, ldr;
     int64_t temb_sel_stride, temb_b_stride;
     int64_t epilogue, splitk;
-    int64_t ws_bytes, reserved1;
+    int64_t ws_bytes;
+    int64_t upsample2x;
 } MdxConvDesc;
 int mdx_conv2d_bf16(const MdxConvDesc* d, void* stream);
 
diff --git a/magicdrive_amd/_lib.py b/magicdrive_amd/_lib.py
--- a/magicdrive_amd/_lib.py
+++ b/magicdrive_amd/_lib.py
@@ -7,7 +7,7 @@
 _HERE = os.path.dirname(os.path.abspath(__file__))
 LIB_PATH = os.environ.get("MDX_LIB_PATH") or os.path.join(_HERE, "libmdx.so")
 
-ABI_VERSION = 10
+ABI_VERSION = 11
 
 OP_GEMM, OP_CONV, OP_CONV_DIRECT, OP_ATTN, OP_GROUPNORM, OP_LAYERNORM = 1, 2, 3, 4, 5, 6
 OP_EW, OP_FOURIER, OP_GATHER, OP_TIMEEMB, OP_DDIM, OP_UNIPC, OP_SOFTMAX = 7, 8, 9, 10, 11, 12, 13
@@ -31,7 +31,7 @@
                       "temb_sel_stride temb_b_stride rows_per_b epilogue splitk c_is_f32 ws_bytes") + _f(P, "Vt") + _f(I, "vt_from vt_T vt_ld vt_stride")
                       + _f(D, "ln_eps") + _f(P, "ln_csum ln_scratch") + _f(P, "rowstat_out") + _f(I, "rowstat_parts") + _f(P, "ln_stats") + _f(I, "ln_stats_parts") + _f(P, "Wq"))
 MdxConvDesc = _struct("MdxConvDesc", _f(P, "X Wt Y R bias temb sel_ptr ws") + _f(I, "B Hi Wi Cin Ho Wo Cout kh kw sh sw ph pw "
-                      "ldx ldy ldr temb_sel_stride temb_b_stride epilogue splitk ws_bytes reserved1"))
+                      "ldx ldy ldr temb_sel_stride temb_b_stride epilogue splitk ws_bytes upsample2x"))
 MdxConvDirectDesc = _struct("MdxConvDirectDesc", _f(P, "X Wt Y R bias temb sel_ptr reserved_p") + _f(I, "B Hi Wi Cin Ho Wo Cout kh kw sh sw ph pw "
                             "ldx ldy ldr temb_sel_stride temb_b_stride epilogue x_is_f32 y_is_f32 reserved0"))
 MdxAttnDesc = _struct("MdxAttnDesc", _f(P, "Q K Vt O kvmap reserved_p") + _f(I, "B H Tq Tk d nsrc ldq sQ ldk sK ldv sV ldo sO")
diff --git a/magicdrive_amd/csrc/gemm_conv.hip b/magicdrive_amd/csrc/gemm_conv.hip
--- a/magicdrive_amd/csrc/gemm_conv.hip
+++ b/magicdrive_amd/csrc/gemm_conv.hip
@@ -366,6 +366,21 @@
         const int wide_on = (int)opt(OPT_EPI_WIDE);
         p.wide = wide_on && !p.c_f32 && (nout % 8) == 0 && (p.ldc % 8) == 0 && (p.sC % 8) == 0 && (((uintptr_t)p.C) & 15) == 0 &&
                  (!p.R || ((p.ldr % 8) == 0 && (p.sR % 8) == 0 && (((uintptr_t)p.R) & 15) == 0));
+    }
+    if (p.up2) {
+        if (!conv) return set_error(MDX_EINVAL, "upsample2x: conv only");
+        int bn_up = 0; double best = 1e300;
+        const int mt = up_mtiles(p);
+        for (int bn : {320, 256}) {
+            if (!xl_supported(p, true, bn)) continue;
+            const long t = (long)mt * ((p.N + bn - 1) / bn);
+            const double a = bn == 320 ? 23.7 : 13.4, b = bn == 320 ? 1.896 : 1.565;
+            const double c = (double)((t + 255) / 256) * (a + b * p.K / 64.0);
+            if (c < best) { best = c; bn_up = bn; }
+        }
+        if (const int xl_bn = (int)opt(OPT_XL_BN)) if ((xl_bn == 320 || xl_bn == 256) && xl_supported(p, true, xl_bn)) bn_up = xl_bn;
+        if (!bn_up) return set_error(MDX_EINVAL, "mdx_conv2d: upsample2x needs Cin %% 64 == 0, Ho in {2 Hi, 2 Hi - 1}, Wo in {2 Wi, 2 Wi - 1}, bias-only epilogue, no split-K; with a cropped axis B * Hi * Wi * ldx * 2 < 2^31");
+        return launch_gemm_xl(p, true, bn_up, st);
     }
     if (!opt(OPT_LN_STATS)) { p.rowstat = nullptr; p.rowstat_parts = 0; p.ln_stats = nullptr; p.ln_stats_parts = 0; }
     if (geglu && (p.N % 64) != 0) return set_error(MDX_EINVAL, "GEGLU needs packed N %% 64 == 0 (N=%d)", p.N);
@@ -637,6 +652,13 @@
     MDX_NEED(need_int(op, "kh * kw", d->kh * d->kw));
     int64_t K = d->kh * d->kw * d->Cin;
     MDX_NEED(need_int(op, "kh * kw * Cin", K));
+    if (d->upsample2x != 0 && d->upsample2x != 1) return set_error(MDX_EINVAL, "%s: upsample2x=%ld must be 0 or 1", op, (long)d->upsample2x);
+    if (d->upsample2x) {
+        if (d->kh != 2 || d->kw != 2 || d->sh != 1 || d->sw != 1 || d->R || d->temb || d->epilogue || d->splitk > 1 || d->B < 1 || d->Hi < 1 || d->Wi < 1 ||
+            (d->Ho != 2 * d->Hi && d->Ho != 2 * d->Hi - 1) || (d->Wo != 2 * d->Wi && d->Wo != 2 * d->Wi - 1))
+            return set_error(MDX_EINVAL, "%s: upsample2x needs kh = kw = 2 (phase weights), stride 1, Ho in {2 Hi, 2 Hi - 1}, Wo in {2 Wi, 2 Wi - 1}, "
+                                         "no residual / temb / activation / split-K", op);
+    }
     MDX_NEED(check_common(op, K, d->ldx, K, d->ldy, d->ldr, d->X, d->Wt, d->Y, "X", "Wt", "Y", "ldx", "ldy"));
     MDX_NEED(check_epilogue_operands(op, d->R, d->bias, d->temb, d->sel_ptr, d->ws, d->temb_sel_stride, d->temb_b_stride));
     if (d->epilogue == MDX_EPI_GEGLU) return set_error(MDX_EINVAL, "conv has no GEGLU epilogue");
@@ -654,5 +676,6 @@
     p.kh = (int)d->kh; p.kw = (int)d->kw; p.sh = (int)d->sh; p.sw = (int)d->sw; p.ph = (int)d->ph; p.pw = (int)d->pw;
     const int cim = (int)opt(OPT_CONV_CIMAJOR);
     p.cimajor = (cim && d->kh * d->kw > 1 && d->Cin % 64 == 0) ? 1 : 0;
+    if (d->upsample2x) { p.up2 = 1; p.upB = (int)d->B; p.splitk = 1; }
     return launch_gemm_conv(p, true, (hipStream_t)stream);
 }
diff --git a/magicdrive_amd/csrc/gemm_params.h b/magicdrive_amd/csrc/gemm_params.h
--- a/magicdrive_amd/csrc/gemm_params.h
+++ b/magicdrive_amd/csrc/gemm_params.h
@@ -26,8 +26,27 @@
     float* rowstat; int rowstat_parts;
     const float* ln_stats; int ln_stats_parts;
     const bf16_t* Wq;
+    int up2, upB;
     int dbg;
 };
+
+struct UpAxis { int cnt, first, pad, par; };
+__host__ __device__ __forceinline__ UpAxis up_axis(int c, int n_in, int n_out) {
+    const int crop = n_out != 2 * n_in;
+    UpAxis a;
+    a.cnt = c == 2 ? 1 : n_in - crop;
+    a.first = c == 2 ? n_in - 1 : 0;
+    a.pad = c == 1 ? 0 : 1;
+    a.par = c == 1 ? 1 : 0;
+    return a;
+}
+__host__ __device__ __forceinline__ int up_mtiles(const GCParams& p) {
+    const int ny = 2 + (p.Ho != 2 * p.Hi), nx = 2 + (p.Wo != 2 * p.Wi);
+    int mt = 0;
+    for (int yc = 0; yc < ny; ++yc)
+        for (int xc = 0; xc < nx; ++xc) mt += (int)(((long)p.upB * up_axis(yc, p.Hi, p.Ho).cnt * up_axis(xc, p.Wi, p.Wo).cnt + 255) / 256);
+    return mt;
+}
 
 __device__ __forceinline__ bool tile_coords_at(const GCParams& p, int bid, int& tm, int& tn) {
     if (!p.swz) { tm = bid % p.mt; tn = bid / p.mt; return true; }
diff --git a/magicdrive_amd/csrc/gemm_xl.hip b/magicdrive_amd/csrc/gemm_xl.hip
--- a/magicdrive_amd/csrc/gemm_xl.hip
+++ b/magicdrive_amd/csrc/gemm_xl.hip
@@ -18,9 +18,18 @@
 }
 __device__ __forceinline__ bool xl_tile_coords(const GCParams& p, int& tm, int& tn) { return xl_tile_coords_at(p, (int)blockIdx.x, tm, tn); }
 
-template <int BN, bool CONV, int SCHED>
+__device__ __forceinline__ int xl_div24(int n, int d, float rd) {
+    const int q = (int)((float)n * rd);
+    const int r = n - q * d;
+    return r < 0 ? q - 1 : r >= d ? q + 1 : q;
+}
+
+template <int BN, bool CONV, int SCHED, int TAPS = 9>
 __global__ __launch_bounds__(512, 2) void gemm_xl_kernel(GCParams p) {
     using G = Geo<BN>;
+    constexpr bool UP = CONV && TAPS == 4;
+    constexpr int KW = UP ? 2 : 3;
+    static_assert(TAPS == 9 || (TAPS == 4 && CONV && SCHED == 0), "tap counts: 9 (3x3) or 4 (2x2 phase of the upsampled-2x conv)");
     constexpr int BM = 256, NTH = 512;
     constexpr int TI = G::TI, TJ = G::TJ, TJ0 = G::TJ0, TJ1 = TJ - TJ0, TIH = TI / 2;
     constexpr int A_BYTES = BM * 128, B_BYTES = G::BNP * 128, BUF = A_BYTES + B_BYTES;
@@ -43,21 +52,43 @@
     unsigned long long ts_[8] = {0, 0, 0, 0, 0, 0, 0, 0};
 #define XL_STAMP(k) if (p.timing) ts_[k] = __builtin_amdgcn_s_memtime();
     XL_STAMP(0)
+    int M_ = p.M, y_org = -p.ph, x_org = -p.pw, sh_ = p.sh, sw_ = p.sw;
+    int up_Hp = 1, up_Wp = 1, up_oy0 = 0, up_ox0 = 0;
+    const bf16_t* Wb = p.W;
+    if constexpr (UP) {
+        const int nx = 2 + (p.Wo != 2 * p.Wi), nph = (2 + (p.Ho != 2 * p.Hi)) * nx;
+        for (int ph = 0; ph < nph; ++ph) {
+            const int yc = ph / nx, xc = ph - yc * nx;
+            const UpAxis ay = up_axis(yc, p.Hi, p.Ho), ax = up_axis(xc, p.Wi, p.Wo);
+            const int rows = p.upB * ay.cnt * ax.cnt, mtp = (rows + 255) / 256;
+            if (tile_m < mtp || ph == nph - 1) {
+                M_ = rows; up_Hp = ay.cnt; up_Wp = ax.cnt;
+                y_org = ay.first - ay.pad; x_org = ax.first - ax.pad;
+                up_oy0 = 2 * ay.first + ay.par; up_ox0 = 2 * ax.first + ax.par;
+                Wb = p.W + (long)ph * p.N * p.ldw;
+                break;
+            }
+            tile_m -= mtp;
+        }
+        sh_ = 1; sw_ = 1;
+    }
     const int m0 = tile_m * BM, n0 = tile_n * BN;
     const int nt = p.K / 64;
 
     long a_base_el;
     int hw = 1, Wo = 1;
+    int tile_b0 = 0, tile_r0 = 0;
     if (CONV) {
-        hw = p.Ho * p.Wo; Wo = p.Wo;
+        hw = UP ? up_Hp * up_Wp : p.Ho * p.Wo; Wo = UP ? up_Wp : p.Wo;
         const int b = m0 / hw, rem = m0 - b * hw;
+        tile_b0 = b; tile_r0 = rem;
         const int oy = rem / Wo, ox = rem - oy * Wo;
-        a_base_el = (((long)b * p.Hi + (oy * p.sh - p.ph)) * p.Wi + (ox * p.sw - p.pw)) * p.lda;
+        a_base_el = (((long)b * p.Hi + (oy * sh_ + y_org)) * p.Wi + (ox * sw_ + x_org)) * p.lda;
     } else {
         a_base_el = (long)m0 * p.lda;
     }
     const xl_rsrc_t rsA = xl_make_rsrc(p.A + a_base_el);
-    const xl_rsrc_t rsB = xl_make_rsrc(p.W + (long)n0 * p.ldw);
+    const xl_rsrc_t rsB = xl_make_rsrc(Wb + (long)n0 * p.ldw);
     const unsigned lds0 = (unsigned)(unsigned long long)(lds_void_t*)smem;
 
     unsigned xs_bits = 0;
@@ -87,21 +118,21 @@
                 xs_bits |= bits << (3 * (2 * h + e));
             } else
             if (CONV) {
-                const int mm = min(m, p.M - 1);
+                const int mm = min(m, M_ - 1);
                 const int b = mm / hw, rem = mm - b * hw;
                 const int oy = rem / Wo, ox = rem - oy * Wo;
-                const int iy0 = oy * p.sh - p.ph, ix0 = ox * p.sw - p.pw;
+                const int iy0 = oy * sh_ + y_org, ix0 = ox * sw_ + x_org;
                 const long pix = ((long)b * p.Hi + iy0) * p.Wi + ix0;
                 a_voff[h][e] = (unsigned)((pix * p.lda - a_base_el) * 2 + cl * 16);
                 unsigned bits = 0;
 #pragma unroll
-                for (int t = 0; t < 9; ++t) {
-                    const int iy = iy0 + t / 3, ix = ix0 + t % 3;
-                    if (m < p.M && (unsigned)iy < (unsigned)p.Hi && (unsigned)ix < (unsigned)p.Wi) bits |= 1u << t;
+                for (int t = 0; t < TAPS; ++t) {
+                    const int iy = iy0 + t / KW, ix = ix0 + t % KW;
+                    if (m < M_ && (unsigned)iy < (unsigned)p.Hi && (unsigned)ix < (unsigned)p.Wi) bits |= 1u << t;
                 }
                 a_taps[h][e] = bits;
             } else {
-                a_voff[h][e] = m < p.M ? (unsigned)(((long)R * p.lda) * 2 + cl * 16) : XL_OOB;
+                a_voff[h][e] = m < M_ ? (unsigned)(((long)R * p.lda) * 2 + cl * 16) : XL_OOB;
             }
         }
     unsigned b_voff[2][UNIT_MAX];
@@ -134,9 +165,9 @@
     const int row_bytes = (int)(p.lda * 2);
     auto a_soff = [&](int T, int& tap) -> int {
         if (CONV) {
-            const int cb = T / 9;
-            tap = T - cb * 9;
-            const int ky = tap / 3, kx = tap - ky * 3;
+            const int cb = T / TAPS;
+            tap = T - cb * TAPS;
+            const int ky = tap / KW, kx = tap - ky * KW;
             return (ky * p.Wi + kx) * row_bytes + cb * 128;
         }
         tap = 0;
@@ -144,7 +175,7 @@
     };
     auto b_soff = [&](int T) -> int {
         if (CONV) {
-            const int cb = T / 9, tap = T - cb * 9;
+            const int cb = T / TAPS, tap = T - cb * TAPS;
             return (tap * p.Cin + cb * 64) * 2;
         }
         return T * 128;
@@ -621,6 +652,18 @@
 #else
     const bool rpref = Rg != nullptr && p.wide && !geglu;
 #endif
+    const float up_rhw = UP ? 1.0f / (float)hw : 0.f, up_rw = UP ? 1.0f / (float)Wo : 0.f;
+    auto c_off = [&](int rt) -> long {
+        if constexpr (UP) {
+            int r = tile_r0 + rt;
+            const int bb = xl_div24(r, hw, up_rhw);
+            r -= bb * hw;
+            const int j = xl_div24(r, Wo, up_rw), i = r - j * Wo;
+            return (((long)(tile_b0 + bb) * p.Ho + (up_oy0 + 2 * j)) * p.Wo + (up_ox0 + 2 * i)) * p.ldc;
+        } else {
+            return (long)(m0 + rt) * p.ldc;
+        }
+    };
     uint4 rpre[RIT];
     auto fetch_residual = [&](int hh) {
         const int mh_ = m0 + hh * HROWS;
@@ -803,7 +846,7 @@
                 for (int u = 0; u < 8; ++u) {
                     const int idx = i0 + u * NTH + tid;
                     const int row = idx / cpr, c8 = (idx - row * cpr) * 8;
-                    if (idx < total && mh + row < p.M && n0o + c8 < Nout) *(uint4*)(Cg + (long)(mh + row) * p.ldc + n0o + c8) = v[u];
+                    if (idx < total && mh + row < M_ && n0o + c8 < Nout) *(uint4*)(Cg + c_off(hh * HROWS + row) + n0o + c8) = v[u];
                 }
             }
         } else if (p.wide) {
@@ -819,7 +862,7 @@
                     const int idx = i0 + u * NTH + tid;
                     row[u] = idx / cpr;
                     c8[u] = (idx - row[u] * cpr) * 8;
-                    ok[u] = idx < total && mh + row[u] < p.M && n0o + c8[u] < Nout;
+                    ok[u] = idx < total && mh + row[u] < M_ && n0o + c8[u] < Nout;
                     rv[u] = make_uint4(0, 0, 0, 0);
                     if (Rg && ok[u]) rv[u] = *(const uint4*)(Rg + (long)(mh + row[u]) * p.ldr + n0o + c8[u]);
                 }
@@ -828,7 +871,7 @@
                     if (!ok[u]) continue;
                     uint4 v = *(const uint4*)(Cs + row[u] * CSTR + c8[u]);
                     if (Rg) { v.x = add2bf(v.x, rv[u].x); v.y = add2bf(v.y, rv[u].y); v.z = add2bf(v.z, rv[u].z); v.w = add2bf(v.w, rv[u].w); }
-                    *(uint4*)(Cg + (long)(mh + row[u]) * p.ldc + n0o + c8[u]) = v;
+                    *(uint4*)(Cg + c_off(hh * HROWS + row[u]) + n0o + c8[u]) = v;
                 }
             }
         } else {
@@ -844,7 +887,7 @@
                     const int idx = i0 + u * NTH + tid;
                     row[u] = idx / cpr;
                     c4[u] = (idx - row[u] * cpr) * 4;
-                    ok[u] = idx < total && mh + row[u] < p.M && n0o + c4[u] < Nout;
+                    ok[u] = idx < total && mh + row[u] < M_ && n0o + c4[u] < Nout;
                     rv[u] = make_uint2(0, 0);
                     if (Rg && ok[u]) rv[u] = *(const uint2*)(Rg + (long)(mh + row[u]) * p.ldr + n0o + c4[u]);
                 }
@@ -853,7 +896,7 @@
                     if (!ok[u]) continue;
                     uint2 v = *(const uint2*)(Cs + row[u] * CSTR + c4[u]);
                     if (Rg) { v.x = add2bf(v.x, rv[u].x); v.y = add2bf(v.y, rv[u].y); }
-                    *(uint2*)(Cg + (long)(mh + row[u]) * p.ldc + n0o + c4[u]) = v;
+                    *(uint2*)(Cg + c_off(hh * HROWS + row[u]) + n0o + c4[u]) = v;
                 }
             }
         }
@@ -1151,15 +1194,15 @@
 bool xd_supported(const GCParams& q);
 int launch_gemm_xd(const GCParams& q, int cus, hipStream_t st);
 
-template <int BN, bool CONV, int SCHED>
+template <int BN, bool CONV, int SCHED, int TAPS = 9>
 static int launch_xl(const GCParams& p, hipStream_t st) {
     constexpr size_t smem_kxs = (size_t)2 * 272 * 128 + (size_t)2 * Geo<BN>::BNP * 128;
     constexpr size_t smem = (SCHED == 4 && smem_kxs > xl_smem_bytes<BN>()) ? smem_kxs : xl_smem_bytes<BN>();
     static_assert(smem <= 163840, "LDS budget");
-    auto kern = gemm_xl_kernel<BN, CONV, SCHED>;
+    auto kern = gemm_xl_kernel<BN, CONV, SCHED, TAPS>;
     if (int rc = ensure_dyn_smem((const void*)kern, smem, "xl")) return rc;
     GCParams q = p;
-    q.mt = (p.M + 255) / 256; q.nt = (p.N + BN - 1) / BN;
+    q.mt = TAPS == 4 ? up_mtiles(p) : (p.M + 255) / 256; q.nt = (p.N + BN - 1) / BN;
     const int swz = (int)opt(OPT_GEMM_SWZ);
     const int dbg = (int)opt(OPT_XL_DBG);
     q.dbg = dbg;
@@ -1203,7 +1246,7 @@
     }
     hipLaunchKernelGGL(kern, dim3(nblk), dim3(512), smem, st, q);
     char tag[96];
-    snprintf(tag, sizeof tag, "gemm_xl_kernel<256x%d,%s>", BN, CONV ? (SCHED == 4 ? "conv,kxs" : "conv") : "gemm");
+    snprintf(tag, sizeof tag, "gemm_xl_kernel<256x%d,%s>", BN, CONV ? (SCHED == 4 ? "conv,kxs" : TAPS == 4 ? "conv,up2x" : "conv") : "gemm");
     return check_launch(tag);
 }
 
@@ -1213,7 +1256,14 @@
     if (bn != 256 && bn != 160 && bn != 320) return false;
     if (p.epi == 1 && (bn != 256 || (p.N % 64))) return false;
     if (p.epi == 2) return false;
-    if (conv) {
+    if (conv && p.up2) {
+        if (bn == 160 || p.kh != 2 || p.kw != 2 || (p.Cin % 64) || p.R || p.temb || p.epi || p.col_split) return false;
+        if (p.upB < 1 || p.Hi < 1 || p.Wi < 1 || (p.Ho != 2 * p.Hi && p.Ho != 2 * p.Hi - 1) || (p.Wo != 2 * p.Wi && p.Wo != 2 * p.Wi - 1)) return false;
+        if ((long)p.Hi * p.Wi + 256 >= (1L << 24) || (long)p.upB * p.Hi * p.Wi >= 0x7fffff00L) return false;
+        const long span = ((long)(256 / p.Wi + 3) * p.Wi + 256L + 2 * p.Wi) * p.lda * 2;
+        if (span >= 0x40000000L) return false;
+        if ((p.Ho != 2 * p.Hi || p.Wo != 2 * p.Wi) && ((long)p.upB * p.Hi * p.Wi + p.Wi + 2) * p.lda * 2 >= 0x7fff0000L) return false;
+    } else if (conv) {
         if (p.kh != 3 || p.kw != 3 || p.ph != 1 || p.pw != 1 || (p.Cin % 64) || !p.cimajor) return false;
         const long span = ((long)(256 / p.Wo + 3) * p.sh * p.Wi + 256L * p.sw + 3 * p.Wi) * p.lda * 2;
         if (span >= 0x40000000L) return false;
@@ -1229,6 +1279,10 @@
 int launch_gemm_xl(const GCParams& p, bool conv, int bn, hipStream_t st) {
     if (p.rowstat) return set_error(MDX_EINVAL, "gemm_xl: rowstat_out reached a route that does not emit row statistics");
     const int sched = (int)opt(OPT_XL_SCHED);
+    if (p.up2) {
+        if (!conv || !xl_supported(p, true, bn)) return set_error(MDX_EINVAL, "gemm_xl: upsampled-2x conv on an unsupported shape");
+        return bn == 320 ? launch_xl<320, true, 0, 4>(p, st) : launch_xl<256, true, 0, 4>(p, st);
+    }
 #define XL_GO(BN_, S_) (conv ? launch_xl<BN_, true, S_>(p, st) : launch_xl<BN_, false, S_>(p, st))
     if (bn == 320) {
 #ifdef MDX_XL_KXS
diff --git a/magicdrive_amd/engine.py b/magicdrive_amd/engine.py
--- a/magicdrive_amd/engine.py
+++ b/magicdrive_amd/engine.py
@@ -39,6 +39,9 @@
 
     def conv(self, key):
         return self._get("conv", [key], lambda w: PK.pack_conv_weight(w, self.dtype))
+
+    def conv_up2x(self, key, crop_h: bool, crop_w: bool):
+        return self._get(("convup2x", bool(crop_h), bool(crop_w)), [key], lambda w: PK.fold_upsample_conv(w, crop_h, crop_w, self.dtype))
 
     def conv_cin_padded(self, key, cin_pad: int):
         def f(w):
@@ -210,7 +213,19 @@
         return self.parent.btc[..., self.c0:self.c0 + self.C]
 
 
+def upsample_conv_folds(device, fold, Hi: int, Wi: int, Ho: int, Wo: int, cin: int, B: int = 0, ldx: int = 0) -> bool:
+    if fold is None:
+        fold = torch.device(device).type == "cuda"
+    if not (bool(fold) and cin % 64 == 0 and Hi * Wi + 256 < (1 << 24) and PK.upsample_fold_ok(Hi, Ho) and PK.upsample_fold_ok(Wi, Wo)):
+        return False
+    if B and (Ho != 2 * Hi or Wo != 2 * Wi) and (B * Hi * Wi + Wi + 2) * (ldx or cin) * 2 >= 0x7fff0000:
+        return False
+    return True
+
+
 class Builder:
+
+    fold_upsample = None
 
     def __init__(self, cfg, device, n_views: int, n_cam: int, ws_mb: int = 64, dtype=BF16):
         self.cfg = cfg
@@ -517,6 +532,15 @@
             uk = f"up_blocks.{i}.upsamplers.0.conv."
             if net.has(uk + "weight"):
                 Ho, Wo = skips[-1].H, skips[-1].W
+                if upsample_conv_folds(self.device, self.fold_upsample, x.H, x.W, Ho, Wo, x.C, B=x.B, ldx=x.bhwc.stride(2)):
+                    cat = cats.pop(0) if placed else self.new(x.B, Ho, Wo, x.C + skips[-1].C)
+                    assert (cat.H, cat.W, cat.C) == (Ho, Wo, x.C + skips[-1].C)
+                    y = cat.channels(0, x.C)
+                    self.emit(O.Conv(x.bhwc, net.conv_up2x(uk + "weight", Ho != 2 * x.H, Wo != 2 * x.W), y.bhwc, bias=net.vec(uk + "bias"), ws=self.ws,
+                                     upsample2x=True, name=f"{tag}.u{i}.upconv"))
+                    self.free(x)
+                    x = y
+                    continue
                 up = self.new(x.B, Ho, Wo, x.C)
                 self.emit(O.Upsample(x.bhwc, up.bhwc, PK.nearest_index(x.H, Ho).to(self.device), PK.nearest_index(x.W, Wo).to(self.device), name=f"{tag}.u{i}.nearest"))
                 self.free(x)
diff --git a/magicdrive_amd/flops.py b/magicdrive_amd/flops.py
--- a/magicdrive_amd/flops.py
+++ b/magicdrive_amd/flops.py
@@ -30,6 +30,8 @@
         return 2.0 * batch * M * N * K
     if isinstance(op, O.Conv):
         B, Ho, Wo, Cout = op.Y.shape
+        if getattr(op, "upsample2x", False):
+            return 2.0 * B * Ho * Wo * Cout * 9 * op.Wt.shape[-1]
         _, kh, kw, Cin = op.Wt.shape
         return 2.0 * B * Ho * Wo * Cout * kh * kw * Cin
     if isinstance(op, O.Attn):
diff --git a/magicdrive_amd/ops.py b/magicdrive_amd/ops.py
--- a/magicdrive_amd/ops.py
+++ b/magicdrive_amd/ops.py
@@ -161,12 +161,38 @@
     splitk: int = 0
     ws: Optional[torch.Tensor] = None
     name: str = ""
+    upsample2x: bool = False
 
     @property
     def opcode(self):
         return L.OP_CONV_DIRECT if self.direct else L.OP_CONV
 
-    def lower(self):
+    def _lower_upsample2x(self):
+        B, Hi, Wi, Cin, ldx = _nhwc(self.X)
+        B2, Ho, Wo, Cout, ldy = _nhwc(self.Y)
+        _chk(self.Wt.dim() == 5 and self.Wt.is_contiguous() and self.Wt.dtype in H16, f"conv {self.name}: upsample2x takes packed phase weights")
+        nph, Co2, kh, kw, Ci2 = self.Wt.shape
+        _chk(B == B2 and Cout == Co2 and Cin == Ci2 and (kh, kw) == (2, 2), f"conv {self.name}: shape mismatch")
+        _chk(Ho in (2 * Hi, 2 * Hi - 1) and Wo in (2 * Wi, 2 * Wi - 1) and nph == (2 + (Ho != 2 * Hi)) * (2 + (Wo != 2 * Wi)), f"conv {self.name}: upsample2x sizes")
+        _chk(not self.direct and self.R is None and self.temb is None and self.epilogue == L.EPI_NONE and tuple(self.stride) == (1, 1),
+             f"conv {self.name}: upsample2x has a bias-only epilogue")
+        _chk(self.X.dtype == self.Wt.dtype and self.Y.dtype == self.Wt.dtype, f"conv {self.name}: the MFMA path takes one 16-bit type")
+        d = L.MdxConvDesc()
+        d.X, d.Wt, d.Y = _p(self.X), _p(self.Wt), _p(self.Y)
+        if self.bias is not None:
+            _chk(self.bias.dtype == F32 and self.bias.numel() == Cout, f"conv {self.name}: bias")
+            d.bias = _p(self.bias)
+        d.B, d.Hi, d.Wi, d.Cin, d.Ho, d.Wo, d.Cout = B, Hi, Wi, Cin, Ho, Wo, Cout
+        d.kh, d.kw, d.sh, d.sw, d.ph, d.pw = 2, 2, 1, 1, 0, 0
+        d.ldx, d.ldy = ldx, ldy
+        d.upsample2x = 1
+        if self.ws is not None:
+            d.ws = _p(self.ws); d.ws_bytes = self.ws.numel() * self.ws.element_size()
+        return self.opcode, d
+
+    def lower(self):
+        if self.upsample2x:
+            return self._lower_upsample2x()
         B, Hi, Wi, Cin, ldx = _nhwc(self.X)
         B2, Ho, Wo, Cout, ldy = _nhwc(self.Y)
         Co2, kh, kw, Ci2 = self.Wt.shape
diff --git a/magicdrive_amd/packing.py b/magicdrive_amd/packing.py
--- a/magicdrive_amd/packing.py
+++ b/magicdrive_amd/packing.py
@@ -42,5 +42,49 @@
     return torch.from_numpy(src.astype(np.int32))
 
 
+
+def upsample_fold_ok(n_in: int, n_out: int) -> bool:
+    return n_in >= 1 and n_out in (2 * n_in, 2 * n_in - 1) and bool(torch.equal(nearest_index(n_in, n_out), torch.arange(n_out, dtype=torch.int32) >> 1))
+
+
+def upsample_axis_classes(n_in: int, n_out: int):
+    crop = int(n_out != 2 * n_in)
+    cls = [(n_in - crop, 0, 1, 0), (n_in - crop, 0, 0, 1)]
+    if crop:
+        cls.append((1, n_in - 1, 1, 0))
+    return cls
+
+
+def _fold_axis(w: torch.Tensor, dim: int, c: int) -> torch.Tensor:
+    w0, w1, w2 = w.unbind(dim)
+    pair = (w0, w1 + w2) if c == 0 else (w0 + w1, w2) if c == 1 else (w0, w1)
+    return torch.stack(pair, dim)
+
+
+def fold_upsample_conv(w: torch.Tensor, crop_h: bool, crop_w: bool, dtype=torch.bfloat16) -> torch.Tensor:
+    assert w.dim() == 4 and w.shape[2:] == (3, 3)
+    ny, nx = 2 + int(crop_h), 2 + int(crop_w)
+    sets = [_fold_axis(_fold_axis(w.detach(), 2, yc), 3, xc).permute(0, 2, 3, 1) for yc in range(ny) for xc in range(nx)]
+    out = torch.stack(sets, 0).contiguous()
+    return out if dtype is None else out.to(dtype)
+
+
+def folded_upsample_conv_reference(x: torch.Tensor, wf: torch.Tensor, Ho: int, Wo: int, bias=None) -> torch.Tensor:
+    import torch.nn.functional as F
+    B, _, Hi, Wi = x.shape
+    ycls, xcls = upsample_axis_classes(Hi, Ho), upsample_axis_classes(Wi, Wo)
+    assert wf.shape[0] == len(ycls) * len(xcls)
+    y = x.new_zeros(B, wf.shape[1], Ho, Wo)
+    for yc, (hn, h0, hp, hpar) in enumerate(ycls):
+        for xc, (wn, w0, wp, wpar) in enumerate(xcls):
+            if hn == 0 or wn == 0:
+                continue
+            w = wf[yc * len(xcls) + xc].to(x.dtype).permute(0, 3, 1, 2)
+            xp = F.pad(x, (1, 1, 1, 1))
+            win = xp[:, :, h0 - hp + 1:h0 - hp + 1 + hn + 1, w0 - wp + 1:w0 - wp + 1 + wn + 1]
+            y[:, :, 2 * h0 + hpar:2 * (h0 + hn - 1) + hpar + 1:2, 2 * w0 + wpar:2 * (w0 + wn - 1) + wpar + 1:2] = F.conv2d(win, w)
+    return y if bias is None else y + bias.to(x.dtype)[None, :, None, None]
+
+
 def round_up(x: int, m: int) -> int:
     return (x + m - 1) // m * m
diff --git a/magicdrive_amd/vae.py b/magicdrive_amd/vae.py
--- a/magicdrive_amd/vae.py
+++ b/magicdrive_amd/vae.py
@@ -7,7 +7,7 @@
 from . import _lib as L
 from . import ops as O
 from . import packing as PK
-from .engine import PackedNet, Pool
+from .engine import PackedNet, Pool, upsample_conv_folds
 
 BF16, F32 = torch.bfloat16, torch.float32
 ZPAD = 8
@@ -110,6 +110,8 @@
 
 
 class VaeDecodePlan:
+    fold_upsample = None
+
     def __init__(self, vcfg, net: PackedNet, device, n_img: int, latent_hw):
         self.vcfg, self.device, self.n = vcfg, device, n_img
         h, w = latent_hw
@@ -174,6 +176,13 @@
                 x = resnet(x, f"decoder.up_blocks.{i}.resnets.{j}.")
             if i != nlev - 1:
                 H2, W2 = 2 * x.shape[1], 2 * x.shape[2]
+                key = f"decoder.up_blocks.{i}.upsamplers.0.conv."
+                if upsample_conv_folds(device, self.fold_upsample, x.shape[1], x.shape[2], H2, W2, x.shape[3], B=n_img):
+                    wt = net.conv_up2x(key + "weight", False, False)
+                    y = buf(n_img, H2, W2, wt.shape[1])
+                    emit(O.Conv(x, wt, y, bias=net.vec(key + "bias"), ws=self.ws, upsample2x=True, name="vae." + key))
+                    x = y
+                    continue
                 up = buf(n_img, H2, W2, x.shape[3])
                 emit(O.Upsample(x, up, PK.nearest_index(x.shape[1], H2).to(device), PK.nearest_index(x.shape[2], W2).to(device), name=f"vae.up{i}.nearest"))
                 x = conv3(up, f"decoder.up_blocks.{i}.upsamplers.0.conv.")
```

Measured after the change: 7.534 scenes/s, median of 6. 1.02x the previous value.
